# Gardlin/PCR-CG

Hardware: AMD Instinct MI355X
Metric: fragment-pairs/s KPFCNN+GCN fwd, 30k-pt pairs (higher is better)
Workload: dtype f32

## Files before the change

include/pcrcg.h:

```cpp
#ifndef PCRCG_H
#define PCRCG_H

#include <stddef.h>
#include <stdint.h>

#ifdef __cplusplus
extern "C" {
#endif

#define PCRCG_OK 0
#define PCRCG_EBADARG (-1)
#define PCRCG_EWORKSPACE (-2)
#define PCRCG_ELAUNCH (-3)
#define PCRCG_ECAPACITY (-4)

#define PCRCG_KPOINTS 15

const char* pcrcg_last_error(void);
#define PCRCG_ABI_VERSION 4
int pcrcg_abi_version(void);

int pcrcg_debug_set(const char* spec);
int pcrcg_debug_release(void);

size_t pcrcg_grid_subsample_ws_bytes(int n, int nb);
int pcrcg_grid_subsample_batch(const float* pts, int n, const int* len, int nb, float dl, int max_p,
                               float* out_pts, int* out_len, int* out_m, void* ws, size_t ws_bytes,
                               void* stream);

size_t pcrcg_umap_order_ws_bytes(int m);
int pcrcg_umap_order(const uint64_t* keys, int m, int* order, void* ws, size_t ws_bytes, void* stream);

size_t pcrcg_cellgrid_ws_bytes(int ns, int nb);
int pcrcg_cellgrid_build(const float* sup, int ns, const int* slen, int nb, float radius, void* grid,
                         size_t grid_bytes, void* stream);
int pcrcg_radius_query(const float* q, int nq, const int* qlen, int ns, const int* slen, int nb,
                       float radius, const void* grid, int cols, int64_t* out_idx, int* out_count,
                       int* out_max_count, int* status, void* stream);
int pcrcg_radius_query_ex(const float* q, int nq, const int* qlen, int ns, const int* slen, int nb,
                          float radius, const void* grid, int cols, int64_t* out_idx, int* out_count,
                          int* out_max_count, int* status, int* out_tie_rows, int* out_tie_count, void* stream);
int pcrcg_radius_query_groups(const float* q, int nq, const int* qlen, int ns, const int* slen, int nb, int group,
                              float radius, const void* grid, int cols, int64_t* out_idx, int* out_count,
                              int* out_max_count, int* status, int* out_tie_rows, int* out_tie_count, void* stream);
int pcrcg_radius_query_cells(const void* qgrid, const float* q, int nq, const int* qlen, const void* sgrid, int ns,
                             const int* slen, int nb, int group, float radius, int cols, int64_t* out_idx, int* out_count,
                             int* out_max_count, int* status, int* out_tie_rows, int* out_tie_count, void* stream);
size_t pcrcg_radius_neighbors_ws_bytes(int ns, int nb);
int pcrcg_radius_neighbors_batch(const float* q, int nq, const float* sup, int ns, const int* qlen,
                                 const int* slen, int nb, float radius, int cols, int64_t* out_idx,
                                 int* out_count, int* out_max_count, int* status, void* ws,
                                 size_t ws_bytes, void* stream);

#define PCRCG_MAX_REORDER_JOBS 12
typedef struct pcrcg_reorder_job {
    const float* q;
    const int* qlen;
    const int* rows;
    const int* count;
    int64_t* idx;
    int nq, nbq, cloud0, nrows, max_count, cols;
    float radius;
    int group;
    const float* sup;
    const void* forest;
    int forest_ns, forest_nb;
} pcrcg_reorder_job;
size_t pcrcg_kdforest_ws_bytes(int ns, int nb);
int pcrcg_kdforest_build(const float* sup, int ns, const int* slen, int nb, void* forest, size_t forest_bytes,
                         void* stream);
int pcrcg_radius_reorder(const float* q, int nq, const int* qlen, int nbq, const float* sup, int ns, int nb,
                         const void* forest, int cloud0, float radius, const int* rows, int nrows, const int* count,
                         int max_count, int cols, int64_t* idx, int* status, void* stream);
int pcrcg_radius_reorder_jobs(const pcrcg_reorder_job* jobs, int njobs, const float* sup, int ns, int nb,
                              const void* forest, int* status, void* stream);

size_t pcrcg_kpconv_ws_bytes(int ns);
int pcrcg_kpconv_aggregate(const float* q_pts, int nq, const float* s_pts, int ns, const int64_t* idx,
                           int h, int ld_idx, const float* x, int cin, const float* kp, float extent,
                           float* wf, float* inv_n, void* ws, size_t ws_bytes, void* stream);
int pcrcg_kpconv_aggregate_bf16(const float* q_pts, int nq, const float* s_pts, int ns, const int64_t* idx, int h,
                                int ld_idx, const float* x, int cin, const float* kp, float extent, void* x_bf16,
                                void* wf_bf16, float* inv_n, void* ws, size_t ws_bytes, void* stream);

int pcrcg_query_walk(const float* points, int n, int* walk, int* key, void* stream);
int pcrcg_kpconv_aggregate_walk(const float* q_pts, int nq, const float* s_pts, int ns, const int64_t* idx,
                                int h, int ld_idx, const float* x, int cin, const float* kp, float extent,
                                float* wf, float* inv_n, void* ws, size_t ws_bytes, const int* walk, void* stream);
int pcrcg_kpconv_aggregate_bf16_walk(const float* q_pts, int nq, const float* s_pts, int ns, const int64_t* idx, int h,
                                     int ld_idx, const float* x, int cin, const float* kp, float extent, void* x_bf16,
                                     void* wf_bf16, float* inv_n, void* ws, size_t ws_bytes, const int* walk, void* stream);
int pcrcg_gather_max_walk(const float* x, int ns, int c, const int64_t* idx, int nq, int h, int ld_idx,
                          float* out, const int* walk, void* stream);

void pcrcg_profile_kpconv(int enable);
int pcrcg_profile_kpconv_read(float* ms, int* nq, int* h, int* cin, int* cout, int* kind, int cap);

int pcrcg_gemm_f32(const float* a, int lda, const float* b, int ldb, int trans_b, float* c, int ldc, int m,
                   int n, int k, const float* row_scale, const float* bias, void* stream);
size_t pcrcg_gemm_colstats_bytes(int m, int n);
int pcrcg_gemm_f32_colstats(const float* a, int lda, const float* b, int ldb, int trans_b, float* c, int ldc,
                            int m, int n, int k, const float* row_scale, const float* bias, void* colstats,
                            size_t colstats_bytes, int* h_chunks, void* stream);
int pcrcg_gemm_bf16a_f32_colstats(const void* a_bf16, int lda, const float* b, int ldb, float* c, int ldc, int m, int n,
                                  int k, const float* row_scale, const float* bias, void* colstats,
                                  size_t colstats_bytes, int* h_chunks, void* stream);

int pcrcg_gemm_f32_fused(const float* a, int lda, const int64_t* idx, int ld_idx, int ns, const float* zero_row,
                         const void* a_sums, double a_count, float a_eps, float a_slope, const float* b, int ldb,
                         const float* bias, float* c, int ldc, int m, int n, int k, int accumulate, void* stream);

void pcrcg_gemm_set_mode(int mode);
int pcrcg_gemm_get_mode(void);
int pcrcg_gemm_redo_counts(unsigned long long* out2, int reset);
void pcrcg_thread_shares_gpu(int on);

int pcrcg_gather_max(const float* x, int ns, int c, const int64_t* idx, int nq, int h, int ld_idx,
                     float* out, void* stream);
int pcrcg_gather_first(const float* x, int ns, int c, const int64_t* idx, int nq, int ld_idx, float* out,
                       int ld_out, void* stream);
size_t pcrcg_instnorm_ws_bytes(int c);
int pcrcg_instnorm_stats_from_partials(const void* partials, int chunks, int c, double count, float eps,
                                       float* stats, void* stream);
int pcrcg_instnorm_stats(const float* x, int n, int c, int ldx, float eps, float* stats, void* ws,
                         size_t ws_bytes, void* stream);
int pcrcg_instnorm_apply(const float* x, int n, int c, int ldx, const float* stats, const float* res,
                         int ldr, const float* res_stats, float slope, float* y, int ldy, void* stream);
int pcrcg_instnorm_colsums(const float* x, int n, int c, int ldx, void* sums, void* stream);
int pcrcg_instnorm_apply_sums(const float* x, int n, int c, int ldx, const void* sums, double count, float eps,
                              const float* res, int ldr, const void* res_sums, float slope, float* y, int ldy,
                              void* stream);

int pcrcg_fill2d(float* dst, int ld, int rows, int cols, float value, void* stream);
int pcrcg_inject_image_features(const float* fmap, int c, int h, int w, const float* valid, const int64_t* inds2d,
                                const int64_t* inds3d, int n, long row_offset, long n_rows, float* x, int ldx,
                                void* stream);

typedef struct pcrcg_image_frame {
    const float* fmap;
    const float* depth;
    const float* valid;
    float world2camera[16];
    float intrinsics[16];
    float thresh;
    int h, w;
    int depth_h, depth_w;
    int target;
} pcrcg_image_frame;

size_t pcrcg_project_depth_ws_bytes(int n);
int pcrcg_project_depth(const float* points, int n, const float* depth, int h, int w, const float* h_world2camera,
                        const float* h_intrinsics, float thresh, int64_t* inds2d, int64_t* inds3d, int* k, void* ws,
                        size_t ws_bytes, void* stream);
int pcrcg_inject_frames(const float* points, long n_points, long len_src, const pcrcg_image_frame* h_frames, int n_frames,
                        int c, float* x, int ldx, void* stream);
int pcrcg_superglue_valid_maps(const float* keypoints0, int n0, const float* keypoints1, int n1, const int64_t* matches,
                               const float* confidence, int window, int map_w, int map_h, float* src_valid, float* tgt_valid,
                               void* stream);

int pcrcg_knn(const float* coords, int n, int k, int* idx, void* stream);
size_t pcrcg_edgeconv_ws_bytes(int c);
int pcrcg_edgeconv_reduce(const float* ctr, int ld_ctr, const float* nbr, int ld_nbr, const int* idx,
                          int n, int k, int c, float eps, float* emax, int ld_emax, float* stats,
                          void* ws, size_t ws_bytes, void* stream);
int pcrcg_edgeconv_reduce_sums(const float* ctr, int ld_ctr, const float* nbr, int ld_nbr, const int* idx, int n, int k,
                               int c, float* emax, int ld_emax, void* sums, void* stream);
int pcrcg_softmax_rows(float* x, int rows, int cols, int ld, float scale, void* stream);
int pcrcg_attention_supported(int d);
int pcrcg_attention(const float* q, int ldq, const float* k, int ldk, const float* v, int ldv, float* out, int ldo, int n,
                    int ms, int heads, int d, float scale, void* stream);
int pcrcg_softmax_matvec(const float* x, int rows, int cols, int ld, float scale, const float* vec, int ldv, float* y,
                         int ldy, void* stream);

int pcrcg_check_status(const int* status, void* stream);

int pcrcg_copy2d(const float* src, int ld_src, float* dst, int ld_dst, int rows, int cols, void* stream);
int pcrcg_add(const float* a, const float* b, float* dst, long n, void* stream);
int pcrcg_l2norm_rows(const float* src, int ld_src, float* dst, int ld_dst, int rows, int cols, void* stream);
int pcrcg_sigmoid_scores(const float* src, int ld_src, float* dst, int rows, void* stream);

#define PCRCG_MAX_LEVELS 8
#define PCRCG_MAX_BLOCKS 32
#define PCRCG_MAX_GNN 8

enum { PCRCG_BLK_SIMPLE = 0, PCRCG_BLK_RESNETB = 1, PCRCG_BLK_UNARY = 2, PCRCG_BLK_LAST_UNARY = 3,
       PCRCG_BLK_UPSAMPLE = 4 };

typedef struct pcrcg_block {
    int type;
    int layer;
    int strided;
    int in_dim, out_dim;
    int mid_dim;
    float extent;
    const float* kp;
    const float* kp_w;
    const float* kp_wt;
    const float* kp_w_pad;
    int cin_pad;
    const float* unary1;
    const float* unary2;
    const float* shortcut;
    const float* mlp;
    int mlp_ld;
    const float* mlp_skip;
    int mlp_skip_ld, skip_dim;
} pcrcg_block;

typedef struct pcrcg_gnn_layer {
    int cross;
    const float* edge1;
    const float* edge2;
    const float* conv3;
    const float *wq, *bq, *wk, *bk, *wv, *bv;
    const float *wm, *bm;
    const float *w0, *b0;
    const float *w3, *b3;
} pcrcg_gnn_layer;

typedef struct pcrcg_model {
    int n_enc, n_dec, n_gnn;
    pcrcg_block enc[PCRCG_MAX_BLOCKS];
    pcrcg_block dec[PCRCG_MAX_BLOCKS];
    pcrcg_gnn_layer gnn[PCRCG_MAX_GNN];
    int enc_skip[PCRCG_MAX_BLOCKS];
    int dec_concat[PCRCG_MAX_BLOCKS];
    int enc_out_dim, gnn_dim, heads, knn_k, final_dim;
    const float *bottle_w, *bottle_b;
    const float *proj_gnn_w, *proj_gnn_b;
    const float *proj_score_w, *proj_score_b;
    float temperature;
    int feature_bf16;
} pcrcg_model;

typedef struct pcrcg_table { const int64_t* idx; int rows, cols, ld; } pcrcg_table;

typedef struct pcrcg_batch {
    int n_levels;
    const float* points[PCRCG_MAX_LEVELS];
    int n_points[PCRCG_MAX_LEVELS];
    pcrcg_table neighbors[PCRCG_MAX_LEVELS], pools[PCRCG_MAX_LEVELS], upsamples[PCRCG_MAX_LEVELS];
    const float* features;
    int feat_dim;
    int len_src_c;
    const int* stack_lengths[PCRCG_MAX_LEVELS];
} pcrcg_batch;

typedef struct pcrcg_outputs {
    float* feats_f;
    float* scores_overlap;
    float* scores_saliency;
} pcrcg_outputs;

size_t pcrcg_kpfcnn_ws_bytes(const pcrcg_model* model, const pcrcg_batch* batch);
int pcrcg_kpfcnn_forward(const pcrcg_model* model, const pcrcg_batch* batch, const pcrcg_outputs* out, void* ws,
                         size_t ws_bytes, void* stream);

size_t pcrcg_kpfcnn_group_ws_bytes(const pcrcg_model* model, const pcrcg_batch* batches, int n);
int pcrcg_kpfcnn_forward_group(const pcrcg_model* model, const pcrcg_batch* batches, const pcrcg_outputs* outs, int n,
                               void* ws, size_t ws_bytes, void* stream);

typedef struct pcrcg_pyramid_cfg {
    int n_levels;
    float r_conv[PCRCG_MAX_LEVELS], r_pool[PCRCG_MAX_LEVELS], dl[PCRCG_MAX_LEVELS];
    int has_conv[PCRCG_MAX_LEVELS], pooled[PCRCG_MAX_LEVELS], limit[PCRCG_MAX_LEVELS];
    int tie_order;
    int group;
    int up_nearest;
    double shrink;
    void* side_stream;
    void* side_stream2;
} pcrcg_pyramid_cfg;
typedef struct pcrcg_pyramid_restore {
    int njobs;
    pcrcg_reorder_job jobs[PCRCG_MAX_REORDER_JOBS];
    int* tie_status;
} pcrcg_pyramid_restore;
size_t pcrcg_pyramid_ws_bytes(int n0, int nb, const pcrcg_pyramid_cfg* cfg);
int pcrcg_pyramid_build(const float* pts, int n0, const int* len, int nb, const pcrcg_pyramid_cfg* cfg, void* ws,
                        size_t ws_bytes, int* h_scratch, pcrcg_batch* out, int* h_lengths, int* h_status,
                        pcrcg_pyramid_restore* deferred, void* stream);
int pcrcg_pyramid_build_parts(const float* const* pts_parts, const int* n_parts, const int* const* len_parts,
                              const int* nb_parts, int parts, const pcrcg_pyramid_cfg* cfg, void* ws, size_t ws_bytes,
                              int* h_scratch, pcrcg_batch* out, int* h_lengths, int* h_status,
                              pcrcg_pyramid_restore* deferred, void* stream);
int pcrcg_pyramid_restore_run(const pcrcg_pyramid_restore* r, int* h_status, void* stream);

int pcrcg_stream_create(void** stream, int priority);
int pcrcg_stream_destroy(void* stream);
int pcrcg_stream_pipe_classes(void* const* streams, int n, int* cls, void* scratch);

typedef struct pcrcg_ransac_trace {
    int* samples;
    int* pass;
    float* xf32;
    double* xf64;
    int* valid_ids;
    int* counts;
    double* sums;
} pcrcg_ransac_trace;

size_t pcrcg_ransac_ws_bytes(int n, int m, int max_iteration, int max_validation);
int pcrcg_feature_match(const float* src_feat, int ld_src, int n, const float* tgt_feat, int ld_tgt, int m, int c, int mutual,
                        int* corr, int* k, void* ws, size_t ws_bytes, void* stream);
int pcrcg_ransac(const float* src, int n, const float* tgt, int m, const void* grid, const int* corr, int k_max, const int* k,
                 int ransac_n, double threshold, double edge_similarity, int distance_check, int max_iteration,
                 int max_validation, uint64_t seed, double* out_transform, double* out_stats, const pcrcg_ransac_trace* trace,
                 void* ws, size_t ws_bytes, void* stream);

size_t pcrcg_ransac_batch_ws_bytes(int B, int n_total, int m_total, int max_iteration, int max_validation);
int pcrcg_feature_match_batch(const float* src_feat, int ld_src, const int* src_off, int n_total, int n_max,
                              const float* tgt_feat, int ld_tgt, const int* tgt_off, int m_total, int m_max, int c, int B,
                              int* corr, int* k, void* ws, size_t ws_bytes, void* stream);
int pcrcg_ransac_batch(const float* src, const int* src_off, const float* tgt, const int* tgt_off, int m_total, const void* grid,
                       const int* corr, const int* k, int B, int ransac_n, double threshold, double edge_similarity,
                       int distance_check, int max_iteration, int max_validation, const uint64_t* seeds,
                       double* out_transform, double* out_stats, void* ws, size_t ws_bytes, void* stream);

typedef struct pcrcg_icp_trace {
    double* transforms;
    int* counts;
    double* sums;
    int* corr;
} pcrcg_icp_trace;

size_t pcrcg_icp_batch_ws_bytes(int B, int n_total, int m_total, int max_iteration);
int pcrcg_icp_batch(const float* src, const int* src_off, int n_total, int n_max, const int* tgt_off, int m_total,
                    const void* grid, const double* init, int B, double max_correspondence_distance, int max_iteration,
                    double relative_fitness, double relative_rmse, double* out_transform, double* out_stats,
                    const pcrcg_icp_trace* trace, void* ws, size_t ws_bytes, void* stream);

size_t pcrcg_voxel_down_sample_ws_bytes(int B, int n_total);
int pcrcg_voxel_down_sample_batch(const float* pts, const int* off, int n_total, int B, double voxel_size, double* out_pts,
                                  int* out_len, int* out_first, int* out_count, void* ws, size_t ws_bytes, void* stream);

size_t pcrcg_weighted_sample_ws_bytes(int S, int n_total);
int pcrcg_weighted_sample_batch(const float* scores, const int* seg_off, int S, int n_keep, const uint64_t* seeds, int* out_idx,
                                const int* out_off, void* ws, size_t ws_bytes, void* stream);

size_t pcrcg_inlier_stats_batch_ws_bytes(int B, int n_total, int m_total);
int pcrcg_inlier_stats_batch(const float* src, const float* src_feat, int ld_src, const int* src_off, int n_total, int n_max,
                             const float* tgt, const float* tgt_feat, int ld_tgt, const int* tgt_off, int m_total, int m_max,
                             int c, int B, const float* rt, const float* thr, int n_thr, int* counts, int* k_mutual,
                             float* dist, int* mutual, int* arg_s, int* arg_t, void* ws, size_t ws_bytes, void* stream);


size_t pcrcg_chamfer_batch_ws_bytes(int B, int n_total, int m_total, int r_total);
int pcrcg_chamfer_batch(const float* src, const int* src_off, int n_total, const float* ref, const int* ref_off, int m_total,
                        const float* raw, const int* raw_off, int r_total, int B, const float* pred, const float* gt,
                        float* chamfer, float* mean_src, float* mean_ref, float* d_src, int* arg_src, float* d_ref, int* arg_ref,
                        void* ws, size_t ws_bytes, void* stream);

size_t pcrcg_res50unet_arena_bytes(int out_ch);
int pcrcg_res50unet_pack(void* const* h_tensors, int n_tensors, int out_ch, float* arena, void* stream);
// ... 21 lines not shown
```

pcrcg_amd/_lib.py:

```python
import ctypes
import os

_HERE = os.path.dirname(os.path.abspath(__file__))
LIB_PATH = os.path.join(_HERE, "libpcrcg_hip.so")


def lib_identity():
    import hashlib
    with open(LIB_PATH, "rb") as f:
        return LIB_PATH, hashlib.sha256(f.read()).hexdigest()[:16]

ABI_VERSION = 4

c_int, c_float, c_void_p, c_size_t = ctypes.c_int, ctypes.c_float, ctypes.c_void_p, ctypes.c_size_t

SIGNATURES = {
    "pcrcg_last_error": (ctypes.c_char_p, []),
    "pcrcg_abi_version": (c_int, []),
    "pcrcg_debug_set": (c_int, [ctypes.c_char_p]),
    "pcrcg_check_status": (c_int, [c_void_p, c_void_p]),
    "pcrcg_grid_subsample_ws_bytes": (c_size_t, [c_int, c_int]),
    "pcrcg_grid_subsample_batch": (c_int, [c_void_p, c_int, c_void_p, c_int, c_float, c_int, c_void_p, c_void_p,
                                           c_void_p, c_void_p, c_size_t, c_void_p]),
    "pcrcg_umap_order_ws_bytes": (c_size_t, [c_int]),
    "pcrcg_umap_order": (c_int, [c_void_p, c_int, c_void_p, c_void_p, c_size_t, c_void_p]),
    "pcrcg_cellgrid_ws_bytes": (c_size_t, [c_int, c_int]),
    "pcrcg_cellgrid_build": (c_int, [c_void_p, c_int, c_void_p, c_int, c_float, c_void_p, c_size_t, c_void_p]),
    "pcrcg_radius_query": (c_int, [c_void_p, c_int, c_void_p, c_int, c_void_p, c_int, c_float, c_void_p, c_int,
                                   c_void_p, c_void_p, c_void_p, c_void_p, c_void_p]),
    "pcrcg_radius_query_ex": (c_int, [c_void_p, c_int, c_void_p, c_int, c_void_p, c_int, c_float, c_void_p, c_int,
                                      c_void_p, c_void_p, c_void_p, c_void_p, c_void_p, c_void_p, c_void_p]),
    "pcrcg_radius_query_groups": (c_int, [c_void_p, c_int, c_void_p, c_int, c_void_p, c_int, c_int, c_float, c_void_p, c_int,
                                          c_void_p, c_void_p, c_void_p, c_void_p, c_void_p, c_void_p, c_void_p]),
    "pcrcg_radius_query_cells": (c_int, [c_void_p, c_void_p, c_int, c_void_p, c_void_p, c_int, c_void_p, c_int, c_int, c_float,
                                         c_int, c_void_p, c_void_p, c_void_p, c_void_p, c_void_p, c_void_p, c_void_p]),
    "pcrcg_kdforest_ws_bytes": (c_size_t, [c_int, c_int]),
    "pcrcg_kdforest_build": (c_int, [c_void_p, c_int, c_void_p, c_int, c_void_p, c_size_t, c_void_p]),
    "pcrcg_radius_reorder": (c_int, [c_void_p, c_int, c_void_p, c_int, c_void_p, c_int, c_int, c_void_p, c_int,
                                     c_float, c_void_p, c_int, c_void_p, c_int, c_int, c_void_p, c_void_p, c_void_p]),
    "pcrcg_radius_reorder_jobs": (c_int, [c_void_p, c_int, c_void_p, c_int, c_int, c_void_p, c_void_p, c_void_p]),
    "pcrcg_radius_neighbors_ws_bytes": (c_size_t, [c_int, c_int]),
    "pcrcg_radius_neighbors_batch": (c_int, [c_void_p, c_int, c_void_p, c_int, c_void_p, c_void_p, c_int, c_float,
                                             c_int, c_void_p, c_void_p, c_void_p, c_void_p, c_void_p, c_size_t,
                                             c_void_p]),
    "pcrcg_kpconv_ws_bytes": (c_size_t, [c_int]),
    "pcrcg_kpconv_aggregate": (c_int, [c_void_p, c_int, c_void_p, c_int, c_void_p, c_int, c_int, c_void_p, c_int,
                                       c_void_p, c_float, c_void_p, c_void_p, c_void_p, c_size_t, c_void_p]),
    "pcrcg_kpconv_aggregate_bf16": (c_int, [c_void_p, c_int, c_void_p, c_int, c_void_p, c_int, c_int, c_void_p, c_int,
                                            c_void_p, c_float, c_void_p, c_void_p, c_void_p, c_void_p, c_size_t,
                                            c_void_p]),
    "pcrcg_query_walk": (c_int, [c_void_p, c_int, c_void_p, c_void_p, c_void_p]),
    "pcrcg_kpconv_aggregate_walk": (c_int, [c_void_p, c_int, c_void_p, c_int, c_void_p, c_int, c_int, c_void_p, c_int,
                                            c_void_p, c_float, c_void_p, c_void_p, c_void_p, c_size_t, c_void_p, c_void_p]),
    "pcrcg_kpconv_aggregate_bf16_walk": (c_int, [c_void_p, c_int, c_void_p, c_int, c_void_p, c_int, c_int, c_void_p, c_int,
                                                 c_void_p, c_float, c_void_p, c_void_p, c_void_p, c_void_p, c_size_t,
                                                 c_void_p, c_void_p]),
    "pcrcg_gather_max_walk": (c_int, [c_void_p, c_int, c_int, c_void_p, c_int, c_int, c_int, c_void_p, c_void_p, c_void_p]),
    "pcrcg_profile_kpconv": (None, [c_int]),
    "pcrcg_profile_kpconv_read": (c_int, [c_void_p, c_void_p, c_void_p, c_void_p, c_void_p, c_void_p, c_int]),
    "pcrcg_gemm_f32": (c_int, [c_void_p, c_int, c_void_p, c_int, c_int, c_void_p, c_int, c_int, c_int, c_int,
                               c_void_p, c_void_p, c_void_p]),
    "pcrcg_gemm_colstats_bytes": (c_size_t, [c_int, c_int]),
    "pcrcg_gemm_f32_colstats": (c_int, [c_void_p, c_int, c_void_p, c_int, c_int, c_void_p, c_int, c_int, c_int, c_int,
                                        c_void_p, c_void_p, c_void_p, c_size_t, c_void_p, c_void_p]),
    "pcrcg_gemm_bf16a_f32_colstats": (c_int, [c_void_p, c_int, c_void_p, c_int, c_void_p, c_int, c_int, c_int, c_int,
                                              c_void_p, c_void_p, c_void_p, c_size_t, c_void_p, c_void_p]),
    "pcrcg_gemm_f32_fused": (c_int, [c_void_p, c_int, c_void_p, c_int, c_int, c_void_p, c_void_p, ctypes.c_double, c_float,
                                     c_float, c_void_p, c_int, c_void_p, c_void_p, c_int, c_int, c_int, c_int, c_int, c_void_p]),
    "pcrcg_gemm_set_mode": (None, [c_int]),
    "pcrcg_gemm_get_mode": (c_int, []),
    "pcrcg_gemm_redo_counts": (c_int, [c_void_p, c_int]),
    "pcrcg_instnorm_stats_from_partials": (c_int, [c_void_p, c_int, c_int, ctypes.c_double, c_float, c_void_p,
                                                   c_void_p]),
    "pcrcg_gather_max": (c_int, [c_void_p, c_int, c_int, c_void_p, c_int, c_int, c_int, c_void_p, c_void_p]),
    "pcrcg_gather_first": (c_int, [c_void_p, c_int, c_int, c_void_p, c_int, c_int, c_void_p, c_int, c_void_p]),
    "pcrcg_instnorm_ws_bytes": (c_size_t, [c_int]),
    "pcrcg_instnorm_stats": (c_int, [c_void_p, c_int, c_int, c_int, c_float, c_void_p, c_void_p, c_size_t, c_void_p]),
    "pcrcg_instnorm_apply": (c_int, [c_void_p, c_int, c_int, c_int, c_void_p, c_void_p, c_int, c_void_p, c_float,
                                     c_void_p, c_int, c_void_p]),
    "pcrcg_instnorm_colsums": (c_int, [c_void_p, c_int, c_int, c_int, c_void_p, c_void_p]),
    "pcrcg_instnorm_apply_sums": (c_int, [c_void_p, c_int, c_int, c_int, c_void_p, ctypes.c_double, c_float, c_void_p, c_int,
                                          c_void_p, c_float, c_void_p, c_int, c_void_p]),
    "pcrcg_fill2d": (c_int, [c_void_p, c_int, c_int, c_int, c_float, c_void_p]),
    "pcrcg_inject_image_features": (c_int, [c_void_p, c_int, c_int, c_int, c_void_p, c_void_p, c_void_p, c_int, ctypes.c_long,
                                            ctypes.c_long, c_void_p, c_int, c_void_p]),
    "pcrcg_project_depth_ws_bytes": (c_size_t, [c_int]),
    "pcrcg_project_depth": (c_int, [c_void_p, c_int, c_void_p, c_int, c_int, c_void_p, c_void_p, c_float, c_void_p, c_void_p,
                                    c_void_p, c_void_p, c_size_t, c_void_p]),
    "pcrcg_inject_frames": (c_int, [c_void_p, ctypes.c_long, ctypes.c_long, c_void_p, c_int, c_int, c_void_p, c_int, c_void_p]),
    "pcrcg_superglue_valid_maps": (c_int, [c_void_p, c_int, c_void_p, c_int, c_void_p, c_void_p, c_int, c_int, c_int, c_void_p,
                                           c_void_p, c_void_p]),
    "pcrcg_knn": (c_int, [c_void_p, c_int, c_int, c_void_p, c_void_p]),
    "pcrcg_edgeconv_ws_bytes": (c_size_t, [c_int]),
    "pcrcg_edgeconv_reduce": (c_int, [c_void_p, c_int, c_void_p, c_int, c_void_p, c_int, c_int, c_int, c_float,
                                      c_void_p, c_int, c_void_p, c_void_p, c_size_t, c_void_p]),
    "pcrcg_edgeconv_reduce_sums": (c_int, [c_void_p, c_int, c_void_p, c_int, c_void_p, c_int, c_int, c_int, c_void_p, c_int,
                                           c_void_p, c_void_p]),
    "pcrcg_softmax_rows": (c_int, [c_void_p, c_int, c_int, c_int, c_float, c_void_p]),
    "pcrcg_attention_supported": (c_int, [c_int]),
    "pcrcg_attention": (c_int, [c_void_p, c_int, c_void_p, c_int, c_void_p, c_int, c_void_p, c_int, c_int, c_int, c_int,
                                c_int, c_float, c_void_p]),
    "pcrcg_softmax_matvec": (c_int, [c_void_p, c_int, c_int, c_int, c_float, c_void_p, c_int, c_void_p, c_int, c_void_p]),
    "pcrcg_copy2d": (c_int, [c_void_p, c_int, c_void_p, c_int, c_int, c_int, c_void_p]),
    "pcrcg_add": (c_int, [c_void_p, c_void_p, c_void_p, ctypes.c_long, c_void_p]),
    "pcrcg_l2norm_rows": (c_int, [c_void_p, c_int, c_void_p, c_int, c_int, c_int, c_void_p]),
    "pcrcg_sigmoid_scores": (c_int, [c_void_p, c_int, c_void_p, c_int, c_void_p]),
    "pcrcg_kpfcnn_ws_bytes": (c_size_t, [c_void_p, c_void_p]),
    "pcrcg_kpfcnn_group_ws_bytes": (c_size_t, [c_void_p, c_void_p, c_int]),
    "pcrcg_kpfcnn_forward_group": (c_int, [c_void_p, c_void_p, c_void_p, c_int, c_void_p, c_size_t, c_void_p]),
    "pcrcg_kpfcnn_forward": (c_int, [c_void_p, c_void_p, c_void_p, c_void_p, c_size_t, c_void_p]),
    "pcrcg_pyramid_ws_bytes": (c_size_t, [c_int, c_int, c_void_p]),
    "pcrcg_pyramid_build": (c_int, [c_void_p, c_int, c_void_p, c_int, c_void_p, c_void_p, c_size_t, c_void_p, c_void_p,
                                    c_void_p, c_void_p, c_void_p, c_void_p]),
    "pcrcg_pyramid_build_parts": (c_int, [c_void_p, c_void_p, c_void_p, c_void_p, c_int, c_void_p, c_void_p, c_size_t, c_void_p,
                                          c_void_p, c_void_p, c_void_p, c_void_p, c_void_p]),
    "pcrcg_pyramid_restore_run": (c_int, [c_void_p, c_void_p, c_void_p]),
    "pcrcg_debug_release": (c_int, []),
    "pcrcg_stream_pipe_classes": (c_int, [c_void_p, c_int, c_void_p, c_void_p]),
    "pcrcg_thread_shares_gpu": (None, [c_int]),
    "pcrcg_stream_create": (c_int, [c_void_p, c_int]),
    "pcrcg_stream_destroy": (c_int, [c_void_p]),
    "pcrcg_ransac_ws_bytes": (c_size_t, [c_int, c_int, c_int, c_int]),
    "pcrcg_feature_match": (c_int, [c_void_p, c_int, c_int, c_void_p, c_int, c_int, c_int, c_int, c_void_p, c_void_p,
                                    c_void_p, c_size_t, c_void_p]),
    "pcrcg_ransac": (c_int, [c_void_p, c_int, c_void_p, c_int, c_void_p, c_void_p, c_int, c_void_p, c_int, ctypes.c_double,
                             ctypes.c_double, c_int, c_int, c_int, ctypes.c_uint64, c_void_p, c_void_p, c_void_p, c_void_p,
                             c_size_t, c_void_p]),
    "pcrcg_ransac_batch_ws_bytes": (c_size_t, [c_int, c_int, c_int, c_int, c_int]),
    "pcrcg_feature_match_batch": (c_int, [c_void_p, c_int, c_void_p, c_int, c_int, c_void_p, c_int, c_void_p, c_int, c_int,
                                          c_int, c_int, c_void_p, c_void_p, c_void_p, c_size_t, c_void_p]),
    "pcrcg_ransac_batch": (c_int, [c_void_p, c_void_p, c_void_p, c_void_p, c_int, c_void_p, c_void_p, c_void_p, c_int, c_int,
                                   ctypes.c_double, ctypes.c_double, c_int, c_int, c_int, c_void_p, c_void_p, c_void_p,
                                   c_void_p, c_size_t, c_void_p]),
    "pcrcg_inlier_stats_batch_ws_bytes": (c_size_t, [c_int, c_int, c_int]),
    "pcrcg_inlier_stats_batch": (c_int, [c_void_p, c_void_p, c_int, c_void_p, c_int, c_int, c_void_p, c_void_p, c_int, c_void_p,
                                         c_int, c_int, c_int, c_int, c_void_p, c_void_p, c_int, c_void_p, c_void_p, c_void_p,
                                         c_void_p, c_void_p, c_void_p, c_void_p, c_size_t, c_void_p]),
    "pcrcg_icp_batch_ws_bytes": (c_size_t, [c_int, c_int, c_int, c_int]),
    "pcrcg_icp_batch": (c_int, [c_void_p, c_void_p, c_int, c_int, c_void_p, c_int, c_void_p, c_void_p, c_int, ctypes.c_double,
# ... 108 lines not shown
```

pcrcg_amd/csrc/common.h:

```cpp
#pragma once
#include <hip/hip_runtime.h>

#include <cstdarg>
#include <cstdint>
#include <cstdio>
#include <map>
#include <mutex>

#include "pcrcg.h"

namespace pcrcg {

void set_error(const char* fmt, ...);

inline hipStream_t as_stream(void* s) { return reinterpret_cast<hipStream_t>(s); }

struct Carver {
    char* base;
    size_t cap;
    size_t off = 0;
    Carver(void* ws, size_t bytes) : base(static_cast<char*>(ws)), cap(bytes) {}
    template <typename T>
    T* take(size_t count) {
        size_t bytes = (count * sizeof(T) + 255) & ~size_t(255);
        T* p = reinterpret_cast<T*>(base + off);
        off += bytes;
        return p;
    }
    bool ok() const { return off <= cap; }
};
inline size_t carve_bytes(size_t count, size_t elem) { return (count * elem + 255) & ~size_t(255); }

size_t scan_ws_bytes(int n);
int exclusive_scan_i32(const int* in, int* out, int n, int* total, void* ws, hipStream_t stream);

constexpr int kWave = 64;

bool instnorm_pack_ok(int c, int ldx, int ldy);
int instnorm_apply_pack(const float* x, int n, int c, int ldx, const float* stats, const double* sums, double count, float eps,
                        float slope, float* y, int ldy, const float* s_pts, float4* pk, hipStream_t st);
size_t colstats_ws_bytes(int c);
int colstats_finalize(const double* partial, int nchunks, int c, double count, float eps, float* stats,
                      hipStream_t st);
int colstats_chunks();
float4* kpconv_pk_ptr(void* ws, size_t ws_bytes, int ns);

class StreamScratch {
public:
    explicit StreamScratch(bool cleared = false);
    void* get(hipStream_t st, size_t bytes, size_t slack = 0);
    void release();
private:
    struct Buf { void* p = nullptr; size_t bytes = 0; };
    const bool cleared_;
    std::mutex mu_;
    std::map<hipStream_t, Buf> bufs_;
};

int kpconv_pack(const float* x, int ns, int cin, const float* s_pts, void* ws, size_t ws_bytes, hipStream_t st,
                unsigned short* x_bf16 = nullptr);
int kpconv_aggregate_rows(const float* q_pts, int nq, const float* s_pts, int ns, const int64_t* idx, int h, int ld_idx,
                          const float* x, int cin, const float* kp, float extent, float* wf, float* inv_n, void* ws,
                          size_t ws_bytes, hipStream_t st, bool pack, bool stream_out, int c1_ld = 0,
                          const int* walk = nullptr);
int kpconv_aggregate_bf16(const float* q_pts, int nq, const float* s_pts, int ns, const int64_t* idx, int h, int ld_idx,
                          const float* x, unsigned short* x_bf16, int cin, const float* kp, float extent,
                          unsigned short* wf_bf16, float* inv_n, void* ws, size_t ws_bytes, hipStream_t st,
                          const int* walk = nullptr);

int query_walk_multi(const float* const* pts, const int* n, int* const* walk, int* const* key, int count, hipStream_t st);

struct NormJob {
    const float* x; const double* sums; const float* res; const double* res_sums; float* y;
    const float* s_pts; float4* pk;
    int n; double count;
    float* stats_out = nullptr;
};
int instnorm_apply_sums_multi(const NormJob* jobs, int count, int c, int ldx, float eps, int ldr, float slope, int ldy, bool pack,
                              hipStream_t st);
bool instnorm_sums_ok(int c, int ldx, int ldy, int ldr = 0);

struct GatherJob { const float* x; const int64_t* idx; float* out; int ns, nq, h, ld_idx; const int* walk = nullptr; };
int gather_max_multi(const GatherJob* jobs, int count, int c, hipStream_t st);
int heads_multi(const float* const* x, const int* rows, int count, int ld, int fd, float* const* feats, float* const* s_ov,
                float* const* s_sal, hipStream_t st);
int copy2d_multi(const float* const* src, float* const* dst, const int* rows, int count, int ld_src, int ld_dst, int cols,
                 hipStream_t st);
int instnorm_colsums_multi(const float* const* x, double* const* sums, const int* n, int count, int c, int ldx, hipStream_t st);

struct EdgeCloud {
    const float* ctr; const float* nbr; const int* idx; float* emax; double* sums; int n, k;
};
bool edgeconv_rows_ok(const EdgeCloud* cl, int count, int ld_ctr, int ld_nbr, int ld_emax, int c);
int edgeconv_rows_multi(const EdgeCloud* cl, int count, int ld_ctr, int ld_nbr, int ld_emax, int c, bool atomic, int* nchunks_out,
                        hipStream_t st);

struct AttnCloud { const float* q; const float* k; const float* v; float* out; int n, ms; };
bool attention_mfma_ok(const AttnCloud* cl, int count, int ldq, int ldk, int ldv, int d);
int attention_mfma_multi(const AttnCloud* cl, int count, int ldq, int ldk, int ldv, int ldo, int heads, int d, float scale,
                         hipStream_t st);
bool attention_bwd_mfma_ok(int n, int ms, int d, int ldq, int ldk, int ldv, int ld_do);
int attention_bwd_mfma(const float* q, int ldq, const float* k, int ldk, const float* v, int ldv, const float* o, int ldo,
                       const float* d_o, int ld_do, float* dq, int ld_dq, float* dk, int ld_dk, float* dv, int ld_dv, int n, int ms,
                       int heads, int d, float scale, hipStream_t st);

struct DebugOpts {
    int stat_sums = 1;
    int stat_sums_rows = 1 << 30;
    int att_mfma = 1;
    int radius_blocks = 0;
    int kd_blocks = 0;
    int att_tq = 16;
    int kd_spin_limit = 0;
    int gemm_log = 0;
    int x6_tile = -1, x6_splitk = 0, x6_t1 = 1, x6_t2 = 1, x6_order = -1, x6_big = 0, x6_h2 = 1;
    int train_side_stream = 1;
    int gemm_tile = -1, gemm_splitk = 0, gemm_split_target = 768;
    int deterministic = 0;
    int bwd_mfma = 1;
    int walk = 1;
};
const DebugOpts& debug_opts();

struct KpProfScope {
    hipStream_t st;
    hipEvent_t a, b;
    int nq, h, cin, cout, kind;
    bool on;
    KpProfScope(hipStream_t s, int nq, int h, int cin, int cout, int kind);
    ~KpProfScope();
};

}

#define PCRCG_CHECK_ARG(cond)                                                        \
    do {                                                                             \
        if (!(cond)) {                                                               \
            pcrcg::set_error("%s: bad argument: %s", __func__, #cond);               \
            return PCRCG_EBADARG;                                                    \
        }                                                                            \
    } while (0)

#define PCRCG_CHECK_WS(carver)                                                                     \
    do {                                                                                           \
        if (!(carver).ok()) {                                                                      \
            pcrcg::set_error("%s: workspace too small (%zu needed, %zu given)", __func__,          \
                             (carver).off, (carver).cap);                                          \
            return PCRCG_EWORKSPACE;                                                               \
        }                                                                                          \
    } while (0)

#define PCRCG_CHECK_HIP(expr)                                                                  \
    do {                                                                                       \
        hipError_t e_ = (expr);                                                                \
        if (e_ != hipSuccess) {                                                                \
            pcrcg::set_error("%s: %s failed: %s", __func__, #expr, hipGetErrorString(e_));     \
            return PCRCG_ELAUNCH;                                                              \
        }                                                                                      \
    } while (0)
// ... 26 lines not shown
```

pcrcg_amd/csrc/kpconv.hip:

```cpp
#include <mutex>
#include <vector>

#include <hip/hip_ext.h>

#include "common.h"

namespace pcrcg {

struct ProfRec { hipEvent_t a, b; int nq, h, cin, cout, kind; };
static int g_prof_on = 0;
static std::vector<ProfRec> g_prof;
static std::mutex g_prof_mu;

KpProfScope::KpProfScope(hipStream_t s, int nq_, int h_, int cin_, int cout_, int kind_)
    : st(s), a(nullptr), b(nullptr), nq(nq_), h(h_), cin(cin_), cout(cout_), kind(kind_),
      on((g_prof_on & (kind_ == 3 ? 2 : kind_ == 4 ? 4 : 1)) != 0) {
    if (!on) return;
    (void)hipEventCreate(&a);
    (void)hipEventCreate(&b);
}
KpProfScope::~KpProfScope() {
    if (!on) return;
    std::lock_guard<std::mutex> lock(g_prof_mu);
    g_prof.push_back({a, b, nq, h, cin, cout, kind});
}

namespace {

constexpr int K = PCRCG_KPOINTS;
constexpr int kWavesPerBlock = 4;
typedef float f32x4 __attribute__((ext_vector_type(4)));

__device__ __forceinline__ unsigned short bf16_rne(float f) {
    const unsigned u = __float_as_uint(f);
    return (unsigned short)((u + 0x7fffu + ((u >> 16) & 1u)) >> 16);
}

__global__ void __launch_bounds__(256) k_row_positive(const float* __restrict__ x, int ns, int cin,
                                                       const float* __restrict__ s_pts, unsigned char* __restrict__ pos,
                                                       float4* __restrict__ pk, unsigned short* __restrict__ xb) {
    const int lane = threadIdx.x & 63;
    const int row = blockIdx.x * (blockDim.x >> 6) + (threadIdx.x >> 6);
    if (row >= ns) return;
    float s = 0.0f;
    for (int c = lane; c < cin; c += 64) {
        const float v = x[(long)row * cin + c];
        s += v;
        if (xb) xb[(long)row * cin + c] = bf16_rne(v);
    }
#pragma unroll
    for (int d = 32; d >= 1; d >>= 1) s += __shfl_xor(s, d, 64);
    if (lane == 0) {
        pos[row] = s > 0.0f ? 1 : 0;
        pk[row] = make_float4(s_pts[3 * (long)row], s_pts[3 * (long)row + 1], s_pts[3 * (long)row + 2], s > 0.0f ? 1.f : 0.f);
    }
}

__global__ void __launch_bounds__(256) k_pack_c1(const float* __restrict__ x, int ns, const float* __restrict__ s_pts,
                                                  float4* __restrict__ pk) {
    const int row = blockIdx.x * 256 + threadIdx.x;
    if (row < ns) pk[row] = make_float4(s_pts[3 * (long)row], s_pts[3 * (long)row + 1], s_pts[3 * (long)row + 2], x[row]);
}

struct __attribute__((packed, aligned(4))) P3 { float x, y, z; };

__device__ __forceinline__ float4 load4(const float* p) { return *reinterpret_cast<const float4*>(p); }
__device__ __forceinline__ float4 load4(const unsigned short* p) {
    const uint2 u = *reinterpret_cast<const uint2*>(p);
    return make_float4(__uint_as_float(u.x << 16), __uint_as_float(u.x & 0xffff0000u), __uint_as_float(u.y << 16),
                       __uint_as_float(u.y & 0xffff0000u));
}

template <int NB, bool NT_STORE, typename FT, bool TAIL = false>
__global__ void __launch_bounds__(kWavesPerBlock * 64) k_kpconv_mfma(
    const float* __restrict__ q_pts, int nq, const float* __restrict__ s_pts, int ns,
    const long long* __restrict__ idx, int H, int ld_idx, const FT* __restrict__ x, int cin,
    const float* __restrict__ kp, float extent, const float4* __restrict__ pk, FT* __restrict__ wf,
    float* __restrict__ inv_n, int nchunk, const int* __restrict__ walk) {
    constexpr bool BF16 = sizeof(FT) == 2;
    constexpr int STEPS = NB >= 4 ? 2 : 4;
    const int lane = threadIdx.x & 63;
    const int hsub = lane >> 4, j = lane & 15;
    const int wave = __builtin_amdgcn_readfirstlane((int)(threadIdx.x >> 6));
    long gw = (long)blockIdx.x * kWavesPerBlock + wave;
    long nw = (long)gridDim.x * kWavesPerBlock;
    long items = (long)nq * nchunk;
    int pos0 = 0;
    if (walk) {
        const int xcd = blockIdx.x & 7, slot = blockIdx.x >> 3, nslot = gridDim.x >> 3;
        const int xq = nq >> 3, xr = nq & 7;
        pos0 = xcd < xr ? xcd * (xq + 1) : xr * (xq + 1) + (xcd - xr) * xq;
        gw = (long)slot * kWavesPerBlock + wave;
        nw = (long)nslot * kWavesPerBlock;
        const int cnt = __builtin_amdgcn_readfirstlane(xq + (xcd < xr ? 1 : 0));
        items = (long)cnt * nchunk;
    }
    const bool jvalid = j < K;
    const float kpx = jvalid ? kp[3 * j] : 0.f, kpy = jvalid ? kp[3 * j + 1] : 0.f, kpz = jvalid ? kp[3 * j + 2] : 0.f;
    const float inv_extent = 1.0f / extent;

    for (long item = gw; item < items; item += nw) {
        const int p = (int)(item / nchunk), chunk = (int)(item - (long)p * nchunk);
        int q = p;
        if (walk) {
            q = walk[pos0 + p];
            q = q < 0 ? 0 : (q < nq ? q : nq - 1);
        }
        const int c0 = chunk * 64 * NB;
        const float qx = q_pts[3 * (long)q], qy = q_pts[3 * (long)q + 1], qz = q_pts[3 * (long)q + 2];
        f32x4 acc[NB][4];
#pragma unroll
        for (int b = 0; b < NB; ++b)
#pragma unroll
            for (int n = 0; n < 4; ++n) acc[b][n] = (f32x4){0.f, 0.f, 0.f, 0.f};
        int npos = 0;
        float ta0 = 0.f, ta1 = 0.f, ta2 = 0.f, ta3 = 0.f;
        for (int hc = 0; hc < H; hc += 64) {
            const int h = hc + lane;
            const long long iv = idx[(long)q * ld_idx + (h < H ? h : H - 1)];
            const int i = (h < H && iv >= 0 && iv < ns) ? (int)iv : -1;
            const long ic = i >= 0 ? i : 0;
            const float4 sp = pk[ic];
            const float px = sp.x - qx, py = sp.y - qy, pz = sp.z - qz;
            if (chunk == 0) npos += __popcll(__ballot(i >= 0 && sp.w != 0.f));
            const unsigned long long real_lanes = __ballot(i >= 0);
            const int hn_all = H - hc < 64 ? H - hc : 64;
            const int hn_real = real_lanes ? 64 - (int)__clzll(real_lanes) : 0;
            const int hn = hn_real < hn_all ? hn_real : hn_all;
            for (int h0 = 0; h0 < hn; h0 += 4 * STEPS) {
                float w[STEPS];
                float4 v[STEPS][NB];
                float4 vt[STEPS];
#pragma unroll
                for (int s = 0; s < STEPS; ++s) {
                    const int src = h0 + 4 * s + hsub;
                    const int ii = __shfl(i, src, 64);
                    const float nx = __shfl(px, src, 64), ny = __shfl(py, src, 64), nz = __shfl(pz, src, 64);
                    const bool real = ii >= 0 && h0 + 4 * s < hn;
                    w[s] = 0.f;
                    if (real && jvalid) {
                        const float dx = nx - kpx, dy = ny - kpy, dz = nz - kpz;
                        w[s] = fmaxf(1.0f - __builtin_amdgcn_sqrtf(dx * dx + dy * dy + dz * dz) * inv_extent, 0.0f);
                    }
                    const FT* xrow = x + (long)(real ? ii : 0) * cin;
#pragma unroll
                    for (int b = 0; b < NB; ++b) {
                        const int c = c0 + 64 * b + 4 * j;
                        const float4 t = load4(xrow + (c < cin ? c : cin - 4));
                        const bool ok = real && c < cin;
                        v[s][b] = make_float4(ok ? t.x : 0.f, ok ? t.y : 0.f, ok ? t.z : 0.f, ok ? t.w : 0.f);
                    }
                    if constexpr (TAIL) {
                        const float4 t = load4(xrow + 64 * NB);
                        vt[s] = make_float4(real ? t.x : 0.f, real ? t.y : 0.f, real ? t.z : 0.f, real ? t.w : 0.f);
                    }
                }
#pragma unroll
                for (int s = 0; s < STEPS; ++s)
#pragma unroll
                    for (int b = 0; b < NB; ++b) {
                        acc[b][0] = __builtin_amdgcn_mfma_f32_16x16x4f32(w[s], v[s][b].x, acc[b][0], 0, 0, 0);
                        acc[b][1] = __builtin_amdgcn_mfma_f32_16x16x4f32(w[s], v[s][b].y, acc[b][1], 0, 0, 0);
                        acc[b][2] = __builtin_amdgcn_mfma_f32_16x16x4f32(w[s], v[s][b].z, acc[b][2], 0, 0, 0);
                        acc[b][3] = __builtin_amdgcn_mfma_f32_16x16x4f32(w[s], v[s][b].w, acc[b][3], 0, 0, 0);
                    }
                if constexpr (TAIL) {
#pragma unroll
                    for (int s = 0; s < STEPS; ++s) {
                        ta0 += w[s] * vt[s].x;
                        ta1 += w[s] * vt[s].y;
                        ta2 += w[s] * vt[s].z;
                        ta3 += w[s] * vt[s].w;
                    }
                }
            }
        }
        FT* o = wf + (long)q * K * cin + c0;
#pragma unroll
        for (int b = 0; b < NB; ++b) {
            const int c = 64 * b + 4 * j;
            if (c0 + c >= cin) continue;
#pragma unroll
            for (int r = 0; r < 4; ++r) {
                const int k = 4 * hsub + r;
                if (k < K) {
                    if constexpr (BF16) {
                        typedef unsigned v2u __attribute__((ext_vector_type(2)));
                        const v2u val = {(unsigned)bf16_rne(acc[b][0][r]) | ((unsigned)bf16_rne(acc[b][1][r]) << 16),
                                         (unsigned)bf16_rne(acc[b][2][r]) | ((unsigned)bf16_rne(acc[b][3][r]) << 16)};
                        __builtin_nontemporal_store(val, reinterpret_cast<v2u*>(o + (long)k * cin + c));
                    } else {
                        typedef float v4f __attribute__((ext_vector_type(4)));
                        const v4f val = {acc[b][0][r], acc[b][1][r], acc[b][2][r], acc[b][3][r]};
                        if (NT_STORE) __builtin_nontemporal_store(val, reinterpret_cast<v4f*>(o + (long)k * cin + c));
                        else *reinterpret_cast<v4f*>(o + (long)k * cin + c) = val;
                    }
                }
            }
        }
        if constexpr (TAIL) {
            ta0 += __shfl_xor(ta0, 16, 64); ta1 += __shfl_xor(ta1, 16, 64); ta2 += __shfl_xor(ta2, 16, 64); ta3 += __shfl_xor(ta3, 16, 64);
            ta0 += __shfl_xor(ta0, 32, 64); ta1 += __shfl_xor(ta1, 32, 64); ta2 += __shfl_xor(ta2, 32, 64); ta3 += __shfl_xor(ta3, 32, 64);
            if (hsub == 0 && jvalid) {
                typedef float v4f __attribute__((ext_vector_type(4)));
                const v4f val = {ta0, ta1, ta2, ta3};
                v4f* dst = reinterpret_cast<v4f*>(reinterpret_cast<float*>(wf) + (long)q * K * cin + (long)j * cin + 64 * NB);
                if (NT_STORE) __builtin_nontemporal_store(val, dst);
// ... 43 lines not shown
            const float v = p.w;
            xv[b] = real ? v : 0.f;
        }
#pragma unroll
        for (int b = 0; b < C1_BATCH; ++b) {
            npos += xv[b] > 0.0f ? 1 : 0;
#pragma unroll
            for (int k = 0; k < K; ++k) {
                const float dx = nx[b] - kpx[k], dy = ny[b] - kpy[k], dz = nz[b] - kpz[k];
                acc[k] = fmaf(fmaxf(1.0f - __builtin_amdgcn_sqrtf(dx * dx + dy * dy + dz * dz) * inv_extent, 0.0f),
                              xv[b], acc[k]);
            }
        }
    }
#pragma unroll
    for (int d = 1; d < C1_PARTS; d <<= 1) {
#pragma unroll
        for (int k = 0; k < K; ++k) acc[k] += __shfl_xor(acc[k], d, 64);
        npos += __shfl_xor(npos, d, 64);
    }
    if (qraw >= nq) return;
#pragma unroll
    for (int k = 0; k < K; ++k)
        if ((k & (C1_PARTS - 1)) == part) wf[(long)q * ld_wf + k] = acc[k];
    if (ld_wf > K && part == C1_PARTS - 1) wf[(long)q * ld_wf + K] = 0.f;
    if (part == 0) inv_n[q] = 1.0f / (float)(npos > 1 ? npos : 1);
}

__global__ void __launch_bounds__(kWavesPerBlock * 64) k_kpconv_generic(
    const float* __restrict__ q_pts, int nq, const float* __restrict__ s_pts, int ns,
    const long long* __restrict__ idx, int H, int ld_idx, const float* __restrict__ x, int cin,
    const float* __restrict__ kp, float extent, const unsigned char* __restrict__ pos, float* __restrict__ wf,
    float* __restrict__ inv_n) {
    __shared__ __attribute__((aligned(16))) float s_w[kWavesPerBlock][64][16];
    __shared__ int s_idx[kWavesPerBlock][64];
    const int lane = threadIdx.x & 63, wave = threadIdx.x >> 6;
    const int gw = blockIdx.x * kWavesPerBlock + wave, nw = gridDim.x * kWavesPerBlock;
    const float inv_extent = 1.0f / extent;
    for (int q = gw; q < nq; q += nw) {
        const float qx = q_pts[3 * (long)q], qy = q_pts[3 * (long)q + 1], qz = q_pts[3 * (long)q + 2];
        int npos = 0;
        for (int cbase = 0; cbase < cin; cbase += 64) {
            float acc[K];
#pragma unroll
            for (int k = 0; k < K; ++k) acc[k] = 0.0f;
            for (int hc = 0; hc < H; hc += 64) {
                const int h = hc + lane;
                int i = -1;
                if (h < H) {
                    const long long v = idx[(long)q * ld_idx + h];
                    i = (v >= 0 && v < ns) ? (int)v : -1;
                }
                __builtin_amdgcn_wave_barrier();
                if (i >= 0) {
                    const float nx = s_pts[3 * (long)i] - qx, ny = s_pts[3 * (long)i + 1] - qy,
                                nz = s_pts[3 * (long)i + 2] - qz;
                    for (int k = 0; k < K; ++k) {
                        const float dx = nx - kp[3 * k], dy = ny - kp[3 * k + 1], dz = nz - kp[3 * k + 2];
                        s_w[wave][lane][k] = fmaxf(1.0f - sqrtf(dx * dx + dy * dy + dz * dz) * inv_extent, 0.0f);
                    }
                }
                s_idx[wave][lane] = i;
                if (cbase == 0) npos += __popcll(__ballot(i >= 0 && pos[i >= 0 ? i : 0] != 0));
                __builtin_amdgcn_wave_barrier();
                const int hn = H - hc < 64 ? H - hc : 64;
                const int c = cbase + lane;
                for (int hh = 0; hh < hn; ++hh) {
                    const int ii = s_idx[wave][hh];
                    if (ii < 0) continue;
                    const float xv = c < cin ? x[(long)ii * cin + c] : 0.0f;
#pragma unroll
                    for (int k = 0; k < K; ++k) acc[k] = fmaf(s_w[wave][hh][k], xv, acc[k]);
                }
            }
            const int c = cbase + lane;
            if (c < cin)
#pragma unroll
                for (int k = 0; k < K; ++k) wf[(long)q * K * cin + (long)k * cin + c] = acc[k];
        }
        if (lane == 0) inv_n[q] = 1.0f / (float)(npos > 1 ? npos : 1);
    }
}

}

float4* kpconv_pk_ptr(void* ws, size_t ws_bytes, int ns) {
    Carver cv(ws, ws_bytes);
    cv.take<unsigned char>((size_t)ns + 1);
    float4* pk = cv.take<float4>((size_t)ns + 1);
    return cv.ok() ? pk : nullptr;
}

int kpconv_pack(const float* x, int ns, int cin, const float* s_pts, void* ws, size_t ws_bytes, hipStream_t st,
                unsigned short* x_bf16) {
    Carver cv(ws, ws_bytes);
    unsigned char* pos = cv.take<unsigned char>((size_t)ns + 1);
    float4* pk = cv.take<float4>((size_t)ns + 1);
    PCRCG_CHECK_WS(cv);
    if (ns > 0) hipLaunchKernelGGL(k_row_positive, dim3((ns + 3) / 4), dim3(256), 0, st, x, ns, cin, s_pts, pos, pk, x_bf16);
    PCRCG_CHECK_LAUNCH();
    return PCRCG_OK;
}

}

using namespace pcrcg;

extern "C" {

void pcrcg_profile_kpconv(int enable) {
    std::lock_guard<std::mutex> lock(g_prof_mu);
    for (auto& r : g_prof) { (void)hipEventDestroy(r.a); (void)hipEventDestroy(r.b); }
    g_prof.clear();
    g_prof_on = enable;
}

int pcrcg_profile_kpconv_read(float* ms, int* nq, int* h, int* cin, int* cout, int* kind, int cap) {
    std::lock_guard<std::mutex> lock(g_prof_mu);
    int n = 0;
    for (auto& r : g_prof) {
        if (n >= cap) break;
        if (hipEventSynchronize(r.b) != hipSuccess) return -1;
        float t = 0.f;
        if (hipEventElapsedTime(&t, r.a, r.b) != hipSuccess) return -1;
        ms[n] = t; nq[n] = r.nq; h[n] = r.h; cin[n] = r.cin; cout[n] = r.cout; kind[n] = r.kind;
        ++n;
    }
    return n;
}

size_t pcrcg_kpconv_ws_bytes(int ns) {
    const size_t n = (size_t)(ns > 0 ? ns : 0) + 1;
    return carve_bytes(n, 1) + carve_bytes(n, sizeof(float4));
}

int pcrcg_kpconv_aggregate(const float* q_pts, int nq, const float* s_pts, int ns, const int64_t* idx,
                           int h, int ld_idx, const float* x, int cin, const float* kp, float extent,
                           float* wf, float* inv_n, void* ws, size_t ws_bytes, void* stream) {
    return kpconv_aggregate_rows(q_pts, nq, s_pts, ns, idx, h, ld_idx, x, cin, kp, extent, wf, inv_n, ws, ws_bytes,
                                 as_stream(stream), true, true, 0);
}

int pcrcg_kpconv_aggregate_bf16(const float* q_pts, int nq, const float* s_pts, int ns, const int64_t* idx, int h,
                                int ld_idx, const float* x, int cin, const float* kp, float extent, void* x_bf16,
                                void* wf_bf16, float* inv_n, void* ws, size_t ws_bytes, void* stream) {
    return kpconv_aggregate_bf16(q_pts, nq, s_pts, ns, idx, h, ld_idx, x, static_cast<unsigned short*>(x_bf16), cin, kp,
                                 extent, static_cast<unsigned short*>(wf_bf16), inv_n, ws, ws_bytes, as_stream(stream));
}
}

namespace pcrcg {

int kpconv_aggregate_rows(const float* q_pts, int nq, const float* s_pts, int ns, const int64_t* idx, int h, int ld_idx,
                          const float* x, int cin, const float* kp, float extent, float* wf, float* inv_n, void* ws,
                          size_t ws_bytes, hipStream_t st, bool pack, bool stream_out, int c1_ld, const int* walk) {
    PCRCG_CHECK_ARG(nq >= 0 && ns >= 0 && h >= 1 && ld_idx >= h && cin >= 1 && (c1_ld == 0 || c1_ld == K || c1_ld == K + 1));
    PCRCG_CHECK_ARG(extent > 0.0f);
    if (nq == 0) return PCRCG_OK;
    PCRCG_CHECK_ARG(q_pts && s_pts && idx && x && kp && wf && inv_n && ws);
    PCRCG_CHECK_ARG(ns >= 1);
    Carver cv(ws, ws_bytes);
    unsigned char* pos = cv.take<unsigned char>((size_t)ns + 1);
    float4* pk = cv.take<float4>((size_t)ns + 1);
    PCRCG_CHECK_WS(cv);
    const long long* idx_ll = reinterpret_cast<const long long*>(idx);
    const int max_blocks = 256 * 32;
    auto blocks_for = [&](long waves) {
        long b = (waves + kWavesPerBlock - 1) / kWavesPerBlock;
        return (int)(b > max_blocks ? max_blocks : b);
    };
    auto blocks_walk = [&](int nchunk) {
        const int b = blocks_for((long)((nq + 7) / 8) * nchunk);
        return 8 * (b > max_blocks / 8 ? max_blocks / 8 : b);
    };
    if (cin == 1) {
        if (pack) hipLaunchKernelGGL(k_pack_c1, dim3((ns + 255) / 256), dim3(256), 0, st, x, ns, s_pts, pk);
        KpProfScope prof_scope(st, nq, h, cin, 0, 0);
        hipExtLaunchKernelGGL(k_kpconv_c1, dim3((int)(((long)nq * C1_PARTS + 255) / 256)), dim3(256), 0, st, prof_scope.a,
                              prof_scope.b, 0, q_pts, nq, s_pts, ns, idx_ll, h, ld_idx, (const float4*)pk, kp, extent, wf,
                              inv_n, c1_ld > 0 ? c1_ld : K);
        PCRCG_CHECK_LAUNCH();
        return PCRCG_OK;
    }
    if (pack && ns > 0)
        hipLaunchKernelGGL(k_row_positive, dim3((ns + 3) / 4), dim3(256), 0, st, x, ns, cin, s_pts, pos, pk,
                           (unsigned short*)nullptr);
    KpProfScope prof_scope(st, nq, h, cin, 0, 0);
    const bool aligned = (cin % 4 == 0) && ((reinterpret_cast<uintptr_t>(x) & 15) == 0) &&
                         ((reinterpret_cast<uintptr_t>(wf) & 15) == 0);
    if (!aligned) {
        hipLaunchKernelGGL(k_kpconv_generic, dim3(blocks_for(nq)), dim3(kWavesPerBlock * 64), 0, st, q_pts, nq, s_pts,
                           ns, idx_ll, h, ld_idx, x, cin, kp, extent, pos, wf, inv_n);
        PCRCG_CHECK_LAUNCH();
        return PCRCG_OK;
    }
    if (cin == 68 || cin == 132) {
        const int blocks = walk ? blocks_walk(1) : blocks_for((long)nq);
#define LAUNCH_T(NBV, NT)                                                                                                        \
        hipExtLaunchKernelGGL((k_kpconv_mfma<NBV, NT, float, true>), dim3(blocks), dim3(kWavesPerBlock * 64), 0, st, prof_scope.a, \
                              prof_scope.b, 0, q_pts, nq, s_pts, ns, idx_ll, h, ld_idx, x, cin, kp, extent,                      \
                              (const float4*)pk, wf, inv_n, 1, walk)
        if (cin == 132) { if (stream_out) LAUNCH_T(2, true); else LAUNCH_T(2, false); }
        else { if (stream_out) LAUNCH_T(1, true); else LAUNCH_T(1, false); }
#undef LAUNCH_T
        PCRCG_CHECK_LAUNCH();
        return PCRCG_OK;
    }
    const int nblk = (cin + 63) / 64;
    int nb = nblk >= 4 ? 4 : (nblk >= 2 ? 2 : 1);
    while (nb > 1 && ((long)nq * ((nblk + nb - 1) / nb) < 16384 || nblk % nb != 0)) nb >>= 1;
    const int nchunk = (nblk + nb - 1) / nb;
    const int blocks = walk ? blocks_walk(nchunk) : blocks_for((long)nq * nchunk);
#define LAUNCH(NBV, NT)                                                                                                 \
    hipExtLaunchKernelGGL((k_kpconv_mfma<NBV, NT, float>), dim3(blocks), dim3(kWavesPerBlock * 64), 0, st, prof_scope.a, \
                          prof_scope.b, 0, q_pts, nq, s_pts, ns, idx_ll, h, ld_idx, x, cin, kp, extent,                 \
                          (const float4*)pk, wf, inv_n, nchunk, walk)
    if (stream_out) {
        if (nb == 4) LAUNCH(4, true);
        else if (nb == 2) LAUNCH(2, true);
        else LAUNCH(1, true);
    } else {
        if (nb == 4) LAUNCH(4, false);
        else if (nb == 2) LAUNCH(2, false);
        else LAUNCH(1, false);
    }
#undef LAUNCH
    PCRCG_CHECK_LAUNCH();
    return PCRCG_OK;
}

int kpconv_aggregate_bf16(const float* q_pts, int nq, const float* s_pts, int ns, const int64_t* idx, int h, int ld_idx,
                          const float* x, unsigned short* x_bf16, int cin, const float* kp, float extent,
                          unsigned short* wf_bf16, float* inv_n, void* ws, size_t ws_bytes, hipStream_t st, const int* walk) {
    PCRCG_CHECK_ARG(nq >= 0 && ns >= 1 && h >= 1 && ld_idx >= h && cin >= 4 && cin % 4 == 0 && extent > 0.0f);
    if (nq == 0) return PCRCG_OK;
    PCRCG_CHECK_ARG(q_pts && s_pts && idx && x && x_bf16 && kp && wf_bf16 && inv_n && ws);
    PCRCG_CHECK_ARG((reinterpret_cast<uintptr_t>(x_bf16) & 7) == 0 && (reinterpret_cast<uintptr_t>(wf_bf16) & 7) == 0);
    PCRCG_PROPAGATE(kpconv_pack(x, ns, cin, s_pts, ws, ws_bytes, st, x_bf16));
    Carver cv(ws, ws_bytes);
    cv.take<unsigned char>((size_t)ns + 1);
    float4* pk = cv.take<float4>((size_t)ns + 1);
    const long long* idx_ll = reinterpret_cast<const long long*>(idx);
    const int nblk = (cin + 63) / 64;
    int nb = nblk >= 4 ? 4 : (nblk >= 2 ? 2 : 1);
    while (nb > 1 && ((long)nq * ((nblk + nb - 1) / nb) < 16384 || nblk % nb != 0)) nb >>= 1;
    const int nchunk = (nblk + nb - 1) / nb;
    long blocks = ((long)nq * nchunk + kWavesPerBlock - 1) / kWavesPerBlock;
    if (blocks > 256 * 32) blocks = 256 * 32;
    if (walk) {
        blocks = ((long)((nq + 7) / 8) * nchunk + kWavesPerBlock - 1) / kWavesPerBlock;
        blocks = 8 * (blocks > 32 * 32 ? 32 * 32 : blocks);
    }
    KpProfScope prof_scope(st, nq, h, cin, 0, 2);
#define LAUNCHB(NBV)                                                                                                      \
    hipExtLaunchKernelGGL((k_kpconv_mfma<NBV, true, unsigned short>), dim3((int)blocks), dim3(kWavesPerBlock * 64), 0, st, \
                          prof_scope.a, prof_scope.b, 0, q_pts, nq, s_pts, ns, idx_ll, h, ld_idx, x_bf16, cin, kp, extent, \
                          (const float4*)pk, wf_bf16, inv_n, nchunk, walk)
    if (nb == 4) LAUNCHB(4);
    else if (nb == 2) LAUNCHB(2);
    else LAUNCHB(1);
#undef LAUNCHB
    PCRCG_CHECK_LAUNCH();
    return PCRCG_OK;
}

}
```

pcrcg_amd/csrc/pointops.hip:

```cpp
#include "common.h"

namespace pcrcg {
namespace {

constexpr int kWavesPerBlock = 4;

struct GatherMulti { const float* x[4]; const long long* idx[4]; float* out[4]; int ns[4], nq[4], h[4], ld_idx[4]; const int* walk[4]; };
template <bool VEC4>
__global__ void __launch_bounds__(kWavesPerBlock * 64) k_gather_max(GatherMulti mm, int c, int nchunk) {
    const int g = blockIdx.y;
    const float* __restrict__ x = mm.x[g];
    const long long* __restrict__ idx = mm.idx[g];
    float* __restrict__ out = mm.out[g];
    const int ns = mm.ns[g], nq = mm.nq[g], h = mm.h[g], ld_idx = mm.ld_idx[g];
    const int lane = threadIdx.x & 63;
    const int* __restrict__ walk = mm.walk[g];
    const int wave = __builtin_amdgcn_readfirstlane((int)(threadIdx.x >> 6));
    long item = (long)blockIdx.x * kWavesPerBlock + wave, items = (long)nq * nchunk;
    int pos0 = 0;
    if (walk) {
        const int xcd = blockIdx.x & 7, slot = blockIdx.x >> 3;
        const int xq = nq >> 3, xr = nq & 7;
        pos0 = xcd < xr ? xcd * (xq + 1) : xr * (xq + 1) + (xcd - xr) * xq;
        item = (long)slot * kWavesPerBlock + wave;
// ... 99 lines not shown
                                                         double count, float eps, float* __restrict__ stats) {
    const int lane = threadIdx.x & 63;
    const int ch = blockIdx.x * (blockDim.x >> 6) + (threadIdx.x >> 6);
    if (ch >= c) return;
    double s = 0.0, sq = 0.0;
    for (int k = lane; k < nchunks; k += 64) {
        s += partial[(long)ch * nchunks + k];
        sq += partial[((long)c + ch) * nchunks + k];
    }
#pragma unroll
    for (int d = 32; d >= 1; d >>= 1) {
        s += __shfl_xor(s, d, 64);
        sq += __shfl_xor(sq, d, 64);
    }
    if (lane != 0) return;
    const double mean = s / count;
    double var = sq / count - mean * mean;
    if (var < 0.0) var = 0.0;
    stats[2 * ch] = (float)mean;
    stats[2 * ch + 1] = (float)(1.0 / sqrt(var + (double)eps));
}

__global__ void __launch_bounds__(256) k_instnorm_apply(const float* __restrict__ x, int n, int c, int ldx,
                                                         const float* __restrict__ stats, const float* __restrict__ res,
                                                         int ldr, const float* __restrict__ res_stats, float slope,
                                                         float* __restrict__ y, int ldy) {
    const long e = (long)blockIdx.x * blockDim.x + threadIdx.x;
    if (e >= (long)n * c) return;
    const long r = e / c;
    const int ch = (int)(e - r * c);
    float v = (x[r * ldx + ch] - stats[2 * ch]) * stats[2 * ch + 1];
    if (res) {
        float rv = res[r * ldr + ch];
        if (res_stats) rv = (rv - res_stats[2 * ch]) * res_stats[2 * ch + 1];
        v += rv;
    }
    y[r * ldy + ch] = v >= 0.f ? v : v * slope;
}

__global__ void __launch_bounds__(256) k_instnorm_apply4(const float* __restrict__ x, int n, int c4, int ldx,
                                                          const float* __restrict__ stats, const float* __restrict__ res,
                                                          int ldr, const float* __restrict__ res_stats, float slope,
                                                          float* __restrict__ y, int ldy) {
    const long e = (long)blockIdx.x * blockDim.x + threadIdx.x;
    if (e >= (long)n * c4) return;
    const long r = e / c4;
    const int q = (int)(e - r * c4);
    const float4 xv = *reinterpret_cast<const float4*>(x + r * ldx + 4 * q);
    const float4 s0 = *reinterpret_cast<const float4*>(stats + 8 * q), s1 = *reinterpret_cast<const float4*>(stats + 8 * q + 4);
    float4 v = make_float4((xv.x - s0.x) * s0.y, (xv.y - s0.z) * s0.w, (xv.z - s1.x) * s1.y, (xv.w - s1.z) * s1.w);
    if (res) {
        float4 rv = *reinterpret_cast<const float4*>(res + r * ldr + 4 * q);
        if (res_stats) {
            const float4 t0 = *reinterpret_cast<const float4*>(res_stats + 8 * q),
                         t1 = *reinterpret_cast<const float4*>(res_stats + 8 * q + 4);
            rv = make_float4((rv.x - t0.x) * t0.y, (rv.y - t0.z) * t0.w, (rv.z - t1.x) * t1.y, (rv.w - t1.z) * t1.w);
        }
        v.x += rv.x; v.y += rv.y; v.z += rv.z; v.w += rv.w;
    }
    v.x = v.x >= 0.f ? v.x : v.x * slope;
    v.y = v.y >= 0.f ? v.y : v.y * slope;
    v.z = v.z >= 0.f ? v.z : v.z * slope;
    v.w = v.w >= 0.f ? v.w : v.w * slope;
    *reinterpret_cast<float4*>(y + r * ldy + 4 * q) = v;
}

__device__ __forceinline__ void stats4_from_sums(const double* __restrict__ sums, int c, int ch, double count, float eps,
                                                 float4& mean, float4& rstd) {
    float m[4], r[4];
#pragma unroll
    for (int i = 0; i < 4; ++i) {
        const double mu = sums[ch + i] / count;
        double var = sums[c + ch + i] / count - mu * mu;
        if (var < 0.0) var = 0.0;
        m[i] = (float)mu;
        r[i] = (float)(1.0 / sqrt(var + (double)eps));
    }
    mean = make_float4(m[0], m[1], m[2], m[3]);
    rstd = make_float4(r[0], r[1], r[2], r[3]);
}

struct NormMulti {
    const float* x[4]; const double* sums[4]; const float* res[4]; const double* res_sums[4]; float* y[4];
    const float* s_pts[4]; float4* pk[4];
    int n[4]; double count[4];
    float* stats_out[4];
};
template <int RES>
__global__ void __launch_bounds__(256) k_instnorm_apply4_sums(NormMulti mm, int c4, int ldx, float eps, int ldr, float slope, int ldy,
                                                               int rows_per_block) {
    const int g = blockIdx.y;
    const float* __restrict__ x = mm.x[g];
    const double* __restrict__ sums = mm.sums[g];
    const float* __restrict__ res = mm.res[g];
    const double* __restrict__ res_sums = mm.res_sums[g];
    float* __restrict__ y = mm.y[g];
    const int n = mm.n[g];
    const double count = mm.count[g];
    if ((long)blockIdx.x * rows_per_block >= n) return;
    const int cb = c4 < 256 ? c4 : 256;
    const int rp = 256 / cb;
    const int r_lo = blockIdx.x * rows_per_block, r_hi = min(n, r_lo + rows_per_block);
    for (int qb = 0; qb < c4; qb += cb) {
        const int q = qb + (int)(threadIdx.x % cb);
        float4 m0, s0, m1 = make_float4(0.f, 0.f, 0.f, 0.f), s1 = make_float4(1.f, 1.f, 1.f, 1.f);
        stats4_from_sums(sums, 4 * c4, 4 * q, count, eps, m0, s0);
        if (RES == 2) stats4_from_sums(res_sums, 4 * c4, 4 * q, count, eps, m1, s1);
        if (blockIdx.x == 0 && threadIdx.x < cb && mm.stats_out[g]) {
            float4* so = reinterpret_cast<float4*>(mm.stats_out[g] + 8 * q);
            so[0] = make_float4(m0.x, s0.x, m0.y, s0.y);
            so[1] = make_float4(m0.z, s0.z, m0.w, s0.w);
        }
        auto finish = [&](const float4& xv, float4 rv, long r) {
            float4 v = make_float4((xv.x - m0.x) * s0.x, (xv.y - m0.y) * s0.y, (xv.z - m0.z) * s0.z, (xv.w - m0.w) * s0.w);
            if (RES) {
                if (RES == 2) rv = make_float4((rv.x - m1.x) * s1.x, (rv.y - m1.y) * s1.y, (rv.z - m1.z) * s1.z, (rv.w - m1.w) * s1.w);
                v.x += rv.x; v.y += rv.y; v.z += rv.z; v.w += rv.w;
            }
            v.x = v.x >= 0.f ? v.x : v.x * slope;
            v.y = v.y >= 0.f ? v.y : v.y * slope;
            v.z = v.z >= 0.f ? v.z : v.z * slope;
            v.w = v.w >= 0.f ? v.w : v.w * slope;
            *reinterpret_cast<float4*>(y + r * ldy + 4 * q) = v;
        };
        long r = r_lo + (int)(threadIdx.x / cb);
        for (; r + 3 * rp < r_hi; r += 4 * rp) {
            float4 xv[4], rv[4];
#pragma unroll
            for (int u = 0; u < 4; ++u) {
                xv[u] = *reinterpret_cast<const float4*>(x + (r + u * rp) * ldx + 4 * q);
                rv[u] = RES ? *reinterpret_cast<const float4*>(res + (r + u * rp) * ldr + 4 * q) : make_float4(0.f, 0.f, 0.f, 0.f);
            }
#pragma unroll
            for (int u = 0; u < 4; ++u) finish(xv[u], rv[u], r + u * rp);
        }
        for (; r < r_hi; r += rp) {
            const float4 xv = *reinterpret_cast<const float4*>(x + r * ldx + 4 * q);
            const float4 rv = RES ? *reinterpret_cast<const float4*>(res + r * ldr + 4 * q) : make_float4(0.f, 0.f, 0.f, 0.f);
            finish(xv, rv, r);
        }
    }
}

__global__ void __launch_bounds__(256) k_instnorm_apply4_pack(const float* __restrict__ x, int n, int c4, int ldx,
                                                               const float* __restrict__ stats, float slope,
                                                               float* __restrict__ y, int ldy,
                                                               const float* __restrict__ s_pts, float4* __restrict__ pk) {
    const long e = (long)blockIdx.x * blockDim.x + threadIdx.x;
    if (e >= (long)n * c4) return;
    const long r = e / c4;
    const int q = (int)(e - r * c4);
    const float4 xv = *reinterpret_cast<const float4*>(x + r * ldx + 4 * q);
    const float4 s0 = *reinterpret_cast<const float4*>(stats + 8 * q), s1 = *reinterpret_cast<const float4*>(stats + 8 * q + 4);
    float4 v = make_float4((xv.x - s0.x) * s0.y, (xv.y - s0.z) * s0.w, (xv.z - s1.x) * s1.y, (xv.w - s1.z) * s1.w);
    v.x = v.x >= 0.f ? v.x : v.x * slope;
    v.y = v.y >= 0.f ? v.y : v.y * slope;
    v.z = v.z >= 0.f ? v.z : v.z * slope;
    v.w = v.w >= 0.f ? v.w : v.w * slope;
    *reinterpret_cast<float4*>(y + r * ldy + 4 * q) = v;
    float part = (v.x + v.y) + (v.z + v.w);
    for (int sh = c4 >> 1; sh >= 1; sh >>= 1) part += __shfl_xor(part, sh, 64);
    if (q == 0) pk[r] = make_float4(s_pts[3 * r], s_pts[3 * r + 1], s_pts[3 * r + 2], part > 0.0f ? 1.f : 0.f);
}

__global__ void __launch_bounds__(256) k_instnorm_apply4_sums_pack(NormMulti mm, int c4, int ldx, float eps, float slope, int ldy,
                                                                    int rows_per_block) {
    const int g = blockIdx.y;
    const float* __restrict__ x = mm.x[g];
    const double* __restrict__ sums = mm.sums[g];
    float* __restrict__ y = mm.y[g];
    const float* __restrict__ s_pts = mm.s_pts[g];
    float4* __restrict__ pk = mm.pk[g];
    const int n = mm.n[g];
    const double count = mm.count[g];
    if ((long)blockIdx.x * rows_per_block >= n) return;
    const int rp = 256 / c4;
    const int r_lo = blockIdx.x * rows_per_block, r_hi = min(n, r_lo + rows_per_block);
    const int q = (int)(threadIdx.x % c4);
    float4 m0, s0;
    stats4_from_sums(sums, 4 * c4, 4 * q, count, eps, m0, s0);
    for (long r = r_lo + (int)(threadIdx.x / c4); r < r_hi; r += rp) {
        const float4 xv = *reinterpret_cast<const float4*>(x + r * ldx + 4 * q);
        float4 v = make_float4((xv.x - m0.x) * s0.x, (xv.y - m0.y) * s0.y, (xv.z - m0.z) * s0.z, (xv.w - m0.w) * s0.w);
        v.x = v.x >= 0.f ? v.x : v.x * slope;
        v.y = v.y >= 0.f ? v.y : v.y * slope;
        v.z = v.z >= 0.f ? v.z : v.z * slope;
        v.w = v.w >= 0.f ? v.w : v.w * slope;
        *reinterpret_cast<float4*>(y + r * ldy + 4 * q) = v;
        float part = (v.x + v.y) + (v.z + v.w);
        for (int sh = c4 >> 1; sh >= 1; sh >>= 1) part += __shfl_xor(part, sh, 64);
        if (q == 0) pk[r] = make_float4(s_pts[3 * r], s_pts[3 * r + 1], s_pts[3 * r + 2], part > 0.0f ? 1.f : 0.f);
    }
}

}

bool instnorm_pack_ok(int c, int ldx, int ldy) {
    const int c4 = c / 4;
    return c % 4 == 0 && c4 >= 1 && c4 <= 64 && (c4 & (c4 - 1)) == 0 && ldx % 4 == 0 && ldy % 4 == 0;
}
int instnorm_apply_pack(const float* x, int n, int c, int ldx, const float* stats, const double* sums, double count, float eps,
                        float slope, float* y, int ldy, const float* s_pts, float4* pk, hipStream_t st) {
    PCRCG_CHECK_ARG(n >= 0 && instnorm_pack_ok(c, ldx, ldy) && ldx >= c && ldy >= c && (stats != nullptr) != (sums != nullptr));
    if (n == 0) return PCRCG_OK;
    PCRCG_CHECK_ARG(x && y && s_pts && pk && ((reinterpret_cast<uintptr_t>(x) | reinterpret_cast<uintptr_t>(y)) & 15) == 0);
    const int c4 = c / 4;
    if (stats) {
        const long total = (long)n * c4;
        hipLaunchKernelGGL(k_instnorm_apply4_pack, dim3((unsigned)((total + 255) / 256)), dim3(256), 0, st, x, n, c4, ldx, stats,
                           slope, y, ldy, s_pts, pk);
    } else {
        NormJob one{x, sums, nullptr, nullptr, y, s_pts, pk, n, count};
        return instnorm_apply_sums_multi(&one, 1, c, ldx, eps, 0, slope, ldy, true, st);
    }
    PCRCG_CHECK_LAUNCH();
    return PCRCG_OK;
}

bool instnorm_sums_ok(int c, int ldx, int ldy, int ldr) {
    const int c4 = c / 4;
    return c >= 4 && c % 4 == 0 && (c4 <= 256 ? 256 % c4 == 0 : c4 % 256 == 0) && ldx % 4 == 0 && ldy % 4 == 0 && ldr % 4 == 0;
}
int instnorm_apply_sums_multi(const NormJob* jobs, int count, int c, int ldx, float eps, int ldr, float slope, int ldy, bool pack,
                              hipStream_t st) {
    PCRCG_CHECK_ARG(jobs && count >= 1 && count <= 4 && c >= 4 && c % 4 == 0);
    const int c4 = c / 4;
    NormMulti mm;
    int nmax = 0;
    for (int g = 0; g < 4; ++g) {
        const NormJob& j = jobs[g < count ? g : 0];
        mm.x[g] = j.x; mm.sums[g] = j.sums; mm.res[g] = j.res; mm.res_sums[g] = j.res_sums; mm.y[g] = j.y;
        mm.s_pts[g] = j.s_pts; mm.pk[g] = j.pk; mm.n[g] = g < count ? j.n : 0; mm.count[g] = j.count;
        mm.stats_out[g] = g < count ? j.stats_out : nullptr;
        if (g < count) {
            PCRCG_CHECK_ARG(j.n >= 0 && j.x && j.sums && j.y && j.count >= 1.0);
            PCRCG_CHECK_ARG((j.res != nullptr) == (jobs[0].res != nullptr) && (j.res_sums != nullptr) == (jobs[0].res_sums != nullptr));
            nmax = j.n > nmax ? j.n : nmax;
        }
    }
    if (nmax == 0) return PCRCG_OK;
    const int rp = 256 / (c4 < 256 ? c4 : 256);
    int rows_per_block = rp * 8;
    while (rows_per_block > rp && (long)(nmax + rows_per_block - 1) / rows_per_block * count < 256) rows_per_block -= rp;
    const dim3 grid((unsigned)((nmax + rows_per_block - 1) / rows_per_block), count);
    if (pack)
        hipLaunchKernelGGL(k_instnorm_apply4_sums_pack, grid, dim3(256), 0, st, mm, c4, ldx, eps, slope, ldy, rows_per_block);
    else if (!jobs[0].res)
        hipLaunchKernelGGL(k_instnorm_apply4_sums<0>, grid, dim3(256), 0, st, mm, c4, ldx, eps, ldr, slope, ldy, rows_per_block);
    else if (!jobs[0].res_sums)
        hipLaunchKernelGGL(k_instnorm_apply4_sums<1>, grid, dim3(256), 0, st, mm, c4, ldx, eps, ldr, slope, ldy, rows_per_block);
    else
        hipLaunchKernelGGL(k_instnorm_apply4_sums<2>, grid, dim3(256), 0, st, mm, c4, ldx, eps, ldr, slope, ldy, rows_per_block);
    PCRCG_CHECK_LAUNCH();
    return PCRCG_OK;
}

size_t colstats_ws_bytes(int c) { return carve_bytes((size_t)kStatChunks * 2 * (size_t)(c > 0 ? c : 1), sizeof(double)); }

int colstats_finalize(const double* partial, int nchunks, int c, double count, float eps, float* stats,
                      hipStream_t st) {
    hipLaunchKernelGGL(k_colstats_final, dim3((c + 3) / 4), dim3(256), 0, st, partial, nchunks, c, count, eps, stats);
    PCRCG_CHECK_LAUNCH();
    return PCRCG_OK;
}
int colstats_chunks() { return kStatChunks; }

int gather_max_multi(const GatherJob* jobs, int count, int c, hipStream_t st) {
    PCRCG_CHECK_ARG(jobs && count >= 1 && count <= 4 && c >= 1);
    GatherMulti mm;
    bool vec = c % 4 == 0;
    int nq_max = 0;
    for (int g = 0; g < 4; ++g) {
        const GatherJob& j = jobs[g < count ? g : 0];
        mm.x[g] = j.x; mm.idx[g] = reinterpret_cast<const long long*>(j.idx); mm.out[g] = j.out;
        mm.ns[g] = j.ns; mm.nq[g] = g < count ? j.nq : 0; mm.h[g] = j.h; mm.ld_idx[g] = j.ld_idx;
        mm.walk[g] = j.walk;
        if (g < count) {
            PCRCG_CHECK_ARG((j.walk != nullptr) == (jobs[0].walk != nullptr));
            PCRCG_CHECK_ARG(j.ns >= 0 && j.nq >= 0 && j.h >= 1 && j.ld_idx >= j.h && (j.nq == 0 || (j.x && j.idx && j.out)));
            vec = vec && ((reinterpret_cast<uintptr_t>(j.x) | reinterpret_cast<uintptr_t>(j.out)) & 15) == 0;
            nq_max = j.nq > nq_max ? j.nq : nq_max;
        }
    }
    if (nq_max == 0) return PCRCG_OK;
    const int per_wave = vec ? 256 : 64;
    const int nchunk = (c + per_wave - 1) / per_wave;
    const long items = jobs[0].walk ? (long)((nq_max + 7) / 8) * nchunk : (long)nq_max * nchunk;
    const dim3 grid((unsigned)((items + kWavesPerBlock - 1) / kWavesPerBlock) * (jobs[0].walk ? 8 : 1), count);
    if (vec) hipLaunchKernelGGL(k_gather_max<true>, grid, dim3(kWavesPerBlock * 64), 0, st, mm, c, nchunk);
    else hipLaunchKernelGGL(k_gather_max<false>, grid, dim3(kWavesPerBlock * 64), 0, st, mm, c, nchunk);
    PCRCG_CHECK_LAUNCH();
    return PCRCG_OK;
}

int instnorm_colsums_multi(const float* const* x, double* const* sums, const int* n, int count, int c, int ldx, hipStream_t st) {
    PCRCG_CHECK_ARG(count >= 1 && count <= 4 && c >= 1 && ldx >= c);
    ColsMulti mm;
    int nmax = 0;
    for (int g = 0; g < 4; ++g) {
        const int k = g < count ? g : 0;
        PCRCG_CHECK_ARG(n[k] >= 1 && x[k] && sums[k]);
        mm.x[g] = x[k]; mm.partial[g] = sums[k]; mm.n[g] = n[k];
        if (g < count) nmax = n[k] > nmax ? n[k] : nmax;
    }
    int chunks = (nmax + 63) / 64;
    if (chunks > kStatChunks) chunks = kStatChunks;
    if (debug_opts().deterministic) chunks = 1;
    hipLaunchKernelGGL(k_colstats_partial<true>, dim3(chunks, (c + 63) / 64, count), dim3(256), 0, st, mm, c, ldx);
    PCRCG_CHECK_LAUNCH();
    return PCRCG_OK;
}

}

using namespace pcrcg;
// ... 88 lines not shown
```

pcrcg_amd/csrc/pyramid.hip:

```cpp
#include <time.h>

#include <cmath>
#include <cstdlib>
#include <vector>

#include "frontend.h"

namespace pcrcg {
namespace {

inline double now_us() {
    timespec ts;
    clock_gettime(CLOCK_MONOTONIC, &ts);
    return ts.tv_sec * 1e6 + ts.tv_nsec * 1e-3;
}

__global__ void k_probe_many(int* sink, int spin) {
    int x = threadIdx.x;
    for (int i = 0; i < spin; ++i) x = x * 1664525 + 1013904223;
    if (x == 0x7fffffff) sink[0] = x;
}
__global__ void k_probe_tiny(int* sink) {
    if (threadIdx.x == 1234567) sink[1] = 1;
}

int fetch(int* h_scratch, const int* src, int n, const int* src2, int n2, hipStream_t st,
          std::unique_lock<std::mutex>* enqueue = nullptr) {
    PCRCG_CHECK_HIP(hipMemcpyAsync(h_scratch + 1, src, sizeof(int) * n, hipMemcpyDeviceToHost, st));
    if (n2 > 0) PCRCG_CHECK_HIP(hipMemcpyAsync(h_scratch + 1 + n, src2, sizeof(int) * n2, hipMemcpyDeviceToHost, st));
    hipEvent_t ev;
    PCRCG_CHECK_HIP(hipEventCreateWithFlags(&ev, hipEventDisableTiming));
    hipError_t e = hipEventRecord(ev, st);
    if (enqueue && enqueue->owns_lock()) enqueue->unlock();
    if (e == hipSuccess) e = hipEventSynchronize(ev);
    (void)hipEventDestroy(ev);
    PCRCG_CHECK_HIP(e);
    return PCRCG_OK;
}

struct Arena {
    char* base;
    size_t cap, off = 0, peak = 0;
    bool dry;
    Arena(void* p, size_t bytes, bool dry_) : base(static_cast<char*>(p)), cap(bytes), dry(dry_) {}
    void* raw(size_t bytes) {
        bytes = (bytes + 255) & ~size_t(255);
        void* p = base ? base + off : nullptr;
        off += bytes;
        if (off > peak) peak = off;
        return p;
    }
    template <typename T>
    T* take(size_t count) { return static_cast<T*>(raw((count ? count : 1) * sizeof(T))); }
    bool ok() const { return dry || off <= cap; }
};

struct TableRec {
    RadiusSearch s;
    int kind;
    int level, q_level, sup_level;
};

struct MetaView {
    int* w; int P, L;
    struct Table {
        int* w; int P;
        int& max_count(int p) const { return w[p]; }
        int& status() const { return w[P]; }
        int& tie_rows() const { return w[P + 1]; }
        int widest() const { int m = 0; for (int p = 0; p < P; ++p) m = w[p] > m ? w[p] : m; return m; }
    };
    Table table(int i) const { return Table{w + (P + 2) * i, P}; }
    int* row_counts() const { return w + (P + 2) * 3 * L; }
    int& overflow() const { return row_counts()[L]; }
    int words() const { return (P + 2) * 3 * L + L + 1; }
    const int* lengths() const { return w + words(); }
};
}
}

using namespace pcrcg;

struct EventBox {
    std::vector<hipEvent_t> ev;
    int make(hipEvent_t* e) {
        PCRCG_CHECK_HIP(hipEventCreateWithFlags(e, hipEventDisableTiming));
        ev.push_back(*e);
        return PCRCG_OK;
    }
    ~EventBox() { for (hipEvent_t e : ev) (void)hipEventDestroy(e); }
};

struct Parts {
    const float* const* pts;
    const int* n;
    const int* const* len;
    const int* nb;
    int count;
};

static void level_caps(int n0, const pcrcg_pyramid_cfg* cfg, int* cap) {
    double shrink = cfg->shrink;
    if (!(shrink > 0.0) || shrink > 1.0) shrink = 1.0;
    cap[0] = n0;
    for (int l = 1; l < cfg->n_levels; ++l) {
        const double c = ceil((double)cap[l - 1] * shrink);
        cap[l] = c < 1.0 ? 1 : (c > (double)cap[l - 1] ? cap[l - 1] : (int)c);
    }
}

struct EnqueueLocks {
    std::mutex mu;
    hipStream_t key[16];
    std::mutex lock[16];
    int n = 0;
    std::mutex* of(hipStream_t st) {
        std::lock_guard<std::mutex> g(mu);
        for (int i = 0; i < n; ++i)
            if (key[i] == st) return &lock[i];
        if (n == 16) return &lock[15];
        key[n] = st;
        return &lock[n++];
    }
};
static EnqueueLocks g_enqueue;

constexpr int kHostScratchInts = 256;
static int host_scratch_ints(int nb, const pcrcg_pyramid_cfg* cfg) {
    const int L = cfg->n_levels, P = cfg->group > 0 ? nb / cfg->group : 1;
    return 1 + MetaView{nullptr, P, L}.words() + L * nb;
}


struct Build {
    int nb, group;
    bool want_ties, one_forest;
    int cap[PCRCG_MAX_LEVELS];
    float* level_pts[PCRCG_MAX_LEVELS];
    int* lens_all;
    float* feats;
    MetaView meta;
    int* tie_status;
    std::vector<TableRec> tables;
    void* forest[2] = {nullptr, nullptr};
    int forest_ns[2] = {0, 0}, forest_nb[2] = {0, 0};
    EventBox events;
    hipEvent_t forests_done = nullptr;
};

static int pyramid_enqueue(const Parts& in, int n0, int nb, const pcrcg_pyramid_cfg* cfg, Arena& A, hipStream_t st, Build& B) {
    const int L = cfg->n_levels;
    const bool dry = A.dry, want_ties = B.want_ties = cfg->tie_order != 0;
    const int group = B.group = cfg->group > 0 ? cfg->group : 0;
    B.nb = nb;
    int* const cap = B.cap;
    float** const level_pts = B.level_pts;
    level_caps(n0, cfg, cap);
    {
        size_t rows = 0;
        for (int l = 0; l < L; ++l) rows += (size_t)cap[l] + 1;
        float* pts_all = A.take<float>(3 * rows);
        rows = 0;
        for (int l = 0; l < L; ++l) { level_pts[l] = pts_all + 3 * rows; rows += (size_t)cap[l] + 1; }
    }
    int* const lens_all = B.lens_all = A.take<int>((size_t)L * nb);
    float* const feats = B.feats = A.take<float>((size_t)n0);
    MetaView& meta = B.meta = MetaView{nullptr, group > 0 ? nb / group : 1, L};
    const size_t meta_ints = (size_t)meta.words() + 1;
    meta.w = A.take<int>(meta_ints);
    B.tie_status = &meta.overflow() + 1;
    if (!A.ok()) return PCRCG_EWORKSPACE;

    std::vector<TableRec>& tables = B.tables;
    tables.reserve(3 * L);
    if (!dry) {
        PCRCG_CHECK_HIP(hipMemsetAsync(meta.w, 0, sizeof(int) * meta_ints, st));
        size_t row = 0, cloud = 0;
        for (int i = 0; i < in.count; ++i) {
            if (in.n[i] > 0)
                PCRCG_CHECK_HIP(hipMemcpyAsync(level_pts[0] + 3 * row, in.pts[i], sizeof(float) * 3 * (size_t)in.n[i], hipMemcpyDeviceToDevice, st));
            PCRCG_CHECK_HIP(hipMemcpyAsync(lens_all + cloud, in.len[i], sizeof(int) * in.nb[i], hipMemcpyDeviceToDevice, st));
            row += (size_t)in.n[i];
            cloud += (size_t)in.nb[i];
        }
        PCRCG_CHECK_HIP(hipMemsetD32Async(reinterpret_cast<hipDeviceptr_t>(feats), 0x3f800000, (size_t)(n0 > 0 ? n0 : 1), st));
    }

    hipStream_t sub_st = cfg->side_stream ? as_stream(cfg->side_stream) : st;
    hipStream_t f_st = cfg->side_stream2 ? as_stream(cfg->side_stream2) : sub_st;
    auto order = [&](hipStream_t a, hipStream_t b) -> int {
        if (a == b || dry) return PCRCG_OK;
        hipEvent_t ev;
        PCRCG_PROPAGATE(B.events.make(&ev));
        PCRCG_CHECK_HIP(hipEventRecord(ev, a));
        PCRCG_CHECK_HIP(hipStreamWaitEvent(b, ev, 0));
        return PCRCG_OK;
    };
    const bool one_forest = B.one_forest = !want_ties || f_st == st || L < 2;
    int level_base[PCRCG_MAX_LEVELS] = {};
    auto build_forest = [&](int which) -> int {
        if (!want_ties || (which == 1 && L < 2)) return PCRCG_OK;
        const int first = which == 1 ? 1 : 0, last = which == 0 ? 0 : L - 1, slot = which == 1 ? 1 : 0;
        for (int l = first; l <= last; ++l) level_base[l - first] = (int)((level_pts[l] - level_pts[first]) / 3);
        B.forest_ns[slot] = level_base[last - first] + cap[last];
        B.forest_nb[slot] = (last - first + 1) * nb;
        const size_t bytes = pcrcg_kdforest_ws_bytes(B.forest_ns[slot], B.forest_nb[slot]);
        B.forest[slot] = A.raw(bytes);
        if (!A.ok()) return PCRCG_EWORKSPACE;
        if (dry) return PCRCG_OK;
        PCRCG_PROPAGATE(order(which == 0 ? st : sub_st, f_st));
        return kdforest_build_levels(level_pts[first], B.forest_ns[slot], lens_all + (size_t)first * nb, B.forest_nb[slot],
                                     last > first ? nb : 0, level_base, B.forest[slot], bytes, f_st);
    };

    auto add_table = [&](int kind, int level, int q_level, const void* grid, const void* qgrid, float radius, const float* q,
                         const int* qlen, int nq, int ns, const int* slen, int limit, int sup_level) -> int {
        const MetaView::Table m = meta.table((int)tables.size());
        TableRec t;
        t.kind = kind; t.level = level; t.q_level = q_level; t.sup_level = sup_level;
        RadiusSearch& s = t.s;
        s.q = q; s.nq = nq; s.qlen = qlen; s.qgrid = qgrid; s.sgrid = grid; s.ns = ns; s.slen = slen;
        s.nb = nb; s.group = group; s.radius = radius; s.cols = limit;
        s.idx = A.take<int64_t>((size_t)nq * limit);
        s.count = want_ties ? A.take<int>((size_t)nq) : nullptr;
        s.tie_rows = want_ties ? A.take<int>((size_t)nq) : nullptr;
        s.max_count = &m.max_count(0); s.status = &m.status(); s.tie_count = want_ties ? &m.tie_rows() : nullptr;
        if (!A.ok()) return PCRCG_EWORKSPACE;
        if (!dry) PCRCG_PROPAGATE(radius_search(s, RadiusPass::first, st));
        tables.push_back(t);
        return PCRCG_OK;
    };
    auto build_grid = [&](const float* sup, int ns, const int* slen, float radius, void** grid) -> int {
        const size_t gb = pcrcg_cellgrid_ws_bytes(ns, nb);
        *grid = A.raw(gb);
        if (!A.ok()) return PCRCG_EWORKSPACE;
        if (!dry) PCRCG_PROPAGATE(pcrcg_cellgrid_build(sup, ns, slen, nb, radius, *grid, gb, st));
        return PCRCG_OK;
    };

    const size_t sub_wsb = L > 1 ? pcrcg_grid_subsample_ws_bytes(cap[0], nb) : 0;
    void* sub_ws = L > 1 ? A.raw(sub_wsb) : nullptr;
    if (!A.ok()) return PCRCG_EWORKSPACE;

    void* carried = nullptr;
    float carried_r = 0.f;
    PCRCG_PROPAGATE(order(st, sub_st));
    if (!one_forest || L == 1) PCRCG_PROPAGATE(build_forest(0));
    for (int l = 0; l < L; ++l) {
        const int limit = cfg->limit[l];
        const float r_conv = cfg->r_conv[l], r_pool = cfg->r_pool[l];
        float* pts = level_pts[l];
        int* lens = lens_all + (size_t)l * nb;
        const int n = cap[l];
        void* grid = nullptr;
        float grid_r = 0.f;
        const bool pooled = cfg->pooled[l] && l + 1 < L;
        if (!pooled && l + 1 < L) {
            set_error("pcrcg_pyramid_build: level %d of %d is not pooled", l, L);
            return PCRCG_EBADARG;
        }
        if (pooled && !dry)
            PCRCG_PROPAGATE(grid_subsample_bound(pts, n, lens, nb, cfg->dl[l], 0, level_pts[l + 1], lens + nb, meta.row_counts() + l,
                                                 cap[l + 1], &meta.overflow(), sub_ws, sub_wsb, sub_st));
        if (pooled && l + 2 == L) PCRCG_PROPAGATE(build_forest(one_forest ? 2 : 1));
        if (cfg->has_conv[l]) {
            if (carried && carried_r == r_conv) { grid = carried; grid_r = carried_r; }
            else { PCRCG_PROPAGATE(build_grid(pts, n, lens, r_conv, &grid)); grid_r = r_conv; }
            PCRCG_PROPAGATE(add_table(0, l, l, grid, grid, r_conv, pts, lens, n, n, lens, limit, l));
        }
        carried = nullptr;
        if (pooled) {
            float* sub = level_pts[l + 1];
            int* sub_len = lens + nb;
            const int m = cap[l + 1];
            if (grid == nullptr || grid_r != r_pool) {
                PCRCG_PROPAGATE(build_grid(pts, n, lens, r_pool, &grid));
                grid_r = r_pool;
            }
            PCRCG_PROPAGATE(order(sub_st, st));
            void* up_grid = nullptr;
            PCRCG_PROPAGATE(build_grid(sub, m, sub_len, 2 * r_pool, &up_grid));
            PCRCG_PROPAGATE(add_table(1, l, l + 1, grid, up_grid, r_pool, sub, sub_len, m, n, lens, limit, l));
            PCRCG_PROPAGATE(add_table(2, l, l, up_grid, grid, 2 * r_pool, pts, lens, n, m, sub_len, cfg->up_nearest ? 1 : limit, l + 1));
            carried = up_grid;
            carried_r = 2 * r_pool;
        }
    }
    if (!dry && want_ties && f_st != st) {
        PCRCG_PROPAGATE(B.events.make(&B.forests_done));
        PCRCG_CHECK_HIP(hipEventRecord(B.forests_done, f_st));
    }
    return PCRCG_OK;
}

static int pyramid_finish(const Build& B, const pcrcg_pyramid_cfg* cfg, int* h_scratch, pcrcg_batch* out, int* h_lengths,
                          int* h_status, pcrcg_pyramid_restore* deferred, hipStream_t st) {
    const int L = B.meta.L, P = B.meta.P, nb = B.nb, group = B.group, nt = (int)B.tables.size();
    if (B.forests_done) PCRCG_CHECK_HIP(hipStreamWaitEvent(st, B.forests_done, 0));
    const MetaView hm{h_scratch + 1, P, L};
    if (hm.overflow() != 0) {
        set_error("pcrcg_pyramid_build: a level keeps more rows than pcrcg_pyramid_cfg::shrink = %.3f allows -- call again with a "
                  "larger bound (1.0 always fits)", cfg->shrink);
        return PCRCG_EWORKSPACE;
    }
    for (int i = 0; i < L * nb; ++i) h_lengths[i] = hm.lengths()[i];
    int level_n[PCRCG_MAX_LEVELS];
    for (int l = 0; l < L; ++l) {
        level_n[l] = 0;
        for (int c = 0; c < nb; ++c) level_n[l] += h_lengths[(size_t)l * nb + c];
    }
    {
        int redone = 0;
        for (int i = 0; i < nt; ++i) {
            const bool handed_over = (hm.table(i).status() & kRadiusRedoStatus) != 0;
            if (hm.table(i).widest() <= radius_fast_cap() && !handed_over) continue;
            PCRCG_PROPAGATE(radius_search(B.tables[i].s, RadiusPass::redo, st));
            ++redone;
        }
        if (redone) PCRCG_PROPAGATE(fetch(h_scratch, B.meta.w, hm.words(), B.lens_all, L * nb, st));
    }
    auto group_rows = [&](int l, int p, int* row0, int* rows) {
        const int c0 = group > 0 ? p * group : 0, c1 = group > 0 ? c0 + group : nb;
        int a = 0, r = 0;
        for (int c = 0; c < c1; ++c) (c < c0 ? a : r) += h_lengths[(size_t)l * nb + c];
        *row0 = a;
        *rows = r;
    };
    for (int p = 0; p < P; ++p) {
        pcrcg_batch& o = out[p];
        o.n_levels = L;
        int row0, rows;
        group_rows(0, p, &row0, &rows);
        o.features = B.feats + row0;
        o.feat_dim = 1;
        o.len_src_c = h_lengths[(size_t)(L - 1) * nb + (group > 0 ? p * group : 0)];
        for (int l = 0; l < L; ++l) {
            group_rows(l, p, &row0, &rows);
            o.points[l] = B.level_pts[l] + 3 * (size_t)row0;
            o.n_points[l] = rows;
            o.stack_lengths[l] = B.lens_all + (size_t)l * nb + (group > 0 ? p * group : 0);
            o.neighbors[l] = pcrcg_table{nullptr, rows, 0, 1};
            o.pools[l] = pcrcg_table{nullptr, 0, 0, 1};
            o.upsamples[l] = pcrcg_table{nullptr, 0, 0, 1};
        }
    }
    pcrcg_pyramid_restore local;
    pcrcg_pyramid_restore& R = deferred ? *deferred : local;
    R.njobs = 0;
    for (int i = 0; i < nt; ++i) {
        const TableRec& t = B.tables[i];
        const RadiusSearch& s = t.s;
        const MetaView::Table m = hm.table(i);
        if (m.status() != 0) {
            set_error("pcrcg_pyramid_build: radius search capacity exceeded (table %d)", i);
            return PCRCG_ECAPACITY;
        }
        for (int p = 0; p < P; ++p) {
            const int max_count = m.max_count(p);
            const int cols = max_count < s.cols ? (max_count > 0 ? max_count : 0) : s.cols;
            int row0, rows;
            group_rows(t.q_level, p, &row0, &rows);
            pcrcg_table tab{s.idx + (size_t)row0 * s.cols, rows, cols, s.cols};
            if (t.kind == 0) out[p].neighbors[t.level] = tab;
            else if (t.kind == 1) out[p].pools[t.level] = tab;
            else out[p].upsamples[t.level] = tab;
        }
        const int widest = m.widest(), tie_rows = m.tie_rows();
        if (B.want_ties && widest > 0 && tie_rows > 0 && R.njobs < PCRCG_MAX_REORDER_JOBS) {
            pcrcg_reorder_job& j = R.jobs[R.njobs++];
            const int fi = (B.one_forest || t.sup_level == 0) ? 0 : 1;
            j.q = s.q; j.qlen = s.qlen; j.rows = s.tie_rows; j.count = s.count; j.idx = s.idx;
            j.nq = level_n[t.q_level]; j.nbq = nb; j.cloud0 = B.one_forest ? t.sup_level * nb : (fi == 0 ? 0 : (t.sup_level - 1) * nb);
            j.nrows = tie_rows;
            j.max_count = widest < 8192 ? widest : 8192;
            j.cols = s.cols; j.radius = s.radius; j.group = group;
            j.sup = B.level_pts[fi]; j.forest = B.forest[fi]; j.forest_ns = B.forest_ns[fi]; j.forest_nb = B.forest_nb[fi];
        }
    }
    R.tie_status = B.tie_status;
    if (!deferred) return pcrcg_pyramid_restore_run(&R, h_status, st);
    return PCRCG_OK;
}

extern "C" {

size_t pcrcg_pyramid_ws_bytes(int n0, int nb, const pcrcg_pyramid_cfg* cfg) {
    if (!cfg || n0 < 0 || nb < 1 || cfg->n_levels < 1 || cfg->n_levels > PCRCG_MAX_LEVELS) return 0;
    Arena A(nullptr, 0, true);
    Build B;
    if (pyramid_enqueue(Parts{}, n0, nb, cfg, A, nullptr, B) != PCRCG_OK) return 0;
    return A.peak + 4096;
}

int pcrcg_stream_create(void** stream, int priority) {
    PCRCG_CHECK_ARG(stream != nullptr);
    hipStream_t st = nullptr;
    PCRCG_CHECK_HIP(hipStreamCreateWithPriority(&st, hipStreamNonBlocking, priority));
    *stream = st;
    return PCRCG_OK;
}

int pcrcg_stream_pipe_classes(void* const* streams, int n, int* cls, void* scratch) {
    PCRCG_CHECK_ARG(streams && cls && scratch && n >= 1 && n <= 64);
    int* sink = static_cast<int*>(scratch);
    PCRCG_CHECK_HIP(hipDeviceSynchronize());
    for (int i = 0; i < n; ++i) hipLaunchKernelGGL(k_probe_tiny, dim3(1), dim3(64), 0, as_stream(streams[i]), sink);
    PCRCG_CHECK_HIP(hipDeviceSynchronize());
    const int blocks = 2000000;
    double t0 = now_us();
    hipLaunchKernelGGL(k_probe_many, dim3(blocks), dim3(64), 0, as_stream(streams[0]), sink, 64);
    PCRCG_CHECK_HIP(hipStreamSynchronize(as_stream(streams[0])));
    const double big_us = now_us() - t0;
    if (big_us < 400.0) {
        set_error("pcrcg_stream_pipe_classes: the dispatch-bound probe kernel took only %.0f us", big_us);
        return PCRCG_ELAUNCH;
    }
    int reps[8], nrep = 0;
    auto shares = [&](int a, int b, bool* out) -> int {
        int yes = 0, no = 0;
        for (int trial = 0; trial < 10 && yes < 2 && no < 2; ++trial) {
            const double launch = now_us();
            hipLaunchKernelGGL(k_probe_many, dim3(blocks), dim3(64), 0, as_stream(streams[a]), sink, 64);
            const double start = now_us();
            while (now_us() - start < 150.0) {}
            const double a0 = now_us();
            hipLaunchKernelGGL(k_probe_tiny, dim3(1), dim3(64), 0, as_stream(streams[b]), sink);
            const double a1 = now_us();
            PCRCG_CHECK_HIP(hipStreamSynchronize(as_stream(streams[b])));
            const double d = now_us() - a0;
            PCRCG_CHECK_HIP(hipDeviceSynchronize());
            if (a1 - launch > 0.6 * big_us) continue;
            (d > (big_us - 150.0) / 3.0 ? yes : no) += 1;
        }
        if (yes < 2 && no < 2) { set_error("pcrcg_stream_pipe_classes: the host is too busy for the probe's timing"); return PCRCG_ELAUNCH; }
        *out = yes == 2;
        return PCRCG_OK;
    };
    for (int i = 0; i < n; ++i) {
        cls[i] = -1;
        for (int j = 0; j < i && cls[i] < 0; ++j)
            if (streams[j] == streams[i]) cls[i] = cls[j];
        for (int r = 0; r < nrep && cls[i] < 0; ++r) {
            bool same = false;
            PCRCG_PROPAGATE(shares(reps[r], i, &same));
            if (same) cls[i] = r;
        }
        if (cls[i] < 0) {
            if (nrep == 8) { set_error("pcrcg_stream_pipe_classes: more than 8 dispatcher classes -- the probe is not measuring what it should"); return PCRCG_ELAUNCH; }
            reps[nrep] = i;
            cls[i] = nrep++;
        }
    }
    return PCRCG_OK;
}

int pcrcg_stream_destroy(void* stream) {
    PCRCG_CHECK_HIP(hipStreamDestroy(as_stream(stream)));
    return PCRCG_OK;
}
// ... 58 lines not shown
```

pcrcg_amd/csrc/runner.hip:

```cpp
#include <vector>

#include <cstdlib>

#include "gemm.h"

namespace pcrcg {
namespace {

constexpr int GMAX = 4;
static_assert(GMAX <= 4, "instnorm_apply_sums_multi, instnorm_colsums_multi, gather_max_multi, copy2d_multi, heads_multi, "
                         "edgeconv_rows_multi and attention_mfma_multi (common.h) take up to four clouds");

struct Mat {
    float* p[GMAX] = {};
    int rows[GMAX] = {};
    int cols = 0, ld = 0;
    bool zeroed = false;
};

struct Ctx {
    char* base = nullptr;
    size_t cap = 0, off = 0, peak = 0;
    hipStream_t st = nullptr;
    bool dry = false;
// ... 240 lines not shown
    }
    return grp;
}

void linear(Ctx& c, const Mat& x, const float* w, int ldw, const float* bias, const Mat& y, bool c_zeroed, Stat* st = nullptr,
            const float* const* row_scale = nullptr, const Fold* f = nullptr) {
    if (!c.live()) return;
    bool same_ld = true;
    for (int g = 1; g < c.G && f && f->tabs; ++g) same_ld = same_ld && f->tabs[g]->ld == f->tabs[0]->ld;
    const bool grouped = c.paired() && same_ld;
    for (int g = 0; g < (grouped ? 1 : c.G); ++g) {
        GemmCall call;
        call.a = x.p[g]; call.lda = x.ld;
        call.b = w; call.ldb = ldw;
        call.c = y.p[g]; call.ldc = y.ld;
        call.m = (f && f->tabs) ? f->tabs[g]->rows : x.rows[g]; call.n = y.cols; call.k = x.cols;
        call.row_scale = row_scale ? row_scale[g] : nullptr;
        call.bias = bias;
        call.st = c.st;
        stats_into(call, st, g);
        call.c_zeroed = c_zeroed;
        const GemmExtra ex = f ? extra_of(*f, x, g) : GemmExtra();
        const GemmGroup grp = grouped ? group_of(c, x, y, c_zeroed, st, row_scale, f) : GemmGroup();
        if (f) call.ex = &ex;
        if (grouped) call.grp = &grp;
        c.check(gemm_run(call));
    }
}
void linear(Ctx& c, const Mat& x, const float* w, int ldw, const float* bias, const Mat& y, Stat* st = nullptr,
            const float* const* row_scale = nullptr) {
    linear(c, x, w, ldw, bias, y, y.zeroed, st, row_scale);
}

bool lazy_stats_ready(Ctx& c, const Mat& x, Stat* xs) {
    if (!xs || !xs->sums || x.ld % 4 != 0 || x.cols > 4096) return false;
    fill_sums(c, x, xs);
    return true;
}
bool linear_norm(Ctx& c, const Mat& x, Stat* xs, float slope, const float* w, int ldw, const float* bias, const Mat& y,
                 Stat* st = nullptr) {
    if (!gemm_split_terms_on() || !lazy_stats_ready(c, x, xs)) return false;
    Fold f;
    f.sums = xs;
    f.slope = slope;
    linear(c, x, w, ldw, bias, y, y.zeroed, st, nullptr, &f);
    return true;
}

struct Batches { const pcrcg_batch* b[GMAX]; };

struct Walks {
    int* w[PCRCG_MAX_LEVELS][GMAX] = {};
    bool built[PCRCG_MAX_LEVELS] = {};
    int mode = 0;
};

static bool walk_pays(int mode, int ns, int cin, int nq) {
    if (mode != 1) return mode == 2;
    return (size_t)ns * (size_t)cin * sizeof(float) > (size_t)8 << 20 && nq >= 2048;
}

const int* const* level_walks(Ctx& c, const Batches& B, Walks& W, int l) {
    if (c.live() && !W.built[l]) {
        const float* pts[GMAX];
        int n[GMAX];
        for (int g = 0; g < c.G; ++g) { pts[g] = B.b[g]->points[l]; n[g] = B.b[g]->n_points[l]; }
        c.check(query_walk_multi(pts, n, W.w[l], nullptr, c.G, c.st));
        W.built[l] = true;
    }
    return W.w[l];
}

int kp_cin(const pcrcg_block& blk, const Mat& x) { return (blk.kp_w_pad && blk.cin_pad > x.cols) ? blk.cin_pad : x.cols; }
const float* kp_weight(const pcrcg_block& blk, const Mat& x) {
    return (blk.kp_w_pad && blk.cin_pad > 0 && kp_cin(blk, x) == blk.cin_pad) ? blk.kp_w_pad : blk.kp_w;
}

int kp_k(const pcrcg_block& blk, const Mat& x) {
    const int cin = kp_cin(blk, x);
    return (cin == 1 && blk.kp_wt) ? 16 : PCRCG_KPOINTS * cin;
}

void kpconv(Ctx& c, const Batches& B, Walks& W, const pcrcg_block& blk, const Mat& x, const Mat& y, Stat* st = nullptr,
            void* const* packed_ws = nullptr) {
    const int l = blk.layer;
    const size_t m = c.mark();
    Mat xin = x;
    const float* const w = kp_weight(blk, x);
    const int cin = kp_cin(blk, x);
    if (cin > x.cols) {
        xin = c.mat(x.rows, cin);
        if (c.live())
            for (int g = 0; g < c.G; ++g) {
                c.check(hipMemsetAsync(xin.p[g], 0, sizeof(float) * (size_t)x.rows[g] * cin, c.st) == hipSuccess ? PCRCG_OK
                                                                                                                   : PCRCG_ELAUNCH);
                c.check(pcrcg_copy2d(x.p[g], x.ld, xin.p[g], cin, x.rows[g], x.cols, c.st));
            }
    }
    int nq[GMAX], ns[GMAX];
    const float* q[GMAX];
    const pcrcg_table* tab[GMAX];
    float* inv_n[GMAX];
    void* ws[GMAX];
    size_t wsb[GMAX];
    for (int g = 0; g < c.G; ++g) {
        const pcrcg_batch& b = *B.b[g];
        tab[g] = blk.strided ? &b.pools[l] : &b.neighbors[l];
        q[g] = blk.strided ? b.points[l + 1] : b.points[l];
        nq[g] = blk.strided ? b.n_points[l + 1] : b.n_points[l];
        ns[g] = b.n_points[l];
        inv_n[g] = static_cast<float*>(c.raw(sizeof(float) * (nq[g] > 0 ? nq[g] : 1)));
        wsb[g] = pcrcg_kpconv_ws_bytes(ns[g]);
        ws[g] = (packed_ws && packed_ws[g]) ? packed_ws[g] : c.raw(wsb[g]);
    }
    const float* const kp_wt = blk.kp_wt;
    const int kk = kp_k(blk, x);
    const int* const* walks = (cin > 1 && walk_pays(W.mode, c.max_rows(ns), cin, c.max_rows(nq))) ? level_walks(c, B, W, blk.strided ? l + 1 : l) : nullptr;
    if (c.bf16 && kp_wt && cin % 32 == 0) {
        for (int g = 0; g < c.G; ++g) {
            const pcrcg_batch& b = *B.b[g];
            void* xb = c.raw(sizeof(unsigned short) * (size_t)(ns[g] > 0 ? ns[g] : 1) * cin);
            void* wfb = c.raw(sizeof(unsigned short) * (size_t)(nq[g] > 0 ? nq[g] : 1) * kk);
            if (c.live()) {
                c.check(kpconv_aggregate_bf16(q[g], nq[g], b.points[l], ns[g], tab[g]->idx, tab[g]->cols, tab[g]->ld, xin.p[g],
                                              static_cast<unsigned short*>(xb), cin, blk.kp, blk.extent, static_cast<unsigned short*>(wfb),
                                              inv_n[g], ws[g], wsb[g], c.st, walks ? walks[g] : nullptr));
                GemmCall call;
                call.a = wfb; call.lda = kk; call.a_form = GemmA::row_bf16;
                call.b = kp_wt; call.ldb = kk;
                call.c = y.p[g]; call.ldc = y.ld;
                call.m = nq[g]; call.n = y.cols; call.k = kk;
                call.row_scale = inv_n[g];
                call.c_zeroed = y.zeroed;
                call.st = c.st;
                stats_into(call, st, g);
                c.check(gemm_run(call));
            }
        }
        c.release(m);
        return;
    }
    Mat wf = c.mat(nq, kk);
    if (c.live()) {
        for (int g = 0; g < c.G; ++g) {
            const bool packed = kk != 16 && packed_ws && packed_ws[g] && xin.p[g] == x.p[g];
            c.check(kpconv_aggregate_rows(q[g], nq[g], B.b[g]->points[l], ns[g], tab[g]->idx, tab[g]->cols, tab[g]->ld, xin.p[g], cin,
                                          blk.kp, blk.extent, wf.p[g], inv_n[g], ws[g], wsb[g], c.st, !packed,
                                          true, kk == 16 ? 16 : 0, walks ? walks[g] : nullptr));
        }
        if (kp_wt)
            linear(c, wf, kp_wt, kk, nullptr, y, st, inv_n);
        else
            for (int g = 0; g < c.G; ++g)
                c.check(pcrcg_gemm_f32_colstats(wf.p[g], wf.ld, w, y.cols, 0, y.p[g], y.ld, nq[g], y.cols, kk, inv_n[g], nullptr,
                                                (st && !st->sums) ? st->partials[g] : nullptr, (st && !st->sums) ? st->bytes : 0,
                                                (st && !st->sums) ? &st->chunks[g] : nullptr, c.st));
    }
    c.release(m);
}

void out_rows(const Ctx& c, const Batches& B, const pcrcg_block& blk, int* rows) {
    for (int g = 0; g < GMAX; ++g)
        rows[g] = g < c.G ? (blk.strided ? B.b[g]->n_points[blk.layer + 1] : B.b[g]->n_points[blk.layer]) : 0;
}

Mat simple_block(Ctx& c, const Batches& B, Walks& W, const pcrcg_block& blk, const Mat& x) {
    int nq[GMAX];
    out_rows(c, B, blk, nq);
    Mat y = c.mat(nq, blk.mid_dim);
    const size_t m = c.mark();
    Mat t = c.gemm_out(nq, y.cols, kp_k(blk, x));
    Stat ts = stat_buffer(c, nq, t.cols);
    kpconv(c, B, W, blk, x, t, &ts);
    norm_act(c, t, 0.1f, y, &ts);
    c.release(m);
    return y;
}

bool norm_act_pack(Ctx& c, const Batches& B, int layer, const Mat& t, float slope, const Mat& u, Stat* ts, void* const* kp_ws,
                   const size_t* kp_ws_bytes) {
    if (c.bf16 || !instnorm_pack_ok(t.cols, t.ld, u.ld) || u.ld != u.cols) return false;
    const size_t m = c.mark();
    float* stats = static_cast<float*>(c.raw(sizeof(float) * 2 * t.cols));
    const size_t wsb = pcrcg_instnorm_ws_bytes(t.cols);
    void* ws = c.raw(wsb);
    fill_sums(c, t, ts);
    if (c.live() && all_sums(c, ts)) {
        NormJobs nj = norm_jobs(c, t, ts->partials, u);
        bool ok = nj.aligned;
        for (int g = 0; g < c.G; ++g) {
            nj.j[g].s_pts = B.b[g]->points[layer];
            nj.j[g].pk = kpconv_pk_ptr(kp_ws[g], kp_ws_bytes[g], t.rows[g]);
            ok = ok && nj.j[g].pk != nullptr;
        }
        if (ok) {
            c.check(instnorm_apply_sums_multi(nj.j, c.G, t.cols, t.ld, 1e-5f, 0, slope, u.ld, true, c.st));
            c.release(m);
            return true;
        }
    }
    if (c.live())
        for (int g = 0; g < c.G; ++g) {
            const float* s_pts = B.b[g]->points[layer];
            float4* pk = kpconv_pk_ptr(kp_ws[g], kp_ws_bytes[g], t.rows[g]);
            if (!pk) c.check(PCRCG_EWORKSPACE);
            else if (ts && ts->has_sums(g))
                c.check(instnorm_apply_pack(t.p[g], t.rows[g], t.cols, t.ld, nullptr, static_cast<const double*>(ts->partials[g]),
                                            (double)t.rows[g], 1e-5f, slope, u.p[g], u.ld, s_pts, pk, c.st));
            else {
                col_stats(c, t, g, ts, stats, ws, wsb);
                c.check(instnorm_apply_pack(t.p[g], t.rows[g], t.cols, t.ld, stats, nullptr, 0.0, 1e-5f, slope, u.p[g], u.ld, s_pts,
                                            pk, c.st));
            }
        }
    c.release(m);
    return true;
}

Mat resnet_block(Ctx& c, const Batches& B, Walks& W, const pcrcg_block& blk, const Mat& feats) {
    int nq[GMAX];
    out_rows(c, B, blk, nq);
    Mat y = c.mat(nq, blk.out_dim);
    const size_t m = c.mark();
    Mat x = feats;
    void* kp_ws[GMAX] = {};
    size_t kp_wsb[GMAX] = {};
    bool packed = false;
    if (blk.unary1) {
        Mat t = c.gemm_out(feats.rows, blk.mid_dim, feats.cols), u = c.mat(feats.rows, blk.mid_dim);
        Stat ts = stat_buffer(c, t.rows, t.cols);
        linear(c, feats, blk.unary1, feats.cols, nullptr, t, &ts);
        if (blk.mid_dim % 4 == 0 && !(blk.kp_w_pad && blk.cin_pad > blk.mid_dim)) {
            for (int g = 0; g < c.G; ++g) {
                kp_wsb[g] = pcrcg_kpconv_ws_bytes(feats.rows[g]);
                kp_ws[g] = c.raw(kp_wsb[g]);
            }
            packed = norm_act_pack(c, B, blk.layer, t, 0.1f, u, &ts, kp_ws, kp_wsb);
        }
        if (!packed) norm_act(c, t, 0.1f, u, &ts);
        x = u;
    }
    Mat k = c.gemm_out(nq, blk.mid_dim, PCRCG_KPOINTS * kp_cin(blk, x)), kn = c.mat(nq, blk.mid_dim);
    Stat ks = stat_buffer(c, nq, blk.mid_dim);
    kpconv(c, B, W, blk, x, k, &ks, packed ? kp_ws : nullptr);
    Mat u2 = c.gemm_out(nq, blk.out_dim, blk.mid_dim);
    Stat u2s = stat_buffer(c, nq, blk.out_dim);
    if (!linear_norm(c, k, &ks, 0.1f, blk.unary2, blk.mid_dim, nullptr, u2, &u2s)) {
        norm_act(c, k, 0.1f, kn, &ks);
        linear(c, kn, blk.unary2, blk.mid_dim, nullptr, u2, &u2s);
    }
    Mat sc = feats;
    if (blk.strided) {
        sc = c.mat(nq, feats.cols);
        if (c.live()) {
            GatherJob jobs[GMAX];
            const int* const* walks = walk_pays(W.mode, c.max_rows(feats.rows), feats.cols, c.max_rows(nq)) ? level_walks(c, B, W, blk.layer + 1) : nullptr;
            for (int g = 0; g < c.G; ++g) {
                const pcrcg_table& t = B.b[g]->pools[blk.layer];
                jobs[g] = GatherJob{feats.p[g], t.idx, sc.p[g], feats.rows[g], nq[g], t.cols, t.ld, walks ? walks[g] : nullptr};
            }
            c.check(gather_max_multi(jobs, c.G, feats.cols, c.st));
        }
    }
    if (blk.shortcut) {
        Mat s2 = c.gemm_out(nq, blk.out_dim, sc.cols);
        Stat s2s = stat_buffer(c, nq, blk.out_dim);
        linear(c, sc, blk.shortcut, sc.cols, nullptr, s2, &s2s);
        norm_act(c, u2, 0.1f, y, &u2s, &s2, true, &s2s);
    } else {
        norm_act(c, u2, 0.1f, y, &u2s, &sc, false);
    }
    c.release(m);
    return y;
}

void edge_norm(Ctx& c, const float* cn, int ld_cn, int cw, const int* idx, int n, int k, float* emax, int ld_emax, float* out,
               int ld_out, void* sums, bool sums_ok, float* stats, void* ws, size_t wsb) {
    if (sums && sums_ok) {
        c.check(pcrcg_edgeconv_reduce_sums(cn, ld_cn, cn + cw, ld_cn, idx, n, k, cw, emax, ld_emax, sums, c.st));
        c.check(pcrcg_instnorm_apply_sums(emax, n, cw, ld_emax, sums, (double)n * (double)k, 1e-5f, nullptr, 0, nullptr, 0.2f, out,
                                          ld_out, c.st));
        return;
    }
    c.check(pcrcg_edgeconv_reduce(cn, ld_cn, cn + cw, ld_cn, idx, n, k, cw, 1e-5f, emax, ld_emax, stats, ws, wsb, c.st));
    c.check(pcrcg_instnorm_apply(emax, n, cw, ld_emax, stats, nullptr, 0, nullptr, 0.2f, out, ld_out, c.st));
}

void edge_norm_all(Ctx& c, const Mat& cn, int cw, int* const* idx, const int* n, const int* k, const Mat& e, const Mat& out,
                   void* const* sums, bool sums_ok, float* stats, void* ws, size_t wsb) {
    bool multi = sums_ok;
    EdgeCloud cl[GMAX];
    for (int g = 0; g < c.G; ++g) {
        multi = multi && sums[g] != nullptr;
        cl[g] = EdgeCloud{cn.p[g], cn.p[g] + cw, idx[g], e.p[g], static_cast<double*>(sums[g]), n[g], k[g]};
    }
    if (multi && edgeconv_rows_ok(cl, c.G, cn.ld, cn.ld, e.ld, cw)) {
        c.check(edgeconv_rows_multi(cl, c.G, cn.ld, cn.ld, e.ld, cw, true, nullptr, c.st));
        NormJobs nj = norm_jobs(c, e, sums, out);
        bool one = nj.aligned;
        for (int g = 0; g < c.G; ++g) {
            nj.j[g].count = (double)n[g] * (double)k[g];
            one = one && n[g] > 0 && k[g] > 0;
        }
        apply_sums(c, nj.j, one, cw, e.ld, 0, 0.2f, out.ld);
        return;
    }
    for (int g = 0; g < c.G; ++g)
        edge_norm(c, cn.p[g], cn.ld, cw, idx[g], n[g], k[g], e.p[g], e.ld, out.p[g], out.ld, sums[g], sums_ok, stats, ws, wsb);
}

Mat self_attention(Ctx& c, const pcrcg_model& mdl, const pcrcg_gnn_layer& gl, const float* const* coords, const Mat& f,
                   int* const* knn_given = nullptr) {
    const int ch = f.cols;
    Mat y = c.mat(f.rows, ch);
    const size_t m = c.mark();
    int kq[GMAX];
    int* idx[GMAX];
    for (int g = 0; g < c.G; ++g) {
        const int n = f.rows[g];
        kq[g] = mdl.knn_k < n - 1 ? mdl.knn_k : n - 1;
        idx[g] = knn_given ? knn_given[g] : static_cast<int*>(c.raw(sizeof(int) * (size_t)n * (kq[g] > 0 ? kq[g] : 1)));
    }
    Mat cat = c.mat(f.rows, 4 * ch);
    const size_t wsb = pcrcg_edgeconv_ws_bytes(2 * ch);
    void* ws = c.raw(wsb);
    float* stats = static_cast<float*>(c.raw(sizeof(float) * 4 * ch));
    Mat cn1 = c.gemm_out(f.rows, 2 * ch, ch), e1 = c.mat(f.rows, ch), cn2 = c.gemm_out(f.rows, 4 * ch, ch), e2 = c.mat(f.rows, 2 * ch);
// ... 362 lines not shown
```

pcrcg_amd/csrc/tieorder.hip:

```cpp
#include <cfloat>
#include <cstdlib>

#include "block_scan.h"
#include "frontend.h"

namespace pcrcg {
namespace {

typedef unsigned long long u64;

constexpr int kLeafMax = 10;
constexpr int kSubMax = 1024;
constexpr int kSubLevelNodes = 96;
constexpr int kSubThreads = 512;
constexpr int kBigThreads = 512;
constexpr int kBigVec = 4;
constexpr int kOwnMax = 4096;
constexpr int kForestBlocks = 48;
constexpr int kSpinLimitDefault = 1 << 18;
constexpr int kTravStack = 128;
constexpr int kReorderWaves = 4;
constexpr int kMaxRow = 8192;

constexpr int kStUnfinished = 1;
constexpr int kStStack = 2;
constexpr int kStCount = 3;
constexpr int kStWidth = 4;

struct alignas(64) KdNode {
    int left, right;
    int divfeat;
    float divlow, divhigh;
    int child1, child2;
    int is_root;
    float lo[3], hi[3];
    int pad[2];
};

struct KdCtl {
    int node_count, status;
    int q_head, q_tail;
    int pending;
    int pad[3];
};

struct KdView {
    KdCtl* ctl;
    int* soff;
    KdNode* nodes;
    int* vind;
    int* scratch;
    int* taskq;
    int qcap;
};

inline size_t forest_bytes(int ns, int nb) {
    const size_t N = (size_t)(ns > 0 ? ns : 0);
    return carve_bytes(1, sizeof(KdCtl)) + carve_bytes((size_t)nb + 1, sizeof(int)) +
           carve_bytes(2 * N + nb + 2, sizeof(KdNode)) + 2 * carve_bytes(N + 1, sizeof(int)) +
           carve_bytes(2 * N + nb + 2, sizeof(int));
}

inline KdView forest_view(void* ws, size_t bytes, int ns, int nb, bool* ok) {
    const size_t N = (size_t)(ns > 0 ? ns : 0);
    Carver cv(ws, bytes);
    KdView v;
    v.ctl = reinterpret_cast<KdCtl*>(cv.take<char>(sizeof(KdCtl)));
    v.soff = cv.take<int>((size_t)nb + 1);
    v.nodes = cv.take<KdNode>(2 * N + nb + 2);
    v.vind = cv.take<int>(N + 1);
    v.scratch = cv.take<int>(N + 1);
    v.qcap = (int)(2 * N + nb + 2);
    v.taskq = cv.take<int>((size_t)v.qcap);
    *ok = cv.ok();
    return v;
}

struct KdBases {
    int per_level;
    int base[PCRCG_MAX_LEVELS];
};
__global__ void __launch_bounds__(256) k_kd_init(const int* __restrict__ slen, int ns, int nb, KdView v, KdBases bases) {
    if (blockIdx.x == 0 && threadIdx.x == 0) {
        KdCtl* c = v.ctl;
        c->node_count = nb;
        c->status = 0;
// ... 622 lines not shown
        if (vy > rt->hi[1]) { d1 = (vy - rt->hi[1]) * (vy - rt->hi[1]); distsq += d1; }
        if (vz < rt->lo[2]) { d2 = (vz - rt->lo[2]) * (vz - rt->lo[2]); distsq += d2; }
        if (vz > rt->hi[2]) { d2 = (vz - rt->hi[2]) * (vz - rt->hi[2]); distsq += d2; }
        int sp = 1;
        st_node[0] = root;
        st_min[0] = distsq;
        st_d[0] = d0; st_d[1] = d1; st_d[2] = d2;
        while (sp > 0) {
            --sp;
            __builtin_amdgcn_wave_barrier();
            int node = uni(st_node[sp]);
            const float mind = unif(st_min[sp]);
            d0 = unif(st_d[3 * sp]); d1 = unif(st_d[3 * sp + 1]); d2 = unif(st_d[3 * sp + 2]);
            for (;;) {
                const i32x8 nh = node_head(&v.nodes[node]);
                const int feat = nh[2];
                if (feat < 0) {
                    const int l = nh[0], r = nh[1];
                    for (int base = l; base < r; base += 64) {
                        const int i = base + lane;
                        bool hit = false;
                        float result = 0.0f;
                        int g = 0;
                        if (i < r) {
                            g = v.vind[i];
                            const float e0 = vx - sup[3 * (long)g], e1 = vy - sup[3 * (long)g + 1], e2 = vz - sup[3 * (long)g + 2];
                            result += e0 * e0;
                            result += e1 * e1;
                            result += e2 * e2;
                            hit = result < r2;
                        }
                        const u64 mask = __ballot(hit);
                        const int pos = n + __popcll(mask & below);
                        if (hit && pos < W) mine[pos] = ((u64)__float_as_uint(result) << 32) | (unsigned)g;
                        n += __popcll(mask);
                    }
                    break;
                }
                const float val = feat == 0 ? vx : (feat == 1 ? vy : vz);
                const float divlow = __int_as_float(nh[3]), divhigh = __int_as_float(nh[4]);
                const int child1 = nh[5], child2 = nh[6];
                const float diff1 = val - divlow, diff2 = val - divhigh;
                int best, other;
                float cut_dist;
                if ((diff1 + diff2) < 0) { best = child1; other = child2; cut_dist = (val - divhigh) * (val - divhigh); }
                else { best = child2; other = child1; cut_dist = (val - divlow) * (val - divlow); }
                const float dcur = feat == 0 ? d0 : (feat == 1 ? d1 : d2);
                const float mind2 = mind + cut_dist - dcur;
                if (mind2 * 1.0f <= r2) {
                    if (sp < kTravStack) {
                        st_node[sp] = other;
                        st_min[sp] = mind2;
                        st_d[3 * sp] = feat == 0 ? cut_dist : d0;
                        st_d[3 * sp + 1] = feat == 1 ? cut_dist : d1;
                        st_d[3 * sp + 2] = feat == 2 ? cut_dist : d2;
                        ++sp;
                    } else {
                        err = kStStack;
                    }
                }
                node = best;
            }
        }
    }
    if (n > W && !err) err = kStWidth;
    if (jb.count && n != jb.count[qi] && !err) err = kStCount;
    if (err) {
        if (status && lane == 0) *status = err;
        return;
    }
    __builtin_amdgcn_fence(__ATOMIC_SEQ_CST, "wavefront");
    __builtin_amdgcn_wave_barrier();
    if (lane == 0 && n > 16) std_sort_partition_phase(mine, n);
    __builtin_amdgcn_fence(__ATOMIC_SEQ_CST, "wavefront");
    __builtin_amdgcn_wave_barrier();
    stable_sort_wave(mine, sorted, n, lane);
    __builtin_amdgcn_fence(__ATOMIC_SEQ_CST, "wavefront");
    __builtin_amdgcn_wave_barrier();
    long long* row = reinterpret_cast<long long*>(jb.idx) + (long)qi * jb.cols;
    for (int j = lane; j < jb.cols; j += 64)
        row[j] = j < n ? (long long)((int)(unsigned)(sorted[j] & 0xFFFFFFFFull) - seg) : (long long)pad;
}

}
}

using namespace pcrcg;

extern "C" {

size_t pcrcg_kdforest_ws_bytes(int ns, int nb) { return forest_bytes(ns, nb < 1 ? 1 : nb); }

int pcrcg_kdforest_build(const float* sup, int ns, const int* slen, int nb, void* forest, size_t forest_bytes_,
                         void* stream) {
    return pcrcg::kdforest_build_levels(sup, ns, slen, nb, 0, nullptr, forest, forest_bytes_, as_stream(stream));
}
}

int pcrcg::kdforest_build_levels(const float* sup, int ns, const int* slen, int nb, int per_level, const int* level_base,
                                 void* forest, size_t forest_bytes_, hipStream_t stream) {
    PCRCG_CHECK_ARG(ns >= 0 && nb >= 1 && slen && forest);
    PCRCG_CHECK_ARG(per_level == 0 || (per_level > 0 && nb % per_level == 0 && nb / per_level <= PCRCG_MAX_LEVELS && level_base));
    KdBases bases;
    bases.per_level = per_level;
    for (int l = 0; l < PCRCG_MAX_LEVELS; ++l) bases.base[l] = per_level > 0 && l < nb / per_level ? level_base[l] : 0;
    PCRCG_CHECK_ARG(ns == 0 || sup);
    hipStream_t st = stream;
    bool ok;
    KdView v = forest_view(forest, forest_bytes_, ns, nb, &ok);
    if (!ok) {
        set_error("pcrcg_kdforest_build: workspace too small (%zu needed, %zu given)", forest_bytes(ns, nb), forest_bytes_);
        return PCRCG_EWORKSPACE;
    }
    int init_blocks = (v.qcap + 255) / 256;
    init_blocks = init_blocks < 1 ? 1 : (init_blocks > 1024 ? 1024 : init_blocks);
    hipLaunchKernelGGL(k_kd_init, dim3(init_blocks), dim3(256), 0, st, slen, ns, nb, v, bases);
    if (ns > 0) {
        int blocks = ns / (2 * kSubMax) + nb;
        if (blocks > kForestBlocks) blocks = kForestBlocks;
        if (debug_opts().kd_blocks > 0) blocks = debug_opts().kd_blocks;
        const int spin = debug_opts().kd_spin_limit;
        hipLaunchKernelGGL(k_kd_forest, dim3(blocks), dim3(kBigThreads), 0, st, sup, v, spin > 0 ? spin : kSpinLimitDefault);
    }
    PCRCG_CHECK_LAUNCH();
    return PCRCG_OK;
}

extern "C" {

int pcrcg_radius_reorder_jobs(const pcrcg_reorder_job* jobs, int njobs, const float* sup, int ns, int nb,
                              const void* forest, int* status, void* stream) {
    PCRCG_CHECK_ARG(njobs >= 0 && njobs <= PCRCG_MAX_REORDER_JOBS && (njobs == 0 || jobs) && nb >= 1 && ns >= 0);
    ReorderJobs pack;
    int total = 0, width = 1;
    pack.njobs = 0;
    for (int i = 0; i < njobs; ++i) {
        const pcrcg_reorder_job& j = jobs[i];
        const bool own = j.forest != nullptr;
        const int fnb = own ? j.forest_nb : nb, fns = own ? j.forest_ns : ns;
        PCRCG_CHECK_ARG(own || forest);
        PCRCG_CHECK_ARG(j.nq >= 0 && j.nbq >= 1 && j.cloud0 >= 0 && j.cloud0 + j.nbq <= fnb && fns >= 0 && j.qlen && j.idx);
        PCRCG_CHECK_ARG(j.cols >= 1 && j.max_count >= 0 && j.max_count <= kMaxRow && j.radius > 0.0f);
        const int nrows = j.rows ? j.nrows : j.nq;
        PCRCG_CHECK_ARG(nrows >= 0 && nrows <= j.nq && (j.nq == 0 || (j.q && (own ? j.sup : sup))));
        if (nrows == 0) continue;
        bool vok;
        pack.job[pack.njobs] = j;
        pack.view[pack.njobs] = forest_view(const_cast<void*>(own ? j.forest : forest), forest_bytes(fns, fnb), fns, fnb, &vok);
        pack.sup[pack.njobs] = own ? j.sup : sup;
        pack.row_begin[pack.njobs] = total;
        ++pack.njobs;
        total += nrows;
        if (j.max_count > width) width = j.max_count;
    }
    pack.row_begin[pack.njobs] = total;
    if (total == 0) return PCRCG_OK;
    hipStream_t st = as_stream(stream);
    const size_t second = (size_t)width > (size_t)kTravStack * 5 / 2 ? (size_t)width : (size_t)kTravStack * 5 / 2;
    const size_t per_wave = (size_t)width + second + 1;
    const int waves = width > 2000 ? 1 : (width > 512 ? 2 : kReorderWaves);
    const size_t lds = per_wave * waves * sizeof(u64);
    if (lds > 64 * 1024) PCRCG_GRANT_LDS(k_reorder);
    hipLaunchKernelGGL(k_reorder, dim3((total + waves - 1) / waves), dim3(waves * 64), lds, st, pack, width, status);
    PCRCG_CHECK_LAUNCH();
    return PCRCG_OK;
}

int pcrcg_radius_reorder(const float* q, int nq, const int* qlen, int nbq, const float* sup, int ns, int nb,
                         const void* forest, int cloud0, float radius, const int* rows, int nrows, const int* count,
                         int max_count, int cols, int64_t* idx, int* status, void* stream) {
    pcrcg_reorder_job j;
    j.q = q;
    j.qlen = qlen;
    j.rows = rows;
    j.count = count;
    j.idx = idx;
    j.nq = nq;
    j.nbq = nbq;
    j.cloud0 = cloud0;
    j.nrows = nrows;
    j.max_count = max_count;
    j.cols = cols;
    j.radius = radius;
    j.group = 0;
    j.sup = nullptr;
    j.forest = nullptr;
    j.forest_ns = j.forest_nb = 0;
    return pcrcg_radius_reorder_jobs(&j, 1, sup, ns, nb, forest, status, stream);
}
}
```

pcrcg_amd/csrc/walk.hip:

```cpp
#include <cfloat>

#include "block_scan.h"
#include "common.h"

namespace pcrcg {
namespace {

constexpr int kWalkThreads = 1024;
constexpr int kWalkBins = 4096;

struct WalkMulti { const float* pts[4]; int* walk[4]; int* key[4]; int n[4]; };

__device__ __forceinline__ bool finite_f(float v) { return fabsf(v) <= FLT_MAX; }

__device__ __forceinline__ int walk_cell(float p, float lo, float scale) {
    const float v = finite_f(p) ? (p - lo) * scale : 0.f;
    return !(v >= 0.f) ? 0 : (v < 15.f ? (int)v : 15);
}
__device__ __forceinline__ int spread3(int c) { return (c & 1) | ((c & 2) << 2) | ((c & 4) << 4) | ((c & 8) << 6); }

__device__ __forceinline__ int walk_key(const float* p, const float* lo, const float* scale) {
    return spread3(walk_cell(p[0], lo[0], scale[0])) | (spread3(walk_cell(p[1], lo[1], scale[1])) << 1) |
           (spread3(walk_cell(p[2], lo[2], scale[2])) << 2);
}
// ... 48 lines not shown
        float l = FLT_MAX, h = -FLT_MAX;
        for (int w = 0; w < kWalkThreads / 64; ++w) { l = fminf(l, s_red[w][tid]); h = fmaxf(h, s_red[w][3 + tid]); }
        s_lo[tid] = l;
        s_scale[tid] = 16.0f / fmaxf(h - l, 1e-30f);
    }
    __syncthreads();

    for (int i0 = tid; i0 < n; i0 += kWalkBatch * kWalkThreads) {
        walk_fetch(pts, i0, n, v);
#pragma unroll
        for (int u = 0; u < kWalkBatch; ++u) {
            const int i = i0 + u * kWalkThreads;
            if (i < n) {
                const int k = walk_key(v[u], s_lo, s_scale);
                atomicAdd(&s_bin[k], 1);
                if (key_out) key_out[i] = k;
            }
        }
    }
    __syncthreads();

    int c[4], sum = 0;
#pragma unroll
    for (int b = 0; b < 4; ++b) { c[b] = s_bin[4 * tid + b]; sum += c[b]; }
    int total;
    int off = block_excl_scan_i32<kWalkThreads>(sum, &total, s_scan);
#pragma unroll
    for (int b = 0; b < 4; ++b) { s_bin[4 * tid + b] = off; off += c[b]; }
    __syncthreads();

    for (int i0 = tid; i0 < n; i0 += kWalkBatch * kWalkThreads) {
        walk_fetch(pts, i0, n, v);
#pragma unroll
        for (int u = 0; u < kWalkBatch; ++u) {
            const int i = i0 + u * kWalkThreads;
            if (i < n) {
                walk[atomicAdd(&s_bin[walk_key(v[u], s_lo, s_scale)], 1)] = i;
            }
        }
    }
}

}

int query_walk_multi(const float* const* pts, const int* n, int* const* walk, int* const* key, int count, hipStream_t st) {
    PCRCG_CHECK_ARG(pts && n && walk && count >= 1 && count <= 4);
    WalkMulti mm;
    int nmax = 0;
    for (int g = 0; g < 4; ++g) {
        const bool on = g < count;
        if (on) PCRCG_CHECK_ARG(n[g] >= 0 && (n[g] == 0 || (pts[g] && walk[g])));
        mm.pts[g] = on ? pts[g] : nullptr;
        mm.walk[g] = on ? walk[g] : nullptr;
        mm.key[g] = (on && key) ? key[g] : nullptr;
        mm.n[g] = on ? n[g] : 0;
        if (on && n[g] > nmax) nmax = n[g];
    }
    if (nmax == 0) return PCRCG_OK;
    hipLaunchKernelGGL(k_query_walk, dim3(count), dim3(kWalkThreads), 0, st, mm);
    PCRCG_CHECK_LAUNCH();
    return PCRCG_OK;
}

}

using namespace pcrcg;

extern "C" {

int pcrcg_query_walk(const float* points, int n, int* walk, int* key, void* stream) {
    PCRCG_CHECK_ARG(n >= 0);
    if (n == 0) return PCRCG_OK;
    PCRCG_CHECK_ARG(points && walk);
    return query_walk_multi(&points, &n, &walk, key ? &key : nullptr, 1, as_stream(stream));
}

int pcrcg_kpconv_aggregate_walk(const float* q_pts, int nq, const float* s_pts, int ns, const int64_t* idx, int h, int ld_idx,
                                const float* x, int cin, const float* kp, float extent, float* wf, float* inv_n, void* ws,
                                size_t ws_bytes, const int* walk, void* stream) {
    return kpconv_aggregate_rows(q_pts, nq, s_pts, ns, idx, h, ld_idx, x, cin, kp, extent, wf, inv_n, ws, ws_bytes,
                                 as_stream(stream), true, true, 0, walk);
}

int pcrcg_kpconv_aggregate_bf16_walk(const float* q_pts, int nq, const float* s_pts, int ns, const int64_t* idx, int h,
                                     int ld_idx, const float* x, int cin, const float* kp, float extent, void* x_bf16,
                                     void* wf_bf16, float* inv_n, void* ws, size_t ws_bytes, const int* walk, void* stream) {
    return kpconv_aggregate_bf16(q_pts, nq, s_pts, ns, idx, h, ld_idx, x, static_cast<unsigned short*>(x_bf16), cin, kp,
                                 extent, static_cast<unsigned short*>(wf_bf16), inv_n, ws, ws_bytes, as_stream(stream), walk);
}

int pcrcg_gather_max_walk(const float* x, int ns, int c, const int64_t* idx, int nq, int h, int ld_idx, float* out,
                          const int* walk, void* stream) {
    PCRCG_CHECK_ARG(ns >= 0 && c >= 1 && nq >= 0 && h >= 1 && ld_idx >= h);
    if (nq == 0) return PCRCG_OK;
    PCRCG_CHECK_ARG(x && idx && out);
    const GatherJob one{x, idx, out, ns, nq, h, ld_idx, walk};
    return gather_max_multi(&one, 1, c, as_stream(stream));
}
}
```

pcrcg_amd/ops.py:

```python
import ctypes

import torch

from . import _lib

_F32, _I32, _I64 = torch.float32, torch.int32, torch.int64


def _stream():
    return torch.cuda.current_stream().cuda_stream


def _dev(t, dtype, name):
    if not isinstance(t, torch.Tensor) or not t.is_cuda:
        raise RuntimeError(f"pcrcg_amd: `{name}` must be a tensor on a HIP device (no CPU fallback exists)")
    if t.dtype != dtype:
        raise RuntimeError(f"pcrcg_amd: `{name}` must have dtype {dtype}, got {t.dtype}")
    return t


def _rows(t, dtype, name):
    _dev(t, dtype, name)
    if t.dim() != 2:
        raise RuntimeError(f"pcrcg_amd: `{name}` must be 2-D")
# ... 93 lines not shown
        self.ns, self.nb = self.supports.shape[0], self.lengths.shape[0]
        self.nbytes = L.pcrcg_cellgrid_ws_bytes(self.ns, self.nb)
        self.grid = torch.empty(self.nbytes, dtype=torch.uint8, device=self.supports.device)
        _lib.check(L.pcrcg_cellgrid_build(self.supports.data_ptr(), self.ns, self.lengths.data_ptr(), self.nb,
                                          self.radius, self.grid.data_ptr(), self.nbytes, _stream()),
                   "pcrcg_cellgrid_build")

    def query(self, queries, q_lengths, cols, want_counts=False, want_ties=False, query_grid=None):
        L = _lib.lib()
        queries = _dev(queries, _F32, "queries").contiguous()
        q_lengths = _dev(q_lengths, _I32, "q_batches").contiguous()
        if q_lengths.shape[0] != self.nb:
            raise RuntimeError("Wrong number of batch elements: different for queries and supports ")
        nq = queries.shape[0]
        idx = torch.empty((nq, int(cols)), dtype=_I64, device=queries.device)
        meta = torch.zeros(3, dtype=_I32, device=queries.device)
        counts = torch.empty(nq, dtype=_I32, device=queries.device) if (want_counts or want_ties) else None
        ties = torch.empty(max(nq, 1), dtype=_I32, device=queries.device) if want_ties else None
        if query_grid is not None:
            if query_grid.ns != nq or query_grid.nb != self.nb:
                raise RuntimeError("query_grid was not built over these queries")
            cur = torch.cuda.current_stream(queries.device)
            last = getattr(query_grid, "_walk", None)
            if last is not None and last[0] != cur.cuda_stream:
                cur.wait_event(last[1])
            _lib.check(L.pcrcg_radius_query_cells(query_grid.grid.data_ptr(), queries.data_ptr(), nq, q_lengths.data_ptr(),
                                                  self.grid.data_ptr(), self.ns, self.lengths.data_ptr(), self.nb, 0,
                                                  self.radius, int(cols), idx.data_ptr(), _ptr(counts), meta[0:1].data_ptr(),
                                                  meta[1:2].data_ptr(), _ptr(ties),
                                                  meta[2:3].data_ptr() if want_ties else None, _stream()),
                       "pcrcg_radius_query_cells")
            ev = torch.cuda.Event()
            ev.record(cur)
            query_grid._walk = (cur.cuda_stream, ev)
        else:
            _lib.check(L.pcrcg_radius_query_ex(queries.data_ptr(), nq, q_lengths.data_ptr(), self.ns,
                                               self.lengths.data_ptr(), self.nb, self.radius, self.grid.data_ptr(),
                                               int(cols), idx.data_ptr(), _ptr(counts), meta[0:1].data_ptr(),
                                               meta[1:2].data_ptr(), _ptr(ties), meta[2:3].data_ptr() if want_ties else None,
                                               _stream()), "pcrcg_radius_query_ex")
        out = (idx, meta)
        if want_counts or want_ties:
            out += (counts,)
        if want_ties:
            out += (ties,)
        return out


def stream_pipe_classes(streams):
    L = _lib.lib()
    n = len(streams)
    ptrs = (ctypes.c_void_p * n)(*[s.cuda_stream for s in streams])
    cls = (ctypes.c_int * n)()
    scratch = torch.zeros(16, dtype=torch.int32, device=streams[0].device)
    torch.cuda.synchronize(streams[0].device)
    with torch.cuda.device(streams[0].device):
        _lib.check(L.pcrcg_stream_pipe_classes(ptrs, n, cls, scratch.data_ptr()), "pcrcg_stream_pipe_classes")
    return [int(c) for c in cls]


def streams_on_other_dispatchers(n=2, reference=None, candidates=12):
    ref = reference if reference is not None else torch.cuda.current_stream()
    cands = [torch.cuda.Stream(device=ref.device) for _ in range(candidates)]
    cls = stream_pipe_classes([ref] + cands)
    out, seen = [], {cls[0]}
    for s, c in zip(cands, cls[1:]):
        if c not in seen:
            out.append(s)
            seen.add(c)
        if len(out) == n:
            return out
    raise RuntimeError("pcrcg_amd.ops.streams_on_other_dispatchers: only %d dispatcher classes beside the reference stream's "
                       "among %d candidates" % (len(out), candidates))


MAX_REORDER_JOBS = 12


class ReorderJob(ctypes.Structure):
    _fields_ = [("q", ctypes.c_void_p), ("qlen", ctypes.c_void_p), ("rows", ctypes.c_void_p), ("count", ctypes.c_void_p),
                ("idx", ctypes.c_void_p), ("nq", ctypes.c_int), ("nbq", ctypes.c_int), ("cloud0", ctypes.c_int),
                ("nrows", ctypes.c_int), ("max_count", ctypes.c_int), ("cols", ctypes.c_int), ("radius", ctypes.c_float),
                ("group", ctypes.c_int), ("sup", ctypes.c_void_p), ("forest", ctypes.c_void_p), ("forest_ns", ctypes.c_int),
                ("forest_nb", ctypes.c_int)]


class KdForest:

    def __init__(self, supports, lengths):
        L = _lib.lib()
        self.supports = _dev(supports, _F32, "supports").contiguous()
        self.lengths = _dev(lengths, _I32, "s_batches").contiguous()
        self.ns, self.nb = self.supports.shape[0], self.lengths.shape[0]
        self.nbytes = L.pcrcg_kdforest_ws_bytes(self.ns, self.nb)
        self.ws = torch.empty(self.nbytes, dtype=torch.uint8, device=self.supports.device)
        _lib.check(L.pcrcg_kdforest_build(self.supports.data_ptr(), self.ns, self.lengths.data_ptr(), self.nb,
                                          self.ws.data_ptr(), self.nbytes, _stream()), "pcrcg_kdforest_build")

    def reorder(self, idx, queries, q_lengths, cloud0, radius, max_count, rows=None, nrows=None, counts=None,
                status=None):
        return self.reorder_tables([dict(idx=idx, q=queries, qlen=q_lengths, cloud0=cloud0, radius=radius,
                                         max_count=max_count, rows=rows, nrows=nrows, counts=counts)], status)

    def reorder_tables(self, tables, status=None):
        L = _lib.lib()
        if len(tables) > MAX_REORDER_JOBS:
            for i in range(0, len(tables), MAX_REORDER_JOBS):
                status = self.reorder_tables(tables[i:i + MAX_REORDER_JOBS], status)
            return status
        jobs = (ReorderJob * max(len(tables), 1))()
        keep = []
        for j, t in zip(jobs, tables):
            idx = _dev(t["idx"], _I64, "idx")
            if not idx.is_contiguous():
                raise RuntimeError("pcrcg_amd.KdForest.reorder: idx must be contiguous")
            q = _dev(t["q"], _F32, "queries").contiguous()
            qlen = _dev(t["qlen"], _I32, "q_batches").contiguous()
            keep += [q, qlen]
            rows, counts = t.get("rows"), t.get("counts")
            j.q, j.qlen, j.rows, j.count, j.idx = q.data_ptr(), qlen.data_ptr(), _ptr(rows), _ptr(counts), idx.data_ptr()
            j.nq, j.nbq, j.cloud0 = idx.shape[0], qlen.shape[0], int(t["cloud0"])
            j.nrows = idx.shape[0] if rows is None else int(t["nrows"])
            j.max_count, j.cols, j.radius = int(t["max_count"]), idx.shape[1], float(t["radius"])
            j.group = int(t.get("group", 0))
            if status is None:
                status = torch.zeros(1, dtype=_I32, device=idx.device)
        if status is None:
            return None
        _lib.check(L.pcrcg_radius_reorder_jobs(ctypes.cast(jobs, ctypes.c_void_p), len(tables), self.supports.data_ptr(),
                                               self.ns, self.nb, self.ws.data_ptr(), status.data_ptr(), _stream()),
                   "pcrcg_radius_reorder_jobs")
        return status


def _operand_b(b):
    _dev(b, _F32, "b")
    if b.dim() != 2:
        raise RuntimeError("pcrcg_amd: `b` must be 2-D")
    k, n = b.shape
    if b.stride(1) == 1 and (k == 1 or b.stride(0) >= n):
        return b, (b.stride(0) if k > 1 else n), 0
    if b.stride(0) == 1 and (n == 1 or b.stride(1) >= k):
        return b, (b.stride(1) if n > 1 else k), 1
    b = b.contiguous()
    return b, n, 0


def _operand_a(a):
    _dev(a, _F32, "a")
    if a.dim() != 2:
        raise RuntimeError("pcrcg_amd: `a` must be 2-D")
    m, k = a.shape
    if a.stride(1) == 1 and (m == 1 or a.stride(0) >= k):
        return a, (a.stride(0) if m > 1 else k), 0
    if a.stride(0) == 1 and (k == 1 or a.stride(1) >= m):
        return a, (a.stride(1) if k > 1 else m), 1
    return a.contiguous(), k, 0


def gemm(a, b, row_scale=None, bias=None, out=None, grad_operand=0):
    L = _lib.lib()
    a, lda, trans_a = _operand_a(a)
    b, ldb, trans_b = _operand_b(b)
    m, k = a.shape
    k2, n = b.shape
    if k != k2:
        raise RuntimeError(f"pcrcg_amd.gemm: inner dimensions differ ({k} vs {k2})")
# ... 394 lines not shown
```

pcrcg_amd/pyramid.py:

```python
import ctypes
import os

import numpy as np
import torch

from . import _lib, ops
from .config import as_config
from .runner import Batch, PyramidCfg, PyramidRestore

_I32 = torch.int32


def _layer_plan(config):
    arch = config.architecture
    r_normal = config.first_subsampling_dl * config.conv_radius
    levels, layer_blocks = [], []
    for i, block in enumerate(arch):
        if "global" in block or "upsample" in block:
            break
        if not ("pool" in block or "strided" in block):
            layer_blocks.append(block)
            if i < len(arch) - 1 and "upsample" not in arch[i + 1]:
                continue
        deform_conv = any("deformable" in b for b in layer_blocks[:-1])
# ... 61 lines not shown
            counts_out.append(res[2])
        return idx

    for layer, lv in enumerate(plan):
        limit = int(neighborhood_limits[layer])
        grid = None
        if lv["has_conv"]:
            grid = carried if carried is not None and carried.radius == float(lv["r_conv"]) else \
                ops.CellGrid(pts, lens, lv["r_conv"])
            conv_i = search(grid, "neighbors", layer, pts, lens, layer, limit, keep_counts=want_counts, query_grid=grid)
        else:
            conv_i = empty_idx
        if lv["pooled"]:
            rows, pool_b, m_dev = ops.grid_subsample_launch(pts, lens, lv["dl"])
            m_host, ev = ops.host_copy(m_dev)
            yield ev
            pool_p = rows[:int(m_host[0])]
            if grid is None or grid.radius != float(lv["r_pool"]):
                grid = carried if carried is not None and carried.radius == float(lv["r_pool"]) else \
                    ops.CellGrid(pts, lens, lv["r_pool"])
            up_grid = ops.CellGrid(pool_p, pool_b, 2 * lv["r_pool"])
            pool_i = search(grid, "pools", layer, pool_p, pool_b, layer, limit, query_grid=up_grid)
            up_i = search(up_grid, "upsamples", layer, pts, lens, layer + 1, limit, query_grid=grid)
            carried = up_grid
        else:
            pool_i, up_i = empty_idx, empty_idx
            pool_p = torch.zeros((0, 3), dtype=torch.float32, device=pts.device)
            pool_b = torch.zeros((0,), dtype=torch.int64, device=pts.device)
            carried = None
        in_points.append(pts)
        in_neighbors.append(conv_i)
        in_pools.append(pool_i)
        in_ups.append(up_i)
        in_lens.append(lens)
        pts, lens = pool_p, pool_b
    out = {"points": in_points, "neighbors": in_neighbors, "pools": in_pools, "upsamples": in_ups,
           "stack_lengths": in_lens}
    nb = in_lens[0].shape[0]
    host_t, ev = ops.host_copy(torch.cat([m for m in metas] + [l.to(_I32) for l in in_lens]))
    yield ev
    host = host_t.tolist()
    meta_h = [host[3 * i:3 * i + 3] for i in range(len(metas))]
    lens_h = [host[3 * len(metas) + nb * i:3 * len(metas) + nb * (i + 1)] for i in range(len(in_lens))]
    redo = []
    for tab, (max_count, status, tie_rows) in zip(tables, meta_h):
        if status != 0:
            raise RuntimeError(f"pcrcg_amd.build_pyramid: radius search capacity exceeded ({tab['key']}[{tab['layer']}])")
        tab["max_count"] = max_count
        if max_count > 0 and (tie_order == "reference" or (tie_order == "auto" and tie_rows > 0)):
            redo.append((tab, tie_rows))
    if redo:
        for tab, _ in redo:
            tab["idx"] = out[tab["key"]][tab["layer"]]
        status = _restore_reference_order(redo, in_points, in_lens, tie_order == "reference")
        status_h, ev = ops.host_copy(status)
        yield ev
        check_tie_status(int(status_h[0]))
    for tab in tables:
        t = out[tab["key"]][tab["layer"]]
        if tab["max_count"] < t.shape[1]:
            out[tab["key"]][tab["layer"]] = t[:, :max(tab["max_count"], 0)]
    out["features"] = torch.ones((in_points[0].shape[0], 1), dtype=torch.float32, device=points.device)
    out["stack_lengths_host"] = lens_h
    if want_counts:
        out["neighbor_counts"] = counts_out
    return out


def _restore_reference_order(redo, level_points, level_lens, all_rows):
    nb = level_lens[0].shape[0]
    forest = ops.KdForest(torch.cat(level_points, 0), torch.cat([l.to(_I32) for l in level_lens], 0))
    status = torch.zeros(1, dtype=_I32, device=level_points[0].device)
    forest.reorder_tables([dict(idx=tab["idx"], q=tab["q"], qlen=tab["qlen"], cloud0=nb * tab["sup_level"],
                                radius=tab["radius"], max_count=min(tab["max_count"], 8192), counts=tab["counts"],
                                rows=None if all_rows else tab["ties"], nrows=None if all_rows else tie_rows)
                           for tab, tie_rows in redo], status)
    return status


class NativePyramid:

    STATUS_RING = 64

    def __init__(self, config, neighborhood_limits, tie_order=None, up_nearest=False):
        config = as_config(config)
        if tie_order is None:
            tie_order = os.environ.get("PCRCG_TIE_ORDER", "auto")
        if tie_order not in ("auto", "index"):
            raise ValueError("pcrcg_amd.NativePyramid: tie_order must be 'auto' or 'index'")
        plan = _layer_plan(config)
        c = PyramidCfg()
        c.n_levels = len(plan)
        for l, lv in enumerate(plan):
            c.r_conv[l], c.r_pool[l], c.dl[l] = float(lv["r_conv"]), float(lv["r_pool"]), float(lv["dl"])
            c.has_conv[l], c.pooled[l], c.limit[l] = int(lv["has_conv"]), int(lv["pooled"]), int(neighborhood_limits[l])
        c.tie_order = 0 if tie_order == "index" else 1
        c.up_nearest = int(bool(up_nearest))
        self.cfg, self.levels = c, len(plan)
        self.scratch = torch.empty(512, dtype=_I32, pin_memory=True)
        self.status = torch.zeros(self.STATUS_RING, dtype=_I32, pin_memory=True)
        self.arena, self.shrink, self.calls = None, 0.5, 0
        self.side = None

    def set_side_streams(self, sub=None, forest=None):
        self.side = (sub, forest)
        self.cfg.side_stream = sub.cuda_stream if sub is not None else None
        self.cfg.side_stream2 = forest.cuda_stream if forest is not None else None

    def restore(self, deferred, slot):
        _lib.check(_lib.lib().pcrcg_pyramid_restore_run(ctypes.byref(deferred), self.status.data_ptr() + 4 * slot,
                                                        torch.cuda.current_stream().cuda_stream),
                   "pcrcg_pyramid_restore_run")

    def build(self, points, lengths, fresh_arena=False, defer_restore=False, group=0):
        ct, L = ctypes, _lib.lib()
        if not isinstance(points, (list, tuple)):
            points, lengths = [points], [lengths]
        pts_l = [p.to(torch.float32).contiguous() for p in points]
        lens_l = [l.to(_I32).contiguous() for l in lengths]
        if not all(p.is_cuda for p in pts_l):
            raise RuntimeError("pcrcg_amd.build_pyramid: points must be on a HIP device (no CPU path)")
        k, device = len(pts_l), pts_l[0].device
        pp = (ct.c_void_p * k)(*[p.data_ptr() for p in pts_l])
        lp = (ct.c_void_p * k)(*[l.data_ptr() for l in lens_l])
        pn = (ct.c_int * k)(*[int(p.shape[0]) for p in pts_l])
        ln = (ct.c_int * k)(*[int(l.shape[0]) for l in lens_l])
        n0, nb = sum(pn), sum(ln)
        stream = torch.cuda.current_stream().cuda_stream
        if group and nb % group:
            raise RuntimeError("pcrcg_amd.NativePyramid: the number of clouds is not a multiple of `group`")
        self.cfg.group = int(group)
        nbatch = nb // group if group else 1
        h_len = (ct.c_int * (self.levels * nb))()
        deferred = PyramidRestore() if defer_restore else None
        slot = self.calls % self.STATUS_RING
        self.calls += 1
        while True:
            self.cfg.shrink = float(self.shrink)
            need = L.pcrcg_pyramid_ws_bytes(n0, nb, ct.byref(self.cfg))
            if need == 0:
                raise RuntimeError("pcrcg_pyramid_ws_bytes rejected the configuration")
            arena = self.arena
            if fresh_arena or arena is None or arena.numel() < need or arena.device != device:
                arena = torch.empty(int(need), dtype=torch.uint8, device=device)
                if not fresh_arena:
                    self.arena = arena
            b = (Batch * nbatch)() if group else Batch()
            rc = L.pcrcg_pyramid_build_parts(pp, pn, lp, ln, k, ct.byref(self.cfg), arena.data_ptr(), arena.numel(),
                                             self.scratch.data_ptr(), ct.byref(b), h_len, self.status.data_ptr() + 4 * slot,
                                             ct.byref(deferred) if defer_restore else None, stream)
            if rc == -2 and self.shrink < 1.0:
                self.shrink = 1.0
                continue
            _lib.check(rc, "pcrcg_pyramid_build_parts")
            break
        lens_h = [[int(h_len[l * nb + i]) for i in range(nb)] for l in range(self.levels)]
        if defer_restore:
            return b, arena, lens_h, slot, deferred
        return b, arena, lens_h, slot

    def as_dict(self, b, arena, lens_h, part=None):
        base = arena.data_ptr()
        if part is not None:
            lens_h = [row[part[0]:part[0] + part[1]] for row in lens_h]
        nb = len(lens_h[0])

        def view(ptr, nbytes, dtype):
            off = ptr - base
            return arena[off:off + nbytes].view(dtype)

        def table(t):
            if t.idx and t.rows > 0 and t.cols > 0:
                return view(t.idx, t.rows * t.ld * 8, torch.int64).view(t.rows, t.ld)[:, :t.cols]
            if t.idx and t.rows > 0:
                return torch.zeros((t.rows, 0), dtype=torch.int64, device=arena.device)
            return torch.zeros((0, 1), dtype=torch.int64, device=arena.device)

        out = {"points": [], "neighbors": [], "pools": [], "upsamples": [], "stack_lengths": []}
        for l in range(b.n_levels):
            n = b.n_points[l]
# ... 86 lines not shown
```

pcrcg_amd/runner.py:

```python
import ctypes
import threading

import torch

from . import _lib
from .blocks import (LastUnaryBlock, NearestUpsampleBlock, ResnetBottleneckBlock, SimpleBlock, UnaryBlock,
                     aligned_weight)
from .gcn import AttentionalPropagation, SelfAttention

MAX_LEVELS, MAX_BLOCKS, MAX_GNN = 8, 32, 8
BLK_SIMPLE, BLK_RESNETB, BLK_UNARY, BLK_LAST_UNARY, BLK_UPSAMPLE = range(5)
_fp = ctypes.c_void_p


class Block(ctypes.Structure):
    _fields_ = [("type", ctypes.c_int), ("layer", ctypes.c_int), ("strided", ctypes.c_int),
                ("in_dim", ctypes.c_int), ("out_dim", ctypes.c_int), ("mid_dim", ctypes.c_int),
                ("extent", ctypes.c_float), ("kp", _fp), ("kp_w", _fp), ("kp_wt", _fp), ("kp_w_pad", _fp),
                ("cin_pad", ctypes.c_int), ("unary1", _fp), ("unary2", _fp),
                ("shortcut", _fp), ("mlp", _fp), ("mlp_ld", ctypes.c_int),
                ("mlp_skip", _fp), ("mlp_skip_ld", ctypes.c_int), ("skip_dim", ctypes.c_int)]


class GnnLayer(ctypes.Structure):
    _fields_ = [("cross", ctypes.c_int), ("edge1", _fp), ("edge2", _fp), ("conv3", _fp),
                ("wq", _fp), ("bq", _fp), ("wk", _fp), ("bk", _fp), ("wv", _fp), ("bv", _fp),
                ("wm", _fp), ("bm", _fp), ("w0", _fp), ("b0", _fp), ("w3", _fp), ("b3", _fp)]


class Model(ctypes.Structure):
    _fields_ = [("n_enc", ctypes.c_int), ("n_dec", ctypes.c_int), ("n_gnn", ctypes.c_int),
                ("enc", Block * MAX_BLOCKS), ("dec", Block * MAX_BLOCKS), ("gnn", GnnLayer * MAX_GNN),
                ("enc_skip", ctypes.c_int * MAX_BLOCKS), ("dec_concat", ctypes.c_int * MAX_BLOCKS),
                ("enc_out_dim", ctypes.c_int), ("gnn_dim", ctypes.c_int), ("heads", ctypes.c_int),
                ("knn_k", ctypes.c_int), ("final_dim", ctypes.c_int),
                ("bottle_w", _fp), ("bottle_b", _fp), ("proj_gnn_w", _fp), ("proj_gnn_b", _fp),
                ("proj_score_w", _fp), ("proj_score_b", _fp), ("temperature", ctypes.c_float),
                ("feature_bf16", ctypes.c_int)]


class Table(ctypes.Structure):
    _fields_ = [("idx", _fp), ("rows", ctypes.c_int), ("cols", ctypes.c_int), ("ld", ctypes.c_int)]


class Batch(ctypes.Structure):
    _fields_ = [("n_levels", ctypes.c_int), ("points", _fp * MAX_LEVELS), ("n_points", ctypes.c_int * MAX_LEVELS),
                ("neighbors", Table * MAX_LEVELS), ("pools", Table * MAX_LEVELS), ("upsamples", Table * MAX_LEVELS),
                ("features", _fp), ("feat_dim", ctypes.c_int), ("len_src_c", ctypes.c_int),
                ("stack_lengths", _fp * MAX_LEVELS)]


class PyramidCfg(ctypes.Structure):
    _fields_ = [("n_levels", ctypes.c_int), ("r_conv", ctypes.c_float * MAX_LEVELS), ("r_pool", ctypes.c_float * MAX_LEVELS),
                ("dl", ctypes.c_float * MAX_LEVELS), ("has_conv", ctypes.c_int * MAX_LEVELS),
                ("pooled", ctypes.c_int * MAX_LEVELS), ("limit", ctypes.c_int * MAX_LEVELS), ("tie_order", ctypes.c_int),
                ("group", ctypes.c_int), ("up_nearest", ctypes.c_int), ("shrink", ctypes.c_double), ("side_stream", _fp),
                ("side_stream2", _fp)]


from .ops import ReorderJob as ReorderJobC


class PyramidRestore(ctypes.Structure):
    _fields_ = [("njobs", ctypes.c_int), ("jobs", ReorderJobC * 12), ("tie_status", _fp)]


class Outputs(ctypes.Structure):
    _fields_ = [("feats_f", _fp), ("scores_overlap", _fp), ("scores_saliency", _fp)]


def _dense(t):
    t = t.detach()
    if t.dtype != torch.float32 or not t.is_cuda:
        raise RuntimeError("pcrcg_amd.runner: parameters must be float32 tensors on a HIP device")
    return t.contiguous()


class Runner:

    def __init__(self, model):
        self.model = model
        self.sig = None
        self.desc = None
        self.keep = []
        self.ws = {}
        self._lock = threading.Lock()
        self._params = None
        self._built = None
        self._seen = set()
        self._retired = []

    def __deepcopy__(self, memo):
        return None

    def __reduce__(self):
        return (type(None), ())

    def _signature(self):
        if self._params is None:
            self._params = list(self.model.parameters())
        return (bool(getattr(self.model, "feature_bf16", False)),) + tuple(
            (p.data_ptr(), p._version) for p in self._params)

    def invalidate(self):
        with self._lock:
            self._params, self.sig = None, None

    def _w(self, t):
        t = _dense(t)
        self.keep.append(t)
        return t.data_ptr()

    def _kp_weights(self, blk, kp):
        cin = kp.in_channels
        blk.kp_w = self._w(kp.weights.data)
        w = kp.weights.data
        if cin % 4 == 0 or cin < 4:
            blk.kp_w_pad, blk.cin_pad = None, 0
        else:
            cp = (cin + 3) // 4 * 4
            w = torch.zeros((kp.weights.shape[0], cp, kp.out_channels), dtype=torch.float32, device=kp.weights.device)
            w[:, :cin].copy_(kp.weights.data)
            blk.kp_w_pad, blk.cin_pad = self._w(w), cp
        k = w.shape[0] * w.shape[1]
        if cin == 1:
            w16 = torch.zeros((16, kp.out_channels), dtype=torch.float32, device=w.device)
            w16[:15].copy_(w.reshape(15, kp.out_channels))
            blk.kp_wt = self._w(w16.t())
        else:
            blk.kp_wt = self._w(w.reshape(k, kp.out_channels).t()) if k % 4 == 0 else None

    def _fill_block(self, blk, mod):
        if isinstance(mod, SimpleBlock):
            blk.type, blk.layer, blk.strided = BLK_SIMPLE, mod.layer_ind, int("strided" in mod.block_name)
            kp = mod.KPConv
            blk.in_dim, blk.out_dim, blk.mid_dim = kp.in_channels, kp.out_channels, kp.out_channels
            blk.extent = float(kp.KP_extent)
            blk.kp = self._w(kp.kernel_points.data)
            self._kp_weights(blk, kp)
        elif isinstance(mod, ResnetBottleneckBlock):
# ... 188 lines not shown
```

Baseline: 622.8.

## Precompute per-edge relative-position records during pyramid build for KPConv

Adds float4 edge records (neighbor offset relative to query plus index) that are written while the neighbor/pool tables are built or reordered. The KPConv MFMA kernel reads these instead of gathering support points through the index table, which removes the dependent idx-then-point gather. A device flag marks whether any support row is non-positive, so the per-neighbor positivity check can be skipped when it is not needed. The cost is extra memory, extra record-writing kernels in the pyramid stage, and a larger batch struct.

```diff
diff --git a/include/pcrcg.h b/include/pcrcg.h
--- a/include/pcrcg.h
+++ b/include/pcrcg.h
@@ -65,6 +65,7 @@
     const float* sup;
     const void* forest;
     int forest_ns, forest_nb;
+    void* rec;
 } pcrcg_reorder_job;
 size_t pcrcg_kdforest_ws_bytes(int ns, int nb);
 int pcrcg_kdforest_build(const float* sup, int ns, const int* slen, int nb, void* forest, size_t forest_bytes,
@@ -92,6 +93,13 @@
                                      void* wf_bf16, float* inv_n, void* ws, size_t ws_bytes, const int* walk, void* stream);
 int pcrcg_gather_max_walk(const float* x, int ns, int c, const int64_t* idx, int nq, int h, int ld_idx,
                           float* out, const int* walk, void* stream);
+
+int pcrcg_edge_records(const float* q_pts, int nq, const float* s_pts, int ns, const int64_t* idx, int cols, int ld_idx,
+                       const int* rows, int nrows, void* rec, int ld_rec, void* stream);
+int pcrcg_kpconv_aggregate_recs(const float* q_pts, int nq, const float* s_pts, int ns, const int64_t* idx,
+                                int h, int ld_idx, const float* x, int cin, const float* kp, float extent,
+                                float* wf, float* inv_n, void* ws, size_t ws_bytes, const int* walk, const void* rec,
+                                int* nonpos, void* stream);
 
 void pcrcg_profile_kpconv(int enable);
 int pcrcg_profile_kpconv_read(float* ms, int* nq, int* h, int* cin, int* cout, int* kind, int cap);
@@ -244,6 +252,8 @@
     int feat_dim;
     int len_src_c;
     const int* stack_lengths[PCRCG_MAX_LEVELS];
+    const void* neighbor_recs[PCRCG_MAX_LEVELS];
+    const void* pool_recs[PCRCG_MAX_LEVELS];
 } pcrcg_batch;
 
 typedef struct pcrcg_outputs {
@@ -270,6 +280,7 @@
     double shrink;
     void* side_stream;
     void* side_stream2;
+    int edge_records;
 } pcrcg_pyramid_cfg;
 typedef struct pcrcg_pyramid_restore {
     int njobs;
diff --git a/pcrcg_amd/_lib.py b/pcrcg_amd/_lib.py
--- a/pcrcg_amd/_lib.py
+++ b/pcrcg_amd/_lib.py
@@ -55,6 +55,11 @@
     "pcrcg_kpconv_aggregate_bf16_walk": (c_int, [c_void_p, c_int, c_void_p, c_int, c_void_p, c_int, c_int, c_void_p, c_int,
                                                  c_void_p, c_float, c_void_p, c_void_p, c_void_p, c_void_p, c_size_t,
                                                  c_void_p, c_void_p]),
+    "pcrcg_edge_records": (c_int, [c_void_p, c_int, c_void_p, c_int, c_void_p, c_int, c_int, c_void_p, c_int, c_void_p, c_int,
+                                   c_void_p]),
+    "pcrcg_kpconv_aggregate_recs": (c_int, [c_void_p, c_int, c_void_p, c_int, c_void_p, c_int, c_int, c_void_p, c_int,
+                                            c_void_p, c_float, c_void_p, c_void_p, c_void_p, c_size_t, c_void_p, c_void_p,
+                                            c_void_p, c_void_p]),
     "pcrcg_gather_max_walk": (c_int, [c_void_p, c_int, c_int, c_void_p, c_int, c_int, c_int, c_void_p, c_void_p, c_void_p]),
     "pcrcg_profile_kpconv": (None, [c_int]),
     "pcrcg_profile_kpconv_read": (c_int, [c_void_p, c_void_p, c_void_p, c_void_p, c_void_p, c_void_p, c_int]),
diff --git a/pcrcg_amd/csrc/common.h b/pcrcg_amd/csrc/common.h
--- a/pcrcg_amd/csrc/common.h
+++ b/pcrcg_amd/csrc/common.h
@@ -38,7 +38,7 @@
 
 bool instnorm_pack_ok(int c, int ldx, int ldy);
 int instnorm_apply_pack(const float* x, int n, int c, int ldx, const float* stats, const double* sums, double count, float eps,
-                        float slope, float* y, int ldy, const float* s_pts, float4* pk, hipStream_t st);
+                        float slope, float* y, int ldy, const float* s_pts, float4* pk, hipStream_t st, int* nonpos = nullptr);
 size_t colstats_ws_bytes(int c);
 int colstats_finalize(const double* partial, int nchunks, int c, double count, float eps, float* stats,
                       hipStream_t st);
@@ -62,7 +62,8 @@
 int kpconv_aggregate_rows(const float* q_pts, int nq, const float* s_pts, int ns, const int64_t* idx, int h, int ld_idx,
                           const float* x, int cin, const float* kp, float extent, float* wf, float* inv_n, void* ws,
                           size_t ws_bytes, hipStream_t st, bool pack, bool stream_out, int c1_ld = 0,
-                          const int* walk = nullptr);
+                          const int* walk = nullptr,
+                          const float4* rec = nullptr, int* nonpos = nullptr);
 int kpconv_aggregate_bf16(const float* q_pts, int nq, const float* s_pts, int ns, const int64_t* idx, int h, int ld_idx,
                           const float* x, unsigned short* x_bf16, int cin, const float* kp, float extent,
                           unsigned short* wf_bf16, float* inv_n, void* ws, size_t ws_bytes, hipStream_t st,
@@ -75,6 +76,7 @@
     const float* s_pts; float4* pk;
     int n; double count;
     float* stats_out = nullptr;
+    int* nonpos = nullptr;
 };
 int instnorm_apply_sums_multi(const NormJob* jobs, int count, int c, int ldx, float eps, int ldr, float slope, int ldy, bool pack,
                               hipStream_t st);
diff --git a/pcrcg_amd/csrc/edge_records.h b/pcrcg_amd/csrc/edge_records.h
--- /dev/null
+++ b/pcrcg_amd/csrc/edge_records.h
@@ -0,0 +1,25 @@
+#pragma once
+#include "common.h"
+
+namespace pcrcg {
+
+__device__ __forceinline__ void edge_record_row(const long long* __restrict__ idx_row, float4* __restrict__ rec_row, int cols,
+                                                float qx, float qy, float qz, const float* __restrict__ sup, int ns, int lane) {
+    for (int h = lane; h < cols; h += 64) {
+        const long long iv = idx_row[h];
+        const bool real = iv >= 0 && iv < ns;
+        float4 r = make_float4(0.f, 0.f, 0.f, __int_as_float(-1));
+        if (real) r = make_float4(sup[3 * iv] - qx, sup[3 * iv + 1] - qy, sup[3 * iv + 2] - qz, __int_as_float((int)iv));
+        rec_row[h] = r;
+    }
+}
+
+struct EdgeRecJob {
+    const int64_t* idx; float4* rec; const float* q; const float* sup; const int* rows;
+    int nq, nrows, ns, cols, ld_idx, ld_rec;
+    const int* qlen = nullptr; const int* slen = nullptr; int nb = 0, group = 0;
+};
+constexpr int kEdgeRecJobs = 32;
+int edge_records_jobs(const EdgeRecJob* jobs, int count, hipStream_t st);
+
+}
diff --git a/pcrcg_amd/csrc/kpconv.hip b/pcrcg_amd/csrc/kpconv.hip
--- a/pcrcg_amd/csrc/kpconv.hip
+++ b/pcrcg_amd/csrc/kpconv.hip
@@ -4,6 +4,7 @@
 #include <hip/hip_ext.h>
 
 #include "common.h"
+#include "edge_records.h"
 
 namespace pcrcg {
 
@@ -38,7 +39,8 @@
 
 __global__ void __launch_bounds__(256) k_row_positive(const float* __restrict__ x, int ns, int cin,
                                                        const float* __restrict__ s_pts, unsigned char* __restrict__ pos,
-                                                       float4* __restrict__ pk, unsigned short* __restrict__ xb) {
+                                                       float4* __restrict__ pk, unsigned short* __restrict__ xb,
+                                                       int* __restrict__ nonpos) {
     const int lane = threadIdx.x & 63;
     const int row = blockIdx.x * (blockDim.x >> 6) + (threadIdx.x >> 6);
     if (row >= ns) return;
@@ -53,6 +55,7 @@
     if (lane == 0) {
         pos[row] = s > 0.0f ? 1 : 0;
         pk[row] = make_float4(s_pts[3 * (long)row], s_pts[3 * (long)row + 1], s_pts[3 * (long)row + 2], s > 0.0f ? 1.f : 0.f);
+        if (nonpos && !(s > 0.0f)) *nonpos = 1;
     }
 }
 
@@ -71,12 +74,13 @@
                        __uint_as_float(u.y & 0xffff0000u));
 }
 
-template <int NB, bool NT_STORE, typename FT, bool TAIL = false>
+template <int NB, bool NT_STORE, typename FT, bool TAIL = false, bool REC = false>
 __global__ void __launch_bounds__(kWavesPerBlock * 64) k_kpconv_mfma(
     const float* __restrict__ q_pts, int nq, const float* __restrict__ s_pts, int ns,
     const long long* __restrict__ idx, int H, int ld_idx, const FT* __restrict__ x, int cin,
     const float* __restrict__ kp, float extent, const float4* __restrict__ pk, FT* __restrict__ wf,
-    float* __restrict__ inv_n, int nchunk, const int* __restrict__ walk) {
+    float* __restrict__ inv_n, int nchunk, const int* __restrict__ walk, const float4* __restrict__ rec,
+    const int* __restrict__ nonpos) {
     constexpr bool BF16 = sizeof(FT) == 2;
     constexpr int STEPS = NB >= 4 ? 2 : 4;
     const int lane = threadIdx.x & 63;
@@ -98,6 +102,7 @@
     const bool jvalid = j < K;
     const float kpx = jvalid ? kp[3 * j] : 0.f, kpy = jvalid ? kp[3 * j + 1] : 0.f, kpz = jvalid ? kp[3 * j + 2] : 0.f;
     const float inv_extent = 1.0f / extent;
+    const bool flags_needed = REC ? *nonpos != 0 : true;
 
     for (long item = gw; item < items; item += nw) {
         const int p = (int)(item / nchunk), chunk = (int)(item - (long)p * nchunk);
@@ -117,12 +122,25 @@
         float ta0 = 0.f, ta1 = 0.f, ta2 = 0.f, ta3 = 0.f;
         for (int hc = 0; hc < H; hc += 64) {
             const int h = hc + lane;
-            const long long iv = idx[(long)q * ld_idx + (h < H ? h : H - 1)];
-            const int i = (h < H && iv >= 0 && iv < ns) ? (int)iv : -1;
-            const long ic = i >= 0 ? i : 0;
-            const float4 sp = pk[ic];
-            const float px = sp.x - qx, py = sp.y - qy, pz = sp.z - qz;
-            if (chunk == 0) npos += __popcll(__ballot(i >= 0 && sp.w != 0.f));
+            int i;
+            float px, py, pz;
+            if constexpr (REC) {
+                const float4 r = rec[(long)q * ld_idx + (h < H ? h : H - 1)];
+                const int ri = __float_as_int(r.w);
+                i = (h < H && ri >= 0 && ri < ns) ? ri : -1;
+                px = r.x; py = r.y; pz = r.z;
+                if (chunk == 0) {
+                    if (flags_needed) npos += __popcll(__ballot(i >= 0 && pk[i >= 0 ? i : 0].w != 0.f));
+                    else npos += __popcll(__ballot(i >= 0));
+                }
+            } else {
+                const long long iv = idx[(long)q * ld_idx + (h < H ? h : H - 1)];
+                i = (h < H && iv >= 0 && iv < ns) ? (int)iv : -1;
+                const long ic = i >= 0 ? i : 0;
+                const float4 sp = pk[ic];
+                px = sp.x - qx; py = sp.y - qy; pz = sp.z - qz;
+                if (chunk == 0) npos += __popcll(__ballot(i >= 0 && sp.w != 0.f));
+            }
             const unsigned long long real_lanes = __ballot(i >= 0);
             const int hn_all = H - hc < 64 ? H - hc : 64;
             const int hn_real = real_lanes ? 64 - (int)__clzll(real_lanes) : 0;
@@ -332,6 +350,64 @@
     }
 }
 
+struct EdgeRecJobs { EdgeRecJob job[kEdgeRecJobs]; int row_begin[kEdgeRecJobs + 1]; int njobs; };
+__global__ void __launch_bounds__(256) k_edge_records(const EdgeRecJobs jobs) {
+    const int lane = threadIdx.x & 63;
+    const int t = __builtin_amdgcn_readfirstlane((int)(blockIdx.x * (blockDim.x >> 6) + (threadIdx.x >> 6)));
+    if (t >= jobs.row_begin[jobs.njobs]) return;
+    int ji = 0;
+    while (ji + 1 < jobs.njobs && t >= jobs.row_begin[ji + 1]) ++ji;
+    const EdgeRecJob& jb = jobs.job[ji];
+    const int local = t - jobs.row_begin[ji];
+    const int q = jb.rows ? __builtin_amdgcn_readfirstlane(jb.rows[local]) : local;
+    if (q < 0 || q >= jb.nq) return;
+    const float* sup = jb.sup;
+    int ns = jb.ns;
+    if (jb.qlen) {
+        int b = -1, qacc = 0;
+        for (int c = 0; c < jb.nb && b < 0; ++c) {
+            qacc += jb.qlen[c];
+            if (q < qacc) b = c;
+        }
+        if (b < 0) return;
+        const int g0 = jb.group > 0 ? (b / jb.group) * jb.group : 0, g1 = jb.group > 0 ? min(g0 + jb.group, jb.nb) : jb.nb;
+        int s0 = 0;
+        ns = 0;
+        for (int c = 0; c < g1; ++c) (c < g0 ? s0 : ns) += jb.slen[c];
+        sup += 3 * (long)s0;
+    }
+    const float qx = jb.q[3 * (long)q], qy = jb.q[3 * (long)q + 1], qz = jb.q[3 * (long)q + 2];
+    edge_record_row(reinterpret_cast<const long long*>(jb.idx) + (long)q * jb.ld_idx, jb.rec + (long)q * jb.ld_rec, jb.cols, qx, qy,
+                    qz, sup, ns, lane);
+}
+
+}
+
+int edge_records_jobs(const EdgeRecJob* jobs, int count, hipStream_t st) {
+    PCRCG_CHECK_ARG(count >= 0 && (count == 0 || jobs));
+    for (int j0 = 0; j0 < count; j0 += kEdgeRecJobs) {
+        EdgeRecJobs pack;
+        pack.njobs = 0;
+        long total = 0;
+        for (int j = j0; j < count && j < j0 + kEdgeRecJobs; ++j) {
+            const EdgeRecJob& jb = jobs[j];
+            PCRCG_CHECK_ARG(jb.nq >= 0 && jb.nrows >= 0 && jb.ns >= 0 && jb.cols >= 0 && jb.ld_idx >= jb.cols && jb.ld_rec >= jb.cols);
+            PCRCG_CHECK_ARG(jb.rows || jb.nrows <= jb.nq);
+            if (jb.nrows == 0 || jb.nq == 0 || jb.cols == 0) continue;
+            PCRCG_CHECK_ARG(jb.idx && jb.rec && jb.q && (jb.ns == 0 || jb.sup));
+            PCRCG_CHECK_ARG(!jb.qlen || (jb.slen && jb.nb >= 1 && jb.nb <= 64 && jb.group >= 0));
+            PCRCG_CHECK_ARG((reinterpret_cast<uintptr_t>(jb.rec) & 15) == 0);
+            pack.job[pack.njobs] = jb;
+            pack.row_begin[pack.njobs++] = (int)total;
+            total += jb.nrows;
+            PCRCG_CHECK_ARG(total <= 0x7fffffffL);
+        }
+        pack.row_begin[pack.njobs] = (int)total;
+        if (total == 0) continue;
+        hipLaunchKernelGGL(k_edge_records, dim3((unsigned)((total + 3) / 4)), dim3(256), 0, st, pack);
+        PCRCG_CHECK_LAUNCH();
+    }
+    return PCRCG_OK;
 }
 
 float4* kpconv_pk_ptr(void* ws, size_t ws_bytes, int ns) {
@@ -347,7 +423,7 @@
     unsigned char* pos = cv.take<unsigned char>((size_t)ns + 1);
     float4* pk = cv.take<float4>((size_t)ns + 1);
     PCRCG_CHECK_WS(cv);
-    if (ns > 0) hipLaunchKernelGGL(k_row_positive, dim3((ns + 3) / 4), dim3(256), 0, st, x, ns, cin, s_pts, pos, pk, x_bf16);
+    if (ns > 0) hipLaunchKernelGGL(k_row_positive, dim3((ns + 3) / 4), dim3(256), 0, st, x, ns, cin, s_pts, pos, pk, x_bf16, (int*)nullptr);
     PCRCG_CHECK_LAUNCH();
     return PCRCG_OK;
 }
@@ -391,6 +467,12 @@
                                  as_stream(stream), true, true, 0);
 }
 
+int pcrcg_edge_records(const float* q_pts, int nq, const float* s_pts, int ns, const int64_t* idx, int cols, int ld_idx,
+                       const int* rows, int nrows, void* rec, int ld_rec, void* stream) {
+    const EdgeRecJob one{idx, static_cast<float4*>(rec), q_pts, s_pts, rows, nq, rows ? nrows : nq, ns, cols, ld_idx, ld_rec};
+    return edge_records_jobs(&one, 1, as_stream(stream));
+}
+
 int pcrcg_kpconv_aggregate_bf16(const float* q_pts, int nq, const float* s_pts, int ns, const int64_t* idx, int h,
                                 int ld_idx, const float* x, int cin, const float* kp, float extent, void* x_bf16,
                                 void* wf_bf16, float* inv_n, void* ws, size_t ws_bytes, void* stream) {
@@ -403,7 +485,9 @@
 
 int kpconv_aggregate_rows(const float* q_pts, int nq, const float* s_pts, int ns, const int64_t* idx, int h, int ld_idx,
                           const float* x, int cin, const float* kp, float extent, float* wf, float* inv_n, void* ws,
-                          size_t ws_bytes, hipStream_t st, bool pack, bool stream_out, int c1_ld, const int* walk) {
+                          size_t ws_bytes, hipStream_t st, bool pack, bool stream_out, int c1_ld, const int* walk,
+                          const float4* rec, int* nonpos) {
+    PCRCG_CHECK_ARG(!rec || (nonpos && (reinterpret_cast<uintptr_t>(rec) & 15) == 0));
     PCRCG_CHECK_ARG(nq >= 0 && ns >= 0 && h >= 1 && ld_idx >= h && cin >= 1 && (c1_ld == 0 || c1_ld == K || c1_ld == K + 1));
     PCRCG_CHECK_ARG(extent > 0.0f);
     if (nq == 0) return PCRCG_OK;
@@ -434,7 +518,7 @@
     }
     if (pack && ns > 0)
         hipLaunchKernelGGL(k_row_positive, dim3((ns + 3) / 4), dim3(256), 0, st, x, ns, cin, s_pts, pos, pk,
-                           (unsigned short*)nullptr);
+                           (unsigned short*)nullptr, nonpos);
     KpProfScope prof_scope(st, nq, h, cin, 0, 0);
     const bool aligned = (cin % 4 == 0) && ((reinterpret_cast<uintptr_t>(x) & 15) == 0) &&
                          ((reinterpret_cast<uintptr_t>(wf) & 15) == 0);
@@ -446,13 +530,15 @@
     }
     if (cin == 68 || cin == 132) {
         const int blocks = walk ? blocks_walk(1) : blocks_for((long)nq);
-#define LAUNCH_T(NBV, NT)                                                                                                        \
-        hipExtLaunchKernelGGL((k_kpconv_mfma<NBV, NT, float, true>), dim3(blocks), dim3(kWavesPerBlock * 64), 0, st, prof_scope.a, \
+#define LAUNCH_T(NBV, NT) do { if (rec) LAUNCH_TR(NBV, NT, true); else LAUNCH_TR(NBV, NT, false); } while (0)
+#define LAUNCH_TR(NBV, NT, RC)                                                                                                   \
+        hipExtLaunchKernelGGL((k_kpconv_mfma<NBV, NT, float, true, RC>), dim3(blocks), dim3(kWavesPerBlock * 64), 0, st, prof_scope.a, \
                               prof_scope.b, 0, q_pts, nq, s_pts, ns, idx_ll, h, ld_idx, x, cin, kp, extent,                      \
-                              (const float4*)pk, wf, inv_n, 1, walk)
+                              (const float4*)pk, wf, inv_n, 1, walk, rec, (const int*)nonpos)
         if (cin == 132) { if (stream_out) LAUNCH_T(2, true); else LAUNCH_T(2, false); }
         else { if (stream_out) LAUNCH_T(1, true); else LAUNCH_T(1, false); }
 #undef LAUNCH_T
+#undef LAUNCH_TR
         PCRCG_CHECK_LAUNCH();
         return PCRCG_OK;
     }
@@ -461,10 +547,11 @@
     while (nb > 1 && ((long)nq * ((nblk + nb - 1) / nb) < 16384 || nblk % nb != 0)) nb >>= 1;
     const int nchunk = (nblk + nb - 1) / nb;
     const int blocks = walk ? blocks_walk(nchunk) : blocks_for((long)nq * nchunk);
-#define LAUNCH(NBV, NT)                                                                                                 \
-    hipExtLaunchKernelGGL((k_kpconv_mfma<NBV, NT, float>), dim3(blocks), dim3(kWavesPerBlock * 64), 0, st, prof_scope.a, \
+#define LAUNCH(NBV, NT) do { if (rec) LAUNCH_R(NBV, NT, true); else LAUNCH_R(NBV, NT, false); } while (0)
+#define LAUNCH_R(NBV, NT, RC)                                                                                           \
+    hipExtLaunchKernelGGL((k_kpconv_mfma<NBV, NT, float, false, RC>), dim3(blocks), dim3(kWavesPerBlock * 64), 0, st, prof_scope.a, \
                           prof_scope.b, 0, q_pts, nq, s_pts, ns, idx_ll, h, ld_idx, x, cin, kp, extent,                 \
-                          (const float4*)pk, wf, inv_n, nchunk, walk)
+                          (const float4*)pk, wf, inv_n, nchunk, walk, rec, (const int*)nonpos)
     if (stream_out) {
         if (nb == 4) LAUNCH(4, true);
         else if (nb == 2) LAUNCH(2, true);
@@ -475,6 +562,7 @@
         else LAUNCH(1, false);
     }
 #undef LAUNCH
+#undef LAUNCH_R
     PCRCG_CHECK_LAUNCH();
     return PCRCG_OK;
 }
@@ -505,7 +593,7 @@
 #define LAUNCHB(NBV)                                                                                                      \
     hipExtLaunchKernelGGL((k_kpconv_mfma<NBV, true, unsigned short>), dim3((int)blocks), dim3(kWavesPerBlock * 64), 0, st, \
                           prof_scope.a, prof_scope.b, 0, q_pts, nq, s_pts, ns, idx_ll, h, ld_idx, x_bf16, cin, kp, extent, \
-                          (const float4*)pk, wf_bf16, inv_n, nchunk, walk)
+                          (const float4*)pk, wf_bf16, inv_n, nchunk, walk, (const float4*)nullptr, (const int*)nullptr)
     if (nb == 4) LAUNCHB(4);
     else if (nb == 2) LAUNCHB(2);
     else LAUNCHB(1);
diff --git a/pcrcg_amd/csrc/pointops.hip b/pcrcg_amd/csrc/pointops.hip
--- a/pcrcg_amd/csrc/pointops.hip
+++ b/pcrcg_amd/csrc/pointops.hip
@@ -205,7 +205,7 @@
 
 struct NormMulti {
     const float* x[4]; const double* sums[4]; const float* res[4]; const double* res_sums[4]; float* y[4];
-    const float* s_pts[4]; float4* pk[4];
+    const float* s_pts[4]; float4* pk[4]; int* nonpos[4];
     int n[4]; double count[4];
     float* stats_out[4];
 };
@@ -268,7 +268,8 @@
 __global__ void __launch_bounds__(256) k_instnorm_apply4_pack(const float* __restrict__ x, int n, int c4, int ldx,
                                                                const float* __restrict__ stats, float slope,
                                                                float* __restrict__ y, int ldy,
-                                                               const float* __restrict__ s_pts, float4* __restrict__ pk) {
+                                                               const float* __restrict__ s_pts, float4* __restrict__ pk,
+                                                               int* __restrict__ nonpos) {
     const long e = (long)blockIdx.x * blockDim.x + threadIdx.x;
     if (e >= (long)n * c4) return;
     const long r = e / c4;
@@ -283,7 +284,10 @@
     *reinterpret_cast<float4*>(y + r * ldy + 4 * q) = v;
     float part = (v.x + v.y) + (v.z + v.w);
     for (int sh = c4 >> 1; sh >= 1; sh >>= 1) part += __shfl_xor(part, sh, 64);
-    if (q == 0) pk[r] = make_float4(s_pts[3 * r], s_pts[3 * r + 1], s_pts[3 * r + 2], part > 0.0f ? 1.f : 0.f);
+    if (q == 0) {
+        pk[r] = make_float4(s_pts[3 * r], s_pts[3 * r + 1], s_pts[3 * r + 2], part > 0.0f ? 1.f : 0.f);
+        if (nonpos && !(part > 0.0f)) *nonpos = 1;
+    }
 }
 
 __global__ void __launch_bounds__(256) k_instnorm_apply4_sums_pack(NormMulti mm, int c4, int ldx, float eps, float slope, int ldy,
@@ -294,6 +298,7 @@
     float* __restrict__ y = mm.y[g];
     const float* __restrict__ s_pts = mm.s_pts[g];
     float4* __restrict__ pk = mm.pk[g];
+    int* __restrict__ nonpos = mm.nonpos[g];
     const int n = mm.n[g];
     const double count = mm.count[g];
     if ((long)blockIdx.x * rows_per_block >= n) return;
@@ -312,7 +317,10 @@
         *reinterpret_cast<float4*>(y + r * ldy + 4 * q) = v;
         float part = (v.x + v.y) + (v.z + v.w);
         for (int sh = c4 >> 1; sh >= 1; sh >>= 1) part += __shfl_xor(part, sh, 64);
-        if (q == 0) pk[r] = make_float4(s_pts[3 * r], s_pts[3 * r + 1], s_pts[3 * r + 2], part > 0.0f ? 1.f : 0.f);
+        if (q == 0) {
+            pk[r] = make_float4(s_pts[3 * r], s_pts[3 * r + 1], s_pts[3 * r + 2], part > 0.0f ? 1.f : 0.f);
+            if (nonpos && !(part > 0.0f)) *nonpos = 1;
+        }
     }
 }
 
@@ -323,7 +331,7 @@
     return c % 4 == 0 && c4 >= 1 && c4 <= 64 && (c4 & (c4 - 1)) == 0 && ldx % 4 == 0 && ldy % 4 == 0;
 }
 int instnorm_apply_pack(const float* x, int n, int c, int ldx, const float* stats, const double* sums, double count, float eps,
-                        float slope, float* y, int ldy, const float* s_pts, float4* pk, hipStream_t st) {
+                        float slope, float* y, int ldy, const float* s_pts, float4* pk, hipStream_t st, int* nonpos) {
     PCRCG_CHECK_ARG(n >= 0 && instnorm_pack_ok(c, ldx, ldy) && ldx >= c && ldy >= c && (stats != nullptr) != (sums != nullptr));
     if (n == 0) return PCRCG_OK;
     PCRCG_CHECK_ARG(x && y && s_pts && pk && ((reinterpret_cast<uintptr_t>(x) | reinterpret_cast<uintptr_t>(y)) & 15) == 0);
@@ -331,9 +339,10 @@
     if (stats) {
         const long total = (long)n * c4;
         hipLaunchKernelGGL(k_instnorm_apply4_pack, dim3((unsigned)((total + 255) / 256)), dim3(256), 0, st, x, n, c4, ldx, stats,
-                           slope, y, ldy, s_pts, pk);
+                           slope, y, ldy, s_pts, pk, nonpos);
     } else {
         NormJob one{x, sums, nullptr, nullptr, y, s_pts, pk, n, count};
+        one.nonpos = nonpos;
         return instnorm_apply_sums_multi(&one, 1, c, ldx, eps, 0, slope, ldy, true, st);
     }
     PCRCG_CHECK_LAUNCH();
@@ -353,7 +362,7 @@
     for (int g = 0; g < 4; ++g) {
         const NormJob& j = jobs[g < count ? g : 0];
         mm.x[g] = j.x; mm.sums[g] = j.sums; mm.res[g] = j.res; mm.res_sums[g] = j.res_sums; mm.y[g] = j.y;
-        mm.s_pts[g] = j.s_pts; mm.pk[g] = j.pk; mm.n[g] = g < count ? j.n : 0; mm.count[g] = j.count;
+        mm.s_pts[g] = j.s_pts; mm.pk[g] = j.pk; mm.nonpos[g] = j.nonpos; mm.n[g] = g < count ? j.n : 0; mm.count[g] = j.count;
         mm.stats_out[g] = g < count ? j.stats_out : nullptr;
         if (g < count) {
             PCRCG_CHECK_ARG(j.n >= 0 && j.x && j.sums && j.y && j.count >= 1.0);
diff --git a/pcrcg_amd/csrc/pyramid.hip b/pcrcg_amd/csrc/pyramid.hip
--- a/pcrcg_amd/csrc/pyramid.hip
+++ b/pcrcg_amd/csrc/pyramid.hip
@@ -4,6 +4,7 @@
 #include <cstdlib>
 #include <vector>
 
+#include "edge_records.h"
 #include "frontend.h"
 
 namespace pcrcg {
@@ -58,6 +59,7 @@
 struct TableRec {
     RadiusSearch s;
     int kind;
+    float4* rec;
     int level, q_level, sup_level;
 };
 
@@ -142,6 +144,7 @@
     MetaView meta;
     int* tie_status;
     std::vector<TableRec> tables;
+    std::vector<EdgeRecJob> rec_jobs;
     void* forest[2] = {nullptr, nullptr};
     int forest_ns[2] = {0, 0}, forest_nb[2] = {0, 0};
     EventBox events;
@@ -224,6 +227,12 @@
         s.idx = A.take<int64_t>((size_t)nq * limit);
         s.count = want_ties ? A.take<int>((size_t)nq) : nullptr;
         s.tie_rows = want_ties ? A.take<int>((size_t)nq) : nullptr;
+        t.rec = (cfg->edge_records && kind != 2) ? A.take<float4>((size_t)nq * limit) : nullptr;
+        if (t.rec) {
+            EdgeRecJob j{s.idx, t.rec, q, level_pts[sup_level], nullptr, nq, nq, ns, limit, limit, limit};
+            j.qlen = qlen; j.slen = slen; j.nb = nb; j.group = group;
+            B.rec_jobs.push_back(j);
+        }
         s.max_count = &m.max_count(0); s.status = &m.status(); s.tie_count = want_ties ? &m.tie_rows() : nullptr;
         if (!A.ok()) return PCRCG_EWORKSPACE;
         if (!dry) PCRCG_PROPAGATE(radius_search(s, RadiusPass::first, st));
@@ -286,6 +295,7 @@
             carried_r = 2 * r_pool;
         }
     }
+    if (!dry && !B.rec_jobs.empty()) PCRCG_PROPAGATE(edge_records_jobs(B.rec_jobs.data(), (int)B.rec_jobs.size(), st));
     if (!dry && want_ties && f_st != st) {
         PCRCG_PROPAGATE(B.events.make(&B.forests_done));
         PCRCG_CHECK_HIP(hipEventRecord(B.forests_done, f_st));
@@ -317,6 +327,7 @@
             PCRCG_PROPAGATE(radius_search(B.tables[i].s, RadiusPass::redo, st));
             ++redone;
         }
+        if (redone && !B.rec_jobs.empty()) PCRCG_PROPAGATE(edge_records_jobs(B.rec_jobs.data(), (int)B.rec_jobs.size(), st));
         if (redone) PCRCG_PROPAGATE(fetch(h_scratch, B.meta.w, hm.words(), B.lens_all, L * nb, st));
     }
     auto group_rows = [&](int l, int p, int* row0, int* rows) {
@@ -342,6 +353,7 @@
             o.neighbors[l] = pcrcg_table{nullptr, rows, 0, 1};
             o.pools[l] = pcrcg_table{nullptr, 0, 0, 1};
             o.upsamples[l] = pcrcg_table{nullptr, 0, 0, 1};
+            o.neighbor_recs[l] = o.pool_recs[l] = nullptr;
         }
     }
     pcrcg_pyramid_restore local;
@@ -364,6 +376,10 @@
             if (t.kind == 0) out[p].neighbors[t.level] = tab;
             else if (t.kind == 1) out[p].pools[t.level] = tab;
             else out[p].upsamples[t.level] = tab;
+            if (t.rec) {
+                float4* rec = t.rec + (size_t)row0 * s.cols;
+                (t.kind == 0 ? out[p].neighbor_recs : out[p].pool_recs)[t.level] = rec;
+            }
         }
         const int widest = m.widest(), tie_rows = m.tie_rows();
         if (B.want_ties && widest > 0 && tie_rows > 0 && R.njobs < PCRCG_MAX_REORDER_JOBS) {
@@ -375,6 +391,7 @@
             j.max_count = widest < 8192 ? widest : 8192;
             j.cols = s.cols; j.radius = s.radius; j.group = group;
             j.sup = B.level_pts[fi]; j.forest = B.forest[fi]; j.forest_ns = B.forest_ns[fi]; j.forest_nb = B.forest_nb[fi];
+            j.rec = t.rec;
         }
     }
     R.tie_status = B.tie_status;
diff --git a/pcrcg_amd/csrc/runner.hip b/pcrcg_amd/csrc/runner.hip
--- a/pcrcg_amd/csrc/runner.hip
+++ b/pcrcg_amd/csrc/runner.hip
@@ -346,7 +346,7 @@
 }
 
 void kpconv(Ctx& c, const Batches& B, Walks& W, const pcrcg_block& blk, const Mat& x, const Mat& y, Stat* st = nullptr,
-            void* const* packed_ws = nullptr) {
+            void* const* packed_ws = nullptr, int* const* packed_flag = nullptr) {
     const int l = blk.layer;
     const size_t m = c.mark();
     Mat xin = x;
@@ -367,9 +367,13 @@
     float* inv_n[GMAX];
     void* ws[GMAX];
     size_t wsb[GMAX];
+    const float4* rec[GMAX];
+    int* nonpos[GMAX];
     for (int g = 0; g < c.G; ++g) {
         const pcrcg_batch& b = *B.b[g];
         tab[g] = blk.strided ? &b.pools[l] : &b.neighbors[l];
+        rec[g] = static_cast<const float4*>(blk.strided ? b.pool_recs[l] : b.neighbor_recs[l]);
+        nonpos[g] = (packed_flag && packed_flag[g]) ? packed_flag[g] : static_cast<int*>(c.zraw(sizeof(int)));
         q[g] = blk.strided ? b.points[l + 1] : b.points[l];
         nq[g] = blk.strided ? b.n_points[l + 1] : b.n_points[l];
         ns[g] = b.n_points[l];
@@ -410,7 +414,7 @@
             const bool packed = kk != 16 && packed_ws && packed_ws[g] && xin.p[g] == x.p[g];
             c.check(kpconv_aggregate_rows(q[g], nq[g], B.b[g]->points[l], ns[g], tab[g]->idx, tab[g]->cols, tab[g]->ld, xin.p[g], cin,
                                           blk.kp, blk.extent, wf.p[g], inv_n[g], ws[g], wsb[g], c.st, !packed,
-                                          true, kk == 16 ? 16 : 0, walks ? walks[g] : nullptr));
+                                          true, kk == 16 ? 16 : 0, walks ? walks[g] : nullptr, rec[g], nonpos[g]));
         }
         if (kp_wt)
             linear(c, wf, kp_wt, kk, nullptr, y, st, inv_n);
@@ -442,7 +446,7 @@
 }
 
 bool norm_act_pack(Ctx& c, const Batches& B, int layer, const Mat& t, float slope, const Mat& u, Stat* ts, void* const* kp_ws,
-                   const size_t* kp_ws_bytes) {
+                   const size_t* kp_ws_bytes, int* const* kp_flag) {
     if (c.bf16 || !instnorm_pack_ok(t.cols, t.ld, u.ld) || u.ld != u.cols) return false;
     const size_t m = c.mark();
     float* stats = static_cast<float*>(c.raw(sizeof(float) * 2 * t.cols));
@@ -455,6 +459,7 @@
         for (int g = 0; g < c.G; ++g) {
             nj.j[g].s_pts = B.b[g]->points[layer];
             nj.j[g].pk = kpconv_pk_ptr(kp_ws[g], kp_ws_bytes[g], t.rows[g]);
+            nj.j[g].nonpos = kp_flag[g];
             ok = ok && nj.j[g].pk != nullptr;
         }
         if (ok) {
@@ -470,11 +475,11 @@
             if (!pk) c.check(PCRCG_EWORKSPACE);
             else if (ts && ts->has_sums(g))
                 c.check(instnorm_apply_pack(t.p[g], t.rows[g], t.cols, t.ld, nullptr, static_cast<const double*>(ts->partials[g]),
-                                            (double)t.rows[g], 1e-5f, slope, u.p[g], u.ld, s_pts, pk, c.st));
+                                            (double)t.rows[g], 1e-5f, slope, u.p[g], u.ld, s_pts, pk, c.st, kp_flag[g]));
             else {
                 col_stats(c, t, g, ts, stats, ws, wsb);
                 c.check(instnorm_apply_pack(t.p[g], t.rows[g], t.cols, t.ld, stats, nullptr, 0.0, 1e-5f, slope, u.p[g], u.ld, s_pts,
-                                            pk, c.st));
+                                            pk, c.st, kp_flag[g]));
             }
         }
     c.release(m);
@@ -489,6 +494,7 @@
     Mat x = feats;
     void* kp_ws[GMAX] = {};
     size_t kp_wsb[GMAX] = {};
+    int* kp_flag[GMAX] = {};
     bool packed = false;
     if (blk.unary1) {
         Mat t = c.gemm_out(feats.rows, blk.mid_dim, feats.cols), u = c.mat(feats.rows, blk.mid_dim);
@@ -498,15 +504,16 @@
             for (int g = 0; g < c.G; ++g) {
                 kp_wsb[g] = pcrcg_kpconv_ws_bytes(feats.rows[g]);
                 kp_ws[g] = c.raw(kp_wsb[g]);
-            }
-            packed = norm_act_pack(c, B, blk.layer, t, 0.1f, u, &ts, kp_ws, kp_wsb);
+                kp_flag[g] = static_cast<int*>(c.zraw(sizeof(int)));
+            }
+            packed = norm_act_pack(c, B, blk.layer, t, 0.1f, u, &ts, kp_ws, kp_wsb, kp_flag);
         }
         if (!packed) norm_act(c, t, 0.1f, u, &ts);
         x = u;
     }
     Mat k = c.gemm_out(nq, blk.mid_dim, PCRCG_KPOINTS * kp_cin(blk, x)), kn = c.mat(nq, blk.mid_dim);
     Stat ks = stat_buffer(c, nq, blk.mid_dim);
-    kpconv(c, B, W, blk, x, k, &ks, packed ? kp_ws : nullptr);
+    kpconv(c, B, W, blk, x, k, &ks, packed ? kp_ws : nullptr, packed ? kp_flag : nullptr);
     Mat u2 = c.gemm_out(nq, blk.out_dim, blk.mid_dim);
     Stat u2s = stat_buffer(c, nq, blk.out_dim);
     if (!linear_norm(c, k, &ks, 0.1f, blk.unary2, blk.mid_dim, nullptr, u2, &u2s)) {
diff --git a/pcrcg_amd/csrc/tieorder.hip b/pcrcg_amd/csrc/tieorder.hip
--- a/pcrcg_amd/csrc/tieorder.hip
+++ b/pcrcg_amd/csrc/tieorder.hip
@@ -2,6 +2,7 @@
 #include <cstdlib>
 
 #include "block_scan.h"
+#include "edge_records.h"
 #include "frontend.h"
 
 namespace pcrcg {
@@ -790,6 +791,31 @@
         row[j] = j < n ? (long long)((int)(unsigned)(sorted[j] & 0xFFFFFFFFull) - seg) : (long long)pad;
 }
 
+__global__ void __launch_bounds__(256) k_reorder_records(const ReorderJobs jobs) {
+    const int lane = threadIdx.x & 63, wave = uni((int)(threadIdx.x >> 6));
+    const int t = blockIdx.x * (int)(blockDim.x >> 6) + wave;
+    if (t >= jobs.row_begin[jobs.njobs]) return;
+    int ji = 0;
+    while (ji + 1 < jobs.njobs && t >= jobs.row_begin[ji + 1]) ++ji;
+    const pcrcg_reorder_job& jb = jobs.job[ji];
+    if (!jb.rec) return;
+    const KdView& v = jobs.view[ji];
+    const int local = t - jobs.row_begin[ji];
+    const int qi = jb.rows ? uni(jb.rows[local]) : local;
+    if (qi < 0 || qi >= jb.nq) return;
+    int b = 0, qacc = 0;
+    while (b < jb.nbq - 1 && qi >= qacc + jb.qlen[b]) { qacc += jb.qlen[b]; ++b; }
+    int seg = v.soff[jb.cloud0], pad = v.nodes[jb.cloud0 + jb.nbq - 1].right - seg;
+    if (jb.group > 0) {
+        const int g0 = jb.cloud0 + (b / jb.group) * jb.group, g1 = min(g0 + jb.group, jb.cloud0 + jb.nbq);
+        seg = v.soff[g0];
+        pad = v.nodes[g1 - 1].right - seg;
+    }
+    const float* q = jb.q;
+    edge_record_row(reinterpret_cast<const long long*>(jb.idx) + (long)qi * jb.cols, static_cast<float4*>(jb.rec) + (long)qi * jb.cols,
+                    jb.cols, q[3 * (long)qi], q[3 * (long)qi + 1], q[3 * (long)qi + 2], jobs.sup[ji] + 3 * (long)seg, pad, lane);
+}
+
 }
 }
 
@@ -870,6 +896,9 @@
     const size_t lds = per_wave * waves * sizeof(u64);
     if (lds > 64 * 1024) PCRCG_GRANT_LDS(k_reorder);
     hipLaunchKernelGGL(k_reorder, dim3((total + waves - 1) / waves), dim3(waves * 64), lds, st, pack, width, status);
+    bool recs = false;
+    for (int i = 0; i < pack.njobs; ++i) recs = recs || pack.job[i].rec != nullptr;
+    if (recs) hipLaunchKernelGGL(k_reorder_records, dim3((total + 3) / 4), dim3(256), 0, st, pack);
     PCRCG_CHECK_LAUNCH();
     return PCRCG_OK;
 }
@@ -894,6 +923,7 @@
     j.sup = nullptr;
     j.forest = nullptr;
     j.forest_ns = j.forest_nb = 0;
+    j.rec = nullptr;
     return pcrcg_radius_reorder_jobs(&j, 1, sup, ns, nb, forest, status, stream);
 }
 }
diff --git a/pcrcg_amd/csrc/walk.hip b/pcrcg_amd/csrc/walk.hip
--- a/pcrcg_amd/csrc/walk.hip
+++ b/pcrcg_amd/csrc/walk.hip
@@ -154,6 +154,13 @@
                                  as_stream(stream), true, true, 0, walk);
 }
 
+int pcrcg_kpconv_aggregate_recs(const float* q_pts, int nq, const float* s_pts, int ns, const int64_t* idx, int h, int ld_idx,
+                                const float* x, int cin, const float* kp, float extent, float* wf, float* inv_n, void* ws,
+                                size_t ws_bytes, const int* walk, const void* rec, int* nonpos, void* stream) {
+    return kpconv_aggregate_rows(q_pts, nq, s_pts, ns, idx, h, ld_idx, x, cin, kp, extent, wf, inv_n, ws, ws_bytes,
+                                 as_stream(stream), true, true, 0, walk, static_cast<const float4*>(rec), nonpos);
+}
+
 int pcrcg_kpconv_aggregate_bf16_walk(const float* q_pts, int nq, const float* s_pts, int ns, const int64_t* idx, int h,
                                      int ld_idx, const float* x, int cin, const float* kp, float extent, void* x_bf16,
                                      void* wf_bf16, float* inv_n, void* ws, size_t ws_bytes, const int* walk, void* stream) {
diff --git a/pcrcg_amd/ops.py b/pcrcg_amd/ops.py
--- a/pcrcg_amd/ops.py
+++ b/pcrcg_amd/ops.py
@@ -199,7 +199,7 @@
                 ("idx", ctypes.c_void_p), ("nq", ctypes.c_int), ("nbq", ctypes.c_int), ("cloud0", ctypes.c_int),
                 ("nrows", ctypes.c_int), ("max_count", ctypes.c_int), ("cols", ctypes.c_int), ("radius", ctypes.c_float),
                 ("group", ctypes.c_int), ("sup", ctypes.c_void_p), ("forest", ctypes.c_void_p), ("forest_ns", ctypes.c_int),
-                ("forest_nb", ctypes.c_int)]
+                ("forest_nb", ctypes.c_int), ("rec", ctypes.c_void_p)]
 
 
 class KdForest:
diff --git a/pcrcg_amd/pyramid.py b/pcrcg_amd/pyramid.py
--- a/pcrcg_amd/pyramid.py
+++ b/pcrcg_amd/pyramid.py
@@ -167,7 +167,7 @@
 
     STATUS_RING = 64
 
-    def __init__(self, config, neighborhood_limits, tie_order=None, up_nearest=False):
+    def __init__(self, config, neighborhood_limits, tie_order=None, up_nearest=False, edge_records=True):
         config = as_config(config)
         if tie_order is None:
             tie_order = os.environ.get("PCRCG_TIE_ORDER", "auto")
@@ -181,6 +181,7 @@
             c.has_conv[l], c.pooled[l], c.limit[l] = int(lv["has_conv"]), int(lv["pooled"]), int(neighborhood_limits[l])
         c.tie_order = 0 if tie_order == "index" else 1
         c.up_nearest = int(bool(up_nearest))
+        c.edge_records = int(bool(edge_records))
         self.cfg, self.levels = c, len(plan)
         self.scratch = torch.empty(512, dtype=_I32, pin_memory=True)
         self.status = torch.zeros(self.STATUS_RING, dtype=_I32, pin_memory=True)
diff --git a/pcrcg_amd/runner.py b/pcrcg_amd/runner.py
--- a/pcrcg_amd/runner.py
+++ b/pcrcg_amd/runner.py
@@ -47,7 +47,7 @@
     _fields_ = [("n_levels", ctypes.c_int), ("points", _fp * MAX_LEVELS), ("n_points", ctypes.c_int * MAX_LEVELS),
                 ("neighbors", Table * MAX_LEVELS), ("pools", Table * MAX_LEVELS), ("upsamples", Table * MAX_LEVELS),
                 ("features", _fp), ("feat_dim", ctypes.c_int), ("len_src_c", ctypes.c_int),
-                ("stack_lengths", _fp * MAX_LEVELS)]
+                ("stack_lengths", _fp * MAX_LEVELS), ("neighbor_recs", _fp * MAX_LEVELS), ("pool_recs", _fp * MAX_LEVELS)]
 
 
 class PyramidCfg(ctypes.Structure):
@@ -55,7 +55,7 @@
                 ("dl", ctypes.c_float * MAX_LEVELS), ("has_conv", ctypes.c_int * MAX_LEVELS),
                 ("pooled", ctypes.c_int * MAX_LEVELS), ("limit", ctypes.c_int * MAX_LEVELS), ("tie_order", ctypes.c_int),
                 ("group", ctypes.c_int), ("up_nearest", ctypes.c_int), ("shrink", ctypes.c_double), ("side_stream", _fp),
-                ("side_stream2", _fp)]
+                ("side_stream2", _fp), ("edge_records", ctypes.c_int)]
 
 
 from .ops import ReorderJob as ReorderJobC
```

Result: slower. 612.5 (-1.6%).
